# MoonLab-YH/AOD_MEH_HUA

Hardware: AMD Instinct MI355X
Metric: images/sec train+HUA-score, RetinaNet-R50 VOC 512^2 (higher is better)
Workload: dtype bf16x3

## Files before the change

aod_meh_hua_amd/_C.py:

```python
import ctypes as C
import os

import torch

_HERE = os.path.dirname(os.path.abspath(__file__))
LIB_PATH = os.environ.get('AOD_HIP_LIB') or os.path.join(_HERE, 'lib', 'libaodhip.so')


class AodHipError(RuntimeError):
    pass


if not os.path.exists(LIB_PATH):
    raise ImportError(f'{LIB_PATH} is missing: run `python -m aod_meh_hua_amd.build` (hipcc, gfx950). '
                      'There is no CPU fallback for the MEH/HUA hot path.')
lib = C.CDLL(LIB_PATH)


class ConvSeg(C.Structure):
    _fields_ = [('B', C.c_int32), ('H', C.c_int32), ('W', C.c_int32), ('OH', C.c_int32), ('OW', C.c_int32),
                ('src_row0', C.c_int64), ('dst_row0', C.c_int64)]


class ConvDesc(C.Structure):
# ... 76 lines not shown
    'aod_upsample2x_add_bwd': (C.c_int, [P, P, I32, I32, I32, I32, I32, I32, P]),
    'aod_upsample2x_add_to': (C.c_int, [P, P, P, I32, I32, I32, I32, I32, I32, P]),
    'aod_upsample2x_add_bwd_set': (C.c_int, [P, P, I32, I32, I32, I32, I32, I32, P]),
    'aod_act_bwd': (C.c_int, [P, P, P, P, P, P, P, P, P, P, I64, I32, I32, I32, P]),
    'aod_add_relu': (C.c_int, [P, P, P, I64, P]),
    'aod_pad_cast_colsum': (C.c_int, [P, P, P, P, I64, I32, I32, I32, P]),
    'aod_assign_ws_bytes': (SZ, [I32, I32]),
    'aod_max_iou_assign': (C.c_int, [P, P, I64, I32, P, P, P, I32, F32, F32, F32, I32, I32, P, P, P, P, P, P, P, P, P, I32, P, P]),
    'aod_loss_partials_len': (SZ, [I64]),
    'aod_edl_focal_l1_fwd': (C.c_int, [P, P, P, P, P, P, I64, I32, F32, F32, P, P, P, P]),
    'aod_edl_focal_l1_bwd': (C.c_int, [P, P, P, P, P, P, I64, I32, F32, F32, P, P, P, F32, I32, P, P, I32, I32, I32, I32, P]),
    'aod_edl_focal_elem': (C.c_int, [P, P, I64, I32, F32, F32, P, P, P]),
    'aod_meh_loss_fwd': (C.c_int, [P, P, P, I64, P, P, P]),
    'aod_meh_loss_bwd': (C.c_int, [P, P, P, I64, P, P, I32, I32, I32, P]),
    'aod_sigmoid_focal_l1_fwd': (C.c_int, [P, P, P, P, P, P, I64, I32, F32, F32, P, P, P, P]),
    'aod_sigmoid_focal_l1_bwd': (C.c_int, [P, P, P, P, P, P, I64, I32, F32, F32, P, P, P, F32, I32, P, P, I32, I32, I32, I32, P]),
    'aod_sigmoid_focal_elem': (C.c_int, [P, P, I64, I32, F32, F32, P, P, P]),
    'aod_sigmoid_focal_l1_levels_fwd': (C.c_int, [P, P, P, P, P, P, I32, P, I32, F32, F32, P, P, P, P, I32, P, P, P]),
    'aod_sigmoid_focal_l1_levels_bwd': (C.c_int, [P, P, P, P, P, P, I32, P, I32, F32, F32, P, P, P, P, P, I32, I32, I32, I32, P]),
    'aod_loss_levels_partials_len': (SZ, [I32, P]),
    'aod_edl_focal_l1_levels_fwd': (C.c_int, [P, P, P, P, P, P, I32, P, I32, F32, F32, P, P, P, P, I32, P, P, P]),
    'aod_edl_focal_l1_levels_bwd': (C.c_int, [P, P, P, P, P, P, I32, P, I32, F32, F32, P, P, P, P, P, I32, I32, I32, I32, P]),
    'aod_meh_loss_levels_fwd': (C.c_int, [P, P, P, I32, P, P, P, P]),
    'aod_meh_loss_levels_bwd': (C.c_int, [P, P, P, I32, P, P, P, I32, I32, I32, P]),
    'aod_meh_loss_fwd_ex': (C.c_int, [P, P, P, I64, I32, P, P, P]),
    'aod_meh_loss_bwd_ex': (C.c_int, [P, P, P, I64, I32, P, P, I32, I32, I32, P]),
    'aod_meh_loss_levels_fwd_ex': (C.c_int, [P, P, P, I32, P, I32, P, P, P]),
    'aod_meh_loss_levels_bwd_ex': (C.c_int, [P, P, P, I32, P, I32, P, P, I32, I32, I32, P]),
    'aod_softmax_rowmax': (C.c_int, [P, I32, I64, I32, F32, P, P, I32, P]),
    'aod_topk_stable': (C.c_int, [P, I32, I64, I32, P, I64, P]),
    'aod_pre_nms_levels': (C.c_int, [I32, P, P, P, P, P, P, I32, I32, F32, I32, I32, P, P, P, P, F32, P, P, P, P, P, P, P, I64, P]),
    'aod_gather_decode': (C.c_int, [P, P, P, P, P, I32, I64, I32, I32, I64, P, P, P, P, F32, P, P, P, P, I64, I64, I64, I32, P]),
    'aod_nms_ws_bytes': (SZ, [I32, I32, I32]),
    'aod_multiclass_nms': (C.c_int, [P, P, I32, I32, I32, F32, F32, I32, P, P, P, P, P, P]),
    'aod_eval_match': (C.c_int, [P, P, P, P, P, P, P, I32, I32, I32, P, I32, P, P]),
    'aod_coco_match': (C.c_int, [P, P, P, P, P, P, P, P, I32, I32, I32, P, I32, P, I32, P, P]),
    'aod_hua_ws_bytes': (SZ, [I32, I32]),
    'aod_hua_score': (C.c_int, [P, P, P, P, P, P, P, P, P, I32, I32, I32, I32, I32, F32, F32, F32, I32, U64, P, I32, I32, I32, P, P, I32, P, P, P]),
    'aod_hua_score_ex': (C.c_int, [P, P, P, P, P, P, P, P, P, I32, I32, I32, I32, I32, F32, F32, F32, I32, U64, P, I32, I32, I32, P, P, I32, P,
                                   I32, P, P, P, P]),
    'aod_hua_score_ex2': (C.c_int, [P, P, P, P, P, P, P, P, P, I32, I32, I32, I32, I32, F32, F32, F32, I32, U64, P, I32, I32, I32, P, P, I32, P,
                                    I32, I32, P, P, P, P]),
    'aod_maxpool_fwd': (C.c_int, [P, P, I32, I32, I32, I32, I32, I32, I32, I32, I32, P]),
    'aod_maxpool_bwd': (C.c_int, [P, P, P, I32, I32, I32, I32, I32, I32, I32, I32, I32, P]),
    'aod_l2norm_fwd': (C.c_int, [P, P, P, I64, I32, F32, P]),
    'aod_l2norm_bwd': (C.c_int, [P, P, P, P, P, I64, I32, F32, P]),
    'aod_ssd_loss_fwd': (C.c_int, [P, P, P, P, P, P, I32, I32, I32, I32, I32, F32, P, P, P, P]),
    'aod_ssd_loss_bwd': (C.c_int, [P, P, P, P, P, P, P, P, I32, I32, I32, I32, F32, P, P, P, P, P, P]),
    'aod_synth_normal_images': (C.c_int, [P, I32, I64, U64, P, P]),
    'aod_image_xform': (C.c_int, [P, P, I32, I32, I32, P, P]),
    'aod_x3_split': (C.c_int, [P, P, I64, I32, P]),
    'aod_x3_merge': (C.c_int, [P, P, I64, I32, P]),
    'aod_x3_add': (C.c_int, [P, P, P, I64, P]),
    'aod_x3_nchw_f32_to_s2d': (C.c_int, [P, P, I32, I32, I32, I32, P]),
    'aod_x3_maxpool3x3s2': (C.c_int, [P, P, I32, I32, I32, I32, P]),
    'aod_x3_upsample2x_add_to': (C.c_int, [P, P, P, I32, I32, I32, I32, I32, I32, P]),
    'aod_x3_upsample2x_add_bwd_set': (C.c_int, [P, P, I32, I32, I32, I32, I32, I32, P]),
    'aod_x3_act_bwd': (C.c_int, [P, P, P, P, I64, I32, I32, P]),
    'aod_x3_pad_cast_colsum': (C.c_int, [P, P, P, P, I64, I32, P]),
    'aod_x3_pad_cast_colsum_map': (C.c_int, [P, P, P, P, I64, I32, P, P]),
    'aod_x3_nchw_f32_to_nhwc': (C.c_int, [P, P, I32, I32, I32, I32, P]),
    'aod_x3_maxpool_fwd': (C.c_int, [P, P, I32, I32, I32, I32, I32, I32, I32, I32, I32, P]),
    'aod_x3_maxpool_bwd': (C.c_int, [P, P, P, I32, I32, I32, I32, I32, I32, I32, I32, I32, P]),
    'aod_x3_l2norm_fwd': (C.c_int, [P, P, P, I64, I32, F32, P]),
    'aod_x3_l2norm_bwd': (C.c_int, [P, P, P, P, P, I64, I32, F32, P]),
    'aod_sgd_multi': (C.c_int, [P, P, P, P, I32, F32, P, F32, F32, I32, F32, P]),
    'aod_sgd_multi_clipped': (C.c_int, [P, P, P, P, I32, F32, P, F32, F32, I32, F32, P, P]),
    'aod_grad_norm_multi': (C.c_int, [P, P, I32, F32, F32, I32, P, I64, P, P]),
    'aod_ensemble_mi_partials_len': (SZ, [I32, P, I32]),
    'aod_ensemble_mi': (C.c_int, [P, I32, I32, P, I32, I32, P, P, I64, P]),
    'aod_dropout2d_masks': (C.c_int, [P, P, I32, P, I32, I32, F32, U64, C.c_uint32, P]),
    'aod_dropout2d_apply': (C.c_int, [P, P, I64, I32, I32, I32, I32, P]),
    'aod_dropout2d_apply_multi': (C.c_int, [P, P, I64, I32, I32, P, P, P, I32, I32, P]),
    'aod_pool_descriptor': (C.c_int, [P, I32, P, P, I32, I32, I32, P, I64, P]),
    'aod_kcenter_chunk': (C.c_int, []),
    'aod_kcenter_ws_len': (SZ, [I64]),
    'aod_kcenter_greedy': (C.c_int, [P, I64, I32, P, I64, I64, P, P, P, P, P]),
    'aod_kcenter_greedy_ex': (C.c_int, [P, I64, I32, P, I64, I64, P, P, P, P, P, I32]),
    'aod_cdal_chunk': (C.c_int, []),
    'aod_cdal_ws_len': (SZ, [I32, P, I32, I32]),
    'aod_cdal_descriptor': (C.c_int, [P, I32, P, I32, I32, F32, P, I64, P, I64, P]),
    'aod_det_uncertainty': (C.c_int, [P, P, P, P, P, I32, I32, I32, I32, I32, I32, I32, F32, P, P, P, P]),
    'aod_loc_stability_max_levels': (C.c_int, []),
    'aod_pixel_noise': (C.c_int, [P, P, I32, I32, I32, I32, P, P, F32, I32, U64, P, P]),
    'aod_loc_stability': (C.c_int, [P, P, P, I32, I32, I32, F32, I32, I32, P, P, P]),
}
for _n, (_r, _a) in _SIGS.items():
    if hasattr(lib, _n):
        getattr(lib, _n).restype = _r
        getattr(lib, _n).argtypes = _a
lib.aod_last_error.restype = C.c_char_p


def ptr(t):
    if t is None:
        return None
    if not t.is_cuda:
        raise AodHipError('aod_meh_hua_amd ops need tensors on the MI355X (cuda:N); got a CPU tensor. There is no CPU fallback.')
    return C.c_void_p(t.data_ptr())


def stream():
    return C.c_void_p(torch.cuda.current_stream().cuda_stream)


def check(rc, name='aod'):
# ... 7 lines not shown
```

aod_meh_hua_amd/build.py:

```python
import os
import subprocess
import sys

HERE = os.path.dirname(os.path.abspath(__file__))
CSRC = os.path.join(HERE, 'csrc')
LIB = os.path.join(HERE, 'lib', 'libaodhip.so')
FLAGS = ['--offload-arch=gfx950', '-O3', '-std=c++17', '-fPIC', '-ffp-contract=off', '-Wno-unused-result']


def sources():
    return sorted(os.path.join(CSRC, f) for f in os.listdir(CSRC) if f.endswith(('.hip', '.cpp')))


def source_digest():
    import hashlib
    h = hashlib.sha256()
    for f in sources() + [os.path.join(CSRC, 'common.h'), os.path.join(CSRC, 'pointwise.h'), os.path.join(CSRC, 'conv_x3p.h'), os.path.join(CSRC, 'conv_params.h'), os.path.join(HERE, '..', 'include', 'aod_hip.h')]:
        if os.path.exists(f):
            h.update(os.path.basename(f).encode())
            h.update(open(f, 'rb').read())
    return h.hexdigest()[:16]


def needs_build():
    if not os.path.exists(LIB):
        return True
    t = os.path.getmtime(LIB)
    deps = sources() + [os.path.join(CSRC, 'common.h'), os.path.join(CSRC, 'pointwise.h'), os.path.join(CSRC, 'conv_x3p.h'), os.path.join(CSRC, 'conv_params.h'),
                        os.path.join(HERE, '..', 'include', 'aod_hip.h')]
    return any(os.path.getmtime(d) > t for d in deps)


def build(force=False, verbose=True):
    if not force and not needs_build():
        return LIB
    os.makedirs(os.path.dirname(LIB), exist_ok=True)
    objdir = os.path.join(HERE, 'lib', 'obj')
    os.makedirs(objdir, exist_ok=True)
    hipcc = os.environ.get('HIPCC', '/opt/rocm/bin/hipcc')
    procs = []
    objs = []
    for src in sources():
        obj = os.path.join(objdir, os.path.basename(src) + '.o')
        objs.append(obj)
        cmd = [hipcc] + FLAGS + (['-x', 'hip'] if src.endswith('.hip') else []) + ['-c', src, '-o', obj]
        procs.append((src, subprocess.Popen(cmd, stdout=subprocess.PIPE, stderr=subprocess.STDOUT)))
    for src, p in procs:
        out = p.communicate()[0].decode()
        if p.returncode != 0:
            raise RuntimeError(f'hipcc failed on {src}:\n{out}')
        if verbose and out.strip():
            print(out)
    subprocess.check_call([hipcc, '--offload-arch=gfx950', '-shared', '-fPIC', '-o', LIB] + objs)
    if verbose:
        print('built', LIB)
    return LIB


if __name__ == '__main__':
    build(force='--force' in sys.argv)
```

aod_meh_hua_amd/csrc/losses.hip:

```cpp
#include "common.h"

#define FLT_MIN_F 1.17549435e-38f
constexpr int LB = 256;
constexpr int MAXC = 96;

__device__ __forceinline__ float focal_pow(float b, float gamma) { return gamma == 2.f ? b * b : powf(b, gamma); }

#ifndef AOD_LOSS_FAST_MATH
#define AOD_LOSS_FAST_MATH 1
#endif
#if AOD_LOSS_FAST_MATH
__device__ __forceinline__ float l_exp(float x) { return __builtin_amdgcn_exp2f(x * 1.44269504088896341f); }
__device__ __forceinline__ float l_log(float x) { return __builtin_amdgcn_logf(x) * 0.693147180559945309f; }
__device__ __forceinline__ float l_div(float a, float b) { return a * __builtin_amdgcn_rcpf(b); }
#else
__device__ __forceinline__ float l_exp(float x) { return expf(x); }
__device__ __forceinline__ float l_log(float x) { return logf(x); }
__device__ __forceinline__ float l_div(float a, float b) { return a / b; }
#endif

template <int LPR>
__device__ __forceinline__ float grp_max(float v) {
  if (LPR >= 2) v = fmaxf(v, __shfl_xor(v, 1, 64));
  if (LPR >= 4) v = fmaxf(v, __shfl_xor(v, 2, 64));
  return v;
}
template <int LPR>
__device__ __forceinline__ float grp_sum(float v) {
  if (LPR >= 2) v += __shfl_xor(v, 1, 64);
  if (LPR >= 4) v += __shfl_xor(v, 2, 64);
  return v;
}

template <int CT, int LPR>
__device__ __forceinline__ float edl_row_fwd(const float* x, int n, int c0, long long label, float gamma, float alpha, float* p) {
  float m = -INFINITY;
#pragma unroll
  for (int c = 0; c < CT; ++c) if (c < n) m = fmaxf(m, x[c]);
  m = grp_max<LPR>(m);
  float S = 0.f;
#pragma unroll
  for (int c = 0; c < CT; ++c) if (c < n) { p[c] = l_exp(x[c] - m); S += p[c]; }
  S = grp_sum<LPR>(S);
  float tot = 0.f;
#pragma unroll
  for (int c = 0; c < CT; ++c) if (c < n) {
    const float pr = l_div(p[c], S);
    p[c] = pr;
    const float z = l_log(l_div(pr, 1.f - pr + 1e-9f) + 1e-9f);
    const float q = l_div(1.f, 1.f + l_exp(-z));
    const bool pos = label == c0 + c;
    const float lg = l_log(fmaxf(pos ? q : 1.f - q, FLT_MIN_F));
    float l;
    if (pos) l = -alpha * focal_pow(1.f - q, gamma) * lg;
    else l = -(1.f - alpha) * focal_pow(q, gamma) * lg;
    tot += l;
  }
  return grp_sum<LPR>(tot);
}

constexpr int FORM_EDL = 0, FORM_SIGMOID = 1;

__device__ __forceinline__ float sig_focal_term(float x, bool pos, float gamma, float alpha, float* gz) {
  const float q = l_div(1.f, 1.f + l_exp(-x));
  const float lg = l_log(fmaxf(pos ? q : 1.f - q, FLT_MIN_F));
  if (gz) {
    if (pos) *gz = -alpha * focal_pow(1.f - q, gamma) * (1.f - q - gamma * q * lg);
    else *gz = -(1.f - alpha) * focal_pow(q, gamma) * (gamma * (1.f - q) * lg - q);
  }
  return pos ? -alpha * focal_pow(1.f - q, gamma) * lg : -(1.f - alpha) * focal_pow(q, gamma) * lg;
}

template <int CT, int LPR>
__device__ __forceinline__ float sig_row_fwd(const float* x, int n, int c0, long long label, float gamma, float alpha) {
  float tot = 0.f;
#pragma unroll
  for (int c = 0; c < CT; ++c) if (c < n) tot += sig_focal_term(x[c], label == c0 + c, gamma, alpha, nullptr);
  return grp_sum<LPR>(tot);
}

constexpr int MAXLV = 8;
struct LossLevels { int n; int blk_end[MAXLV]; long long row_end[MAXLV]; };
__device__ __forceinline__ void level_of_block(const LossLevels& lv, int bid, int& level, int& blk0, long long& row0, long long& rend) {
  level = 0; blk0 = 0; row0 = 0; rend = lv.row_end[0];
#pragma unroll
  for (int q = 0; q + 1 < MAXLV; ++q)
    if (bid >= lv.blk_end[q]) { level = q + 1; blk0 = lv.blk_end[q]; row0 = lv.row_end[q]; rend = lv.row_end[q + 1]; }
}
static int fill_levels(LossLevels& lv, int nlevels, const int64_t* level_rows, int rows_per_block, long long& total_rows) {
  lv.n = nlevels;
  long long r = 0, b = 0;
  for (int l = 0; l < MAXLV; ++l) {
    if (l < nlevels) { r += level_rows[l]; b += (level_rows[l] + rows_per_block - 1) / rows_per_block; }
    lv.row_end[l] = r;
    lv.blk_end[l] = l < nlevels ? (int)b : 0x7fffffff;
  }
  total_rows = r;
  return (int)b;
}

template <int FORM, int CT, int LPR>
__global__ __launch_bounds__(LB) void edl_l1_fwd_kernel(const float* __restrict__ cls, const long long* __restrict__ labels,
                                                        const float* __restrict__ lw, const float* __restrict__ bp,
                                                        const float* __restrict__ bt, const float* __restrict__ bw, const LossLevels lv, int C,
                                                        float gamma, float alpha, float* __restrict__ loss_noR, float* __restrict__ partials) {
  extern __shared__ __attribute__((aligned(16))) float srow[];
  constexpr int RB = LB / LPR;
  const int P = C | 1;
  int level, blk0; long long row0, rend;
  level_of_block(lv, (int)blockIdx.x, level, blk0, row0, rend);
  const long long r0 = row0 + (long long)((int)blockIdx.x - blk0) * RB;
  const int nr = (int)min((long long)RB, rend - r0);
  aod_stage_rows<LB>(cls + r0 * C, srow, nr, C, P);
  __syncthreads();
  float s_cls = 0.f, s_box = 0.f, s_nor = 0.f;
  const int lrow = threadIdx.x / LPR, part = threadIdx.x % LPR;
  const bool live = lrow < nr;
  const int row = live ? lrow : nr - 1;
  const int cpl = (C + LPR - 1) / LPR, c0 = part * cpl;
  const int n = min(cpl, C - c0);
  {
    const long long r = r0 + row;
    float x[CT], p[CT];
#pragma unroll
    for (int c = 0; c < CT; ++c) x[c] = c < n ? srow[row * P + c0 + c] : 0.f;
    const float l = FORM == FORM_SIGMOID ? sig_row_fwd<CT, LPR>(x, n, c0, labels[r], gamma, alpha)
                                         : edl_row_fwd<CT, LPR>(x, n, c0, labels[r], gamma, alpha, p);
    if (live && part == 0) {
      loss_noR[r] = l;
      s_nor = l;
      s_cls = l * lw[r];
      if (bp) {
        const f32x4 a = *reinterpret_cast<const f32x4*>(bp + r * 4), b = *reinterpret_cast<const f32x4*>(bt + r * 4),
                    w = *reinterpret_cast<const f32x4*>(bw + r * 4);
        for (int j = 0; j < 4; ++j) s_box += fabsf(a[j] - b[j]) * w[j];
      }
    }
  }
  __shared__ float red[3][LB / 64];
  s_cls = wave_sum(s_cls); s_box = wave_sum(s_box); s_nor = wave_sum(s_nor);
  if ((threadIdx.x & 63) == 0) { red[0][threadIdx.x >> 6] = s_cls; red[1][threadIdx.x >> 6] = s_box; red[2][threadIdx.x >> 6] = s_nor; }
  __syncthreads();
  if (threadIdx.x < 3) {
    float v = 0.f;
    for (int i = 0; i < LB / 64; ++i) v += red[threadIdx.x][i];
    partials[(long long)blockIdx.x * 3 + threadIdx.x] = v;
  }
}

__global__ __launch_bounds__(256) void reduce_partials_kernel(const float* __restrict__ partials, long long nblocks, int k, float* __restrict__ out) {
  __shared__ float red[4];
// ... 162 lines not shown
#pragma unroll
    for (int c = 0; c < CT; ++c) x[c] = c < n ? srow[row * P + c0 + c] : 0.f;
    float m = -INFINITY, S = 0.f;
    if (FORM == FORM_EDL) {
#pragma unroll
      for (int c = 0; c < CT; ++c) if (c < n) m = fmaxf(m, x[c]);
      m = grp_max<LPR>(m);
#pragma unroll
      for (int c = 0; c < CT; ++c) if (c < n) { p[c] = l_exp(x[c] - m); S += p[c]; }
      S = grp_sum<LPR>(S);
    }
    const long long label = labels[r];
    const float gc_ = g_div ? g_cls[gl] / g_div[gl] : g_cls[gl];
    const float gn_ = g_noR ? (g_noR_bcast ? (g_div ? g_noR[gl] / g_div[2 * nlv + gl] : g_noR[gl]) : g_noR[r]) : g_noR_s;
    const float coef = gc_ * lw[r] + gn_;
    float dot = 0.f;
    if (FORM == FORM_SIGMOID) {
      if (live) {
#pragma unroll
        for (int c = 0; c < CT; ++c) if (c < n) {
          float gz;
          sig_focal_term(x[c], label == c0 + c, gamma, alpha, &gz);
          srow[row * P + c0 + c] = coef * gz;
        }
      }
    } else {
#pragma unroll
      for (int c = 0; c < CT; ++c) if (c < n) {
        const float pr = l_div(p[c], S);
        p[c] = pr;
        const float om = 1.f - pr + 1e-9f;
        const float u = l_div(pr, om);
        const float z = l_log(u + 1e-9f);
        const float q = l_div(1.f, 1.f + l_exp(-z));
        const bool pos = label == c0 + c;
        const float lg = l_log(fmaxf(pos ? q : 1.f - q, FLT_MIN_F));
        float gz;
        if (pos) gz = -alpha * focal_pow(1.f - q, gamma) * (1.f - q - gamma * q * lg);
        else gz = -(1.f - alpha) * focal_pow(q, gamma) * (gamma * (1.f - q) * lg - q);
        const float g = l_div(coef * gz * (1.f + 1e-9f), om * om * (u + 1e-9f));
        gp[c] = g;
        dot += pr * g;
      }
      dot = grp_sum<LPR>(dot);
      if (live) {
#pragma unroll
        for (int c = 0; c < CT; ++c) if (c < n) srow[row * P + c0 + c] = p[c] * (gp[c] - dot);
      }
    }
    if (live && part == 0 && bp && grad_bbox) {
      const float gb = g_div ? g_bbox[gl] / g_div[nlv + gl] : g_bbox[gl];
      const long long bb = (r / A) * pitch_box + (r % A) * 4;
      for (int j = 0; j < 4; ++j) {
        const float d = bp[r * 4 + j] - bt[r * 4 + j];
        const float sgn = d > 0.f ? 1.f : (d < 0.f ? -1.f : 0.f);
        const float gx = sgn * bw[r * 4 + j] * gb;
        if (OUT_BF16) ((bf16_t*)grad_bbox)[bb + j] = (bf16_t)gx;
        else ((float*)grad_bbox)[bb + j] = gx;
      }
    }
  }
  __syncthreads();
  {
    const int drow = LB / C, dcol = LB - drow * C;
    int row = (int)threadIdx.x / C, c = (int)threadIdx.x - row * C;
    for (int i = threadIdx.x; i < tot; i += LB) {
      const long long o = s_obase[row] + c;
      const float gx = srow[row * P + c];
      if (OUT_BF16) ((bf16_t*)grad_cls)[o] = (bf16_t)gx;
      else ((float*)grad_cls)[o] = gx;
      row += drow; c += dcol;
      if (c >= C) { c -= C; ++row; }
    }
  }
}

#define AOD_FOCAL_BWD_(FORM_, BF, LPR_)                                                                                                    \
  hipLaunchKernelGGL((edl_l1_bwd_kernel<FORM_, BF, 24, LPR_>), dim3((unsigned)nb), dim3(LB), (size_t)(LB / LPR_) * (C | 1) * 4, (hipStream_t)stream, cls, \
                     (const long long*)labels, label_w, bbox_pred, bbox_tgt, bbox_w, lv, C, gamma, alpha, g_cls, g_bbox, g_noR, \
                     g_noR_scalar, g_noR_is_scalar, grad_cls, grad_bbox, A, pitch_cls, pitch_box, g_lstride, g_div, nlv_)
#define AOD_FOCAL_BWD_F(FORM_)                                                                                                             \
  do {                                                                                                                                     \
    if (out_bf16) { if (C <= 24) AOD_FOCAL_BWD_(FORM_, true, 1); else AOD_FOCAL_BWD_(FORM_, true, 4); }                                    \
    else { if (C <= 24) AOD_FOCAL_BWD_(FORM_, false, 1); else AOD_FOCAL_BWD_(FORM_, false, 4); }                                           \
  } while (0)
#define AOD_FOCAL_BWD()                                                                                                                    \
  do {                                                                                                                                     \
    if (form == FORM_SIGMOID) AOD_FOCAL_BWD_F(FORM_SIGMOID); else AOD_FOCAL_BWD_F(FORM_EDL);                                               \
  } while (0)
static int focal_l1_bwd(int form, const char* nm, const float* cls, const int64_t* labels, const float* label_w, const float* bbox_pred,
                        const float* bbox_tgt, const float* bbox_w, int64_t nrows, int C, float gamma, float alpha, const float* g_cls,
                        const float* g_bbox, const float* g_noR, float g_noR_scalar, int g_noR_is_scalar, void* grad_cls, void* grad_bbox,
                        int out_bf16, int A, int pitch_cls, int pitch_box, aod_stream_t stream) {
  AOD_CHECK_ARG(nrows >= 0, "%s: negative row count", nm);
  if (nrows == 0) return 0;
  AOD_CHECK_ARG(cls && labels && label_w && g_cls && grad_cls, "%s: null pointer", nm);
  AOD_CHECK_ARG(C >= 1 && C <= MAXC && A >= 1 && pitch_cls >= A * C, "%s: bad C/A/pitch", nm);
  AOD_CHECK_ARG(!grad_bbox || (bbox_pred && bbox_tgt && bbox_w && g_bbox && pitch_box >= A * 4), "%s: bbox args", nm);
  LossLevels lv; long long tot;
  const long long nb = fill_levels(lv, 1, &nrows, LB / edl_lpr(C), tot);
  const int g_lstride = 0, nlv_ = 1;
  const float* const g_div = nullptr;
  AOD_FOCAL_BWD();
  AOD_LAUNCH_CHECK();
  return 0;
}
extern "C" int aod_edl_focal_l1_bwd(const float* cls, const int64_t* labels, const float* label_w, const float* bbox_pred,
                                    const float* bbox_tgt, const float* bbox_w, int64_t nrows, int C, float gamma, float alpha,
                                    const float* g_cls, const float* g_bbox, const float* g_noR, float g_noR_scalar, int g_noR_is_scalar,
                                    void* grad_cls, void* grad_bbox, int out_bf16, int A, int pitch_cls, int pitch_box, aod_stream_t stream) {
  return focal_l1_bwd(FORM_EDL, "edl_bwd", cls, labels, label_w, bbox_pred, bbox_tgt, bbox_w, nrows, C, gamma, alpha, g_cls, g_bbox, g_noR, g_noR_scalar,
                      g_noR_is_scalar, grad_cls, grad_bbox, out_bf16, A, pitch_cls, pitch_box, stream);
}
extern "C" int aod_sigmoid_focal_l1_bwd(const float* cls, const int64_t* labels, const float* label_w, const float* bbox_pred,
                                        const float* bbox_tgt, const float* bbox_w, int64_t nrows, int C, float gamma, float alpha,
                                        const float* g_cls, const float* g_bbox, const float* g_noR, float g_noR_scalar, int g_noR_is_scalar,
                                        void* grad_cls, void* grad_bbox, int out_bf16, int A, int pitch_cls, int pitch_box, aod_stream_t stream) {
  return focal_l1_bwd(FORM_SIGMOID, "sigmoid_focal_bwd", cls, labels, label_w, bbox_pred, bbox_tgt, bbox_w, nrows, C, gamma, alpha, g_cls, g_bbox, g_noR,
                      g_noR_scalar, g_noR_is_scalar, grad_cls, grad_bbox, out_bf16, A, pitch_cls, pitch_box, stream);
}

static int focal_l1_levels_bwd(int form, const char* nm, const float* cls, const int64_t* labels, const float* label_w, const float* bbox_pred,
                               const float* bbox_tgt, const float* bbox_w, int nlevels, const int64_t* level_rows, int C, float gamma, float alpha,
                               const float* g_sums, const float* divisors, const float* g_noR_rows, void* grad_cls, void* grad_bbox, int out_bf16,
                               int A, int pitch_cls, int pitch_box, aod_stream_t stream) {
  AOD_CHECK_ARG(nlevels >= 1 && nlevels <= MAXLV && level_rows, "%s: 1..8 levels", nm);
  AOD_CHECK_ARG(level_rows_ok(nlevels, level_rows), "%s: negative row count", nm);
  AOD_CHECK_ARG(cls && labels && label_w && g_sums && grad_cls, "%s: null pointer", nm);
  AOD_CHECK_ARG(C >= 1 && C <= MAXC && A >= 1 && pitch_cls >= A * C, "%s: bad C/A/pitch", nm);
  AOD_CHECK_ARG(!grad_bbox || (bbox_pred && bbox_tgt && bbox_w && pitch_box >= A * 4), "%s: bbox args", nm);
  LossLevels lv; long long tot;
  const int nb = fill_levels(lv, nlevels, level_rows, LB / edl_lpr(C), tot);
  if (nb == 0) return 0;
  const float* g_cls = g_sums; const float* g_bbox = g_sums + nlevels;
  const float* g_noR = g_noR_rows ? g_noR_rows : g_sums + 2 * nlevels;
  const float g_noR_scalar = 0.f; const int g_noR_is_scalar = g_noR_rows ? 0 : 1, g_lstride = 1, nlv_ = nlevels;
  const float* const g_div = divisors;
  AOD_FOCAL_BWD();
  AOD_LAUNCH_CHECK();
  return 0;
}
#undef AOD_FOCAL_BWD
#undef AOD_FOCAL_BWD_F
#undef AOD_FOCAL_BWD_
extern "C" int aod_edl_focal_l1_levels_bwd(const float* cls, const int64_t* labels, const float* label_w, const float* bbox_pred,
                                           const float* bbox_tgt, const float* bbox_w, int nlevels, const int64_t* level_rows, int C, float gamma,
                                           float alpha, const float* g_sums, const float* divisors, const float* g_noR_rows, void* grad_cls,
                                           void* grad_bbox, int out_bf16, int A, int pitch_cls, int pitch_box, aod_stream_t stream) {
  return focal_l1_levels_bwd(FORM_EDL, "edl_levels_bwd", cls, labels, label_w, bbox_pred, bbox_tgt, bbox_w, nlevels, level_rows, C, gamma, alpha, g_sums,
                             divisors, g_noR_rows, grad_cls, grad_bbox, out_bf16, A, pitch_cls, pitch_box, stream);
}
extern "C" int aod_sigmoid_focal_l1_levels_bwd(const float* cls, const int64_t* labels, const float* label_w, const float* bbox_pred,
                                               const float* bbox_tgt, const float* bbox_w, int nlevels, const int64_t* level_rows, int C, float gamma,
                                               float alpha, const float* g_sums, const float* divisors, const float* g_noR_rows, void* grad_cls,
                                               void* grad_bbox, int out_bf16, int A, int pitch_cls, int pitch_box, aod_stream_t stream) {
  return focal_l1_levels_bwd(FORM_SIGMOID, "sigmoid_focal_levels_bwd", cls, labels, label_w, bbox_pred, bbox_tgt, bbox_w, nlevels, level_rows, C, gamma,
                             alpha, g_sums, divisors, g_noR_rows, grad_cls, grad_bbox, out_bf16, A, pitch_cls, pitch_box, stream);
}

__device__ __forceinline__ float sign0(float x) { return x > 0.f ? 1.f : (x < 0.f ? -1.f : 0.f); }
template <int FORM>
__global__ __launch_bounds__(256) void meh_fwd_kernel(const float* __restrict__ lam, const float* __restrict__ loss, const float* __restrict__ bw4,
                                                      const LossLevels lv, float* __restrict__ partials) {
  float s = 0.f;
  int level, blk0; long long row0, n;
  level_of_block(lv, (int)blockIdx.x, level, blk0, row0, n);
  const long long i = row0 + (long long)((int)blockIdx.x - blk0) * 256 + threadIdx.x;
  if (i < n) {
    if (FORM == 1) {
      s = fabsf(fabsf(lam[i] + 1e-9f - loss[i]) * bw4[i * 4]);
    } else if (FORM == 2) {
      const float d = fabsf(logf(lam[i] + 1e-9f + 1.f) - logf(loss[i] + 1.f)) * bw4[i * 4];
      s = d * d;
    } else {
      const float d = fabsf(lam[i] + 1e-9f - loss[i]) * bw4[i * 4];
      s = d * d;
    }
  }
  __shared__ float red[4];
  s = wave_sum(s);
  if ((threadIdx.x & 63) == 0) red[threadIdx.x >> 6] = s;
  __syncthreads();
  if (threadIdx.x == 0) partials[blockIdx.x] = red[0] + red[1] + red[2] + red[3];
}
template <bool OUT_BF16, int FORM>
__global__ void meh_bwd_kernel(const float* __restrict__ lam, const float* __restrict__ loss, const float* __restrict__ bw4, const LossLevels lv,
                               const float* __restrict__ g, void* __restrict__ grad, int A, int pitch, int g_lstride) {
  int level, blk0; long long row0, n;
  level_of_block(lv, (int)blockIdx.x, level, blk0, row0, n);
  const long long i = row0 + (long long)((int)blockIdx.x - blk0) * 256 + threadIdx.x;
  if (i < n) {
    const float w = bw4[i * 4];
    float v;
    if (FORM == 1) {
      const float d = lam[i] + 1e-9f - loss[i];
      v = g[level * g_lstride] * sign0(fabsf(d) * w) * w * sign0(d);
    } else if (FORM == 2) {
      const float x = lam[i] + 1e-9f + 1.f;
      const float d = logf(x) - logf(loss[i] + 1.f);
      v = g[level * g_lstride] * 2.f * (fabsf(d) * w) * w * sign0(d) / x;
    } else {
      v = g[level * g_lstride] * 2.f * w * w * (lam[i] + 1e-9f - loss[i]);
    }
    const long long o = (i / A) * pitch + (i % A);
    if (OUT_BF16) ((bf16_t*)grad)[o] = (bf16_t)v; else ((float*)grad)[o] = v;
  }
}
#define AOD_MEH_FWD(nb_)                                                                                                                   \
  do {                                                                                                                                     \
    if (form == 1) hipLaunchKernelGGL(meh_fwd_kernel<1>, dim3((unsigned)(nb_)), dim3(256), 0, (hipStream_t)stream, lam, loss_noR, bbox_w4, lv, partials); \
    else if (form == 2) hipLaunchKernelGGL(meh_fwd_kernel<2>, dim3((unsigned)(nb_)), dim3(256), 0, (hipStream_t)stream, lam, loss_noR, bbox_w4, lv, partials); \
    else hipLaunchKernelGGL(meh_fwd_kernel<0>, dim3((unsigned)(nb_)), dim3(256), 0, (hipStream_t)stream, lam, loss_noR, bbox_w4, lv, partials); \
  } while (0)
#define AOD_MEH_BWD_(BF, F_, nb_, ls_)                                                                                                     \
  hipLaunchKernelGGL((meh_bwd_kernel<BF, F_>), dim3((unsigned)(nb_)), dim3(256), 0, (hipStream_t)stream, lam, loss_noR, bbox_w4, lv, g, grad_lam, A, pitch, ls_)
#define AOD_MEH_BWD(nb_, ls_)                                                                                                              \
  do {                                                                                                                                     \
    if (out_bf16) { if (form == 1) AOD_MEH_BWD_(true, 1, nb_, ls_); else if (form == 2) AOD_MEH_BWD_(true, 2, nb_, ls_); else AOD_MEH_BWD_(true, 0, nb_, ls_); } \
    else { if (form == 1) AOD_MEH_BWD_(false, 1, nb_, ls_); else if (form == 2) AOD_MEH_BWD_(false, 2, nb_, ls_); else AOD_MEH_BWD_(false, 0, nb_, ls_); } \
  } while (0)
extern "C" int aod_meh_loss_fwd_ex(const float* lam, const float* loss_noR, const float* bbox_w4, int64_t n, int form, float* out_sum,
                                   float* partials, aod_stream_t stream) {
  AOD_CHECK_ARG(lam && loss_noR && bbox_w4 && out_sum && partials, "meh_fwd: null pointer");
  AOD_CHECK_ARG(form >= 0 && form <= 2, "meh_fwd: form must be 0 (L2), 1 (L1) or 2 (MSLE)");
  if (n == 0) return 0;
  LossLevels lv; long long tot;
  const long long nb = fill_levels(lv, 1, &n, 256, tot);
  AOD_MEH_FWD(nb);
  hipLaunchKernelGGL(reduce_partials_kernel, dim3(1), dim3(256), 0, (hipStream_t)stream, partials, nb, 1, out_sum);
  AOD_LAUNCH_CHECK();
  return 0;
}
extern "C" int aod_meh_loss_fwd(const float* lam, const float* loss_noR, const float* bbox_w4, int64_t n, float* out_sum, float* partials,
                                aod_stream_t stream) {
  return aod_meh_loss_fwd_ex(lam, loss_noR, bbox_w4, n, 0, out_sum, partials, stream);
}
extern "C" int aod_meh_loss_levels_fwd_ex(const float* lam, const float* loss_noR, const float* bbox_w4, int nlevels, const int64_t* level_rows,
                                          int form, float* out_sums, float* partials, aod_stream_t stream) {
  AOD_CHECK_ARG(nlevels >= 1 && nlevels <= MAXLV && level_rows, "meh_levels_fwd: 1..8 levels");
  AOD_CHECK_ARG(lam && loss_noR && bbox_w4 && out_sums && partials, "meh_levels_fwd: null pointer");
  AOD_CHECK_ARG(form >= 0 && form <= 2, "meh_levels_fwd: form must be 0 (L2), 1 (L1) or 2 (MSLE)");
  LossLevels lv; long long tot;
  const int nb = fill_levels(lv, nlevels, level_rows, 256, tot);
  if (nb) AOD_MEH_FWD(nb);
  hipLaunchKernelGGL(reduce_partials_levels_kernel, dim3(nlevels), dim3(256), 0, (hipStream_t)stream, partials, lv, 1, out_sums, 1, nlevels, (const int*)nullptr,
                     0, (float*)nullptr, (float*)nullptr);
  AOD_LAUNCH_CHECK();
  return 0;
}
extern "C" int aod_meh_loss_levels_fwd(const float* lam, const float* loss_noR, const float* bbox_w4, int nlevels, const int64_t* level_rows,
                                       float* out_sums, float* partials, aod_stream_t stream) {
  return aod_meh_loss_levels_fwd_ex(lam, loss_noR, bbox_w4, nlevels, level_rows, 0, out_sums, partials, stream);
}
extern "C" int aod_meh_loss_bwd_ex(const float* lam, const float* loss_noR, const float* bbox_w4, int64_t n, int form, const float* g,
                                   void* grad_lam, int out_bf16, int A, int pitch, aod_stream_t stream) {
  AOD_CHECK_ARG(lam && loss_noR && bbox_w4 && g && grad_lam && A >= 1 && pitch >= A, "meh_bwd: bad args");
// ... 109 lines not shown
```

aod_meh_hua_amd/csrc/x3_ops.hip:

```cpp
#include "common.h"

static inline int grid_for(long long nvec) {
  long long b = (nvec + 255) / 256;
  return (int)(b > 2048 ? 2048 : (b < 1 ? 1 : b));
}

__device__ __forceinline__ int xoct(int q) { return ((q >> 2) << 6) + ((q & 3) << 3); }

__device__ __forceinline__ void xload(const bf16_t* __restrict__ p, float (&v)[8]) {
  const bf16x8 h = *reinterpret_cast<const bf16x8*>(p), l = *reinterpret_cast<const bf16x8*>(p + 32);
#pragma unroll
  for (int j = 0; j < 8; ++j) v[j] = (float)h[j] + (float)l[j];
}
__device__ __forceinline__ void xstore(bf16_t* __restrict__ p, const float (&v)[8]) {
  bf16x8 h, l;
#pragma unroll
  for (int j = 0; j < 8; ++j) { h[j] = (bf16_t)v[j]; l[j] = (bf16_t)(v[j] - (float)h[j]); }
  *reinterpret_cast<bf16x8*>(p) = h;
  *reinterpret_cast<bf16x8*>(p + 32) = l;
}

__global__ void x3_split_kernel(const float* __restrict__ src, bf16_t* __restrict__ dst, long long M, int C, int Q) {
  const long long n = M * Q;
  for (long long i = blockIdx.x * (long long)blockDim.x + threadIdx.x; i < n; i += (long long)gridDim.x * blockDim.x) {
    const int q = (int)(i % Q); const long long m = i / Q;
    float v[8];
#pragma unroll
    for (int j = 0; j < 8; ++j) v[j] = (q * 8 + j < C) ? src[m * C + q * 8 + j] : 0.f;
    xstore(dst + m * (Q >> 2) * 64 + xoct(q), v);
  }
}
extern "C" int aod_x3_split(const float* src, void* dst, int64_t M, int C, aod_stream_t stream) {
  AOD_CHECK_ARG(src && dst && C >= 1, "x3_split: bad args");
  if (M == 0) return 0;
  const int Q = (C + 31) / 32 * 4;
  hipLaunchKernelGGL(x3_split_kernel, dim3(grid_for(M * Q)), dim3(256), 0, (hipStream_t)stream, src, (bf16_t*)dst, (long long)M, C, Q);
  AOD_LAUNCH_CHECK();
  return 0;
}
__global__ void x3_merge_kernel(const bf16_t* __restrict__ src, float* __restrict__ dst, long long M, int C, int Q) {
  const long long n = M * Q;
  for (long long i = blockIdx.x * (long long)blockDim.x + threadIdx.x; i < n; i += (long long)gridDim.x * blockDim.x) {
    const int q = (int)(i % Q); const long long m = i / Q;
    float v[8];
    xload(src + m * (Q >> 2) * 64 + xoct(q), v);
#pragma unroll
    for (int j = 0; j < 8; ++j)
      if (q * 8 + j < C) dst[m * C + q * 8 + j] = v[j];
  }
}
extern "C" int aod_x3_merge(const void* src, float* dst, int64_t M, int C, aod_stream_t stream) {
  AOD_CHECK_ARG(src && dst && C >= 1, "x3_merge: bad args");
  if (M == 0) return 0;
  const int Q = (C + 31) / 32 * 4;
  hipLaunchKernelGGL(x3_merge_kernel, dim3(grid_for(M * Q)), dim3(256), 0, (hipStream_t)stream, (const bf16_t*)src, dst, (long long)M, C, Q);
  AOD_LAUNCH_CHECK();
  return 0;
}

__global__ void x3_add_kernel(const bf16_t* __restrict__ a, const bf16_t* __restrict__ b, bf16_t* __restrict__ o, long long nq) {
  for (long long i = blockIdx.x * (long long)blockDim.x + threadIdx.x; i < nq; i += (long long)gridDim.x * blockDim.x) {
    const long long off = (i >> 2) * 64 + ((i & 3) << 3);
    float x[8], y[8];
    xload(a + off, x); xload(b + off, y);
#pragma unroll
    for (int j = 0; j < 8; ++j) x[j] += y[j];
    xstore(o + off, x);
  }
}
extern "C" int aod_x3_add(const void* a, const void* b, void* out, int64_t n, aod_stream_t stream) {
  AOD_CHECK_ARG(a && b && out && n % 64 == 0, "x3_add: n (bf16 elements) must be a multiple of 64");
  if (n == 0) return 0;
  hipLaunchKernelGGL(x3_add_kernel, dim3(grid_for(n / 16)), dim3(256), 0, (hipStream_t)stream, (const bf16_t*)a, (const bf16_t*)b, (bf16_t*)out, (long long)(n / 16));
  AOD_LAUNCH_CHECK();
  return 0;
}

__global__ void x3_nchw_to_s2d_kernel(const float* __restrict__ src, bf16_t* __restrict__ dst, int B, int C, int H, int W) {
  const int H2 = H >> 1, W2 = W >> 1;
  const long long n = (long long)B * H2 * W2;
  for (long long i = blockIdx.x * (long long)blockDim.x + threadIdx.x; i < n; i += (long long)gridDim.x * blockDim.x) {
    const int X = (int)(i % W2); long long r = i / W2;
    const int Y = (int)(r % H2); const long long b = r / H2;
    float v[32];
#pragma unroll
    for (int k = 0; k < 32; ++k) v[k] = 0.f;
    for (int c = 0; c < C; ++c)
#pragma unroll
      for (int dy = 0; dy < 2; ++dy) {
        const float2 p = *reinterpret_cast<const float2*>(src + ((b * C + c) * H + 2 * Y + dy) * (long long)W + 2 * X);
        v[(dy * 2 + 0) * C + c] = p.x;
        v[(dy * 2 + 1) * C + c] = p.y;
      }
#pragma unroll
    for (int q = 0; q < 4; ++q) {
      float u[8];
#pragma unroll
      for (int j = 0; j < 8; ++j) u[j] = v[q * 8 + j];
      xstore(dst + i * 64 + q * 8, u);
    }
  }
}
extern "C" int aod_x3_nchw_f32_to_s2d(const float* src, void* dst, int B, int C, int H, int W, aod_stream_t stream) {
  AOD_CHECK_ARG(src && dst && C >= 1 && C <= 4 && H % 2 == 0 && W % 2 == 0, "x3_nchw_to_s2d: C <= 4 and even H, W required (C %d, %d x %d)", C, H, W);
  hipLaunchKernelGGL(x3_nchw_to_s2d_kernel, dim3(grid_for((long long)B * (H / 2) * (W / 2))), dim3(256), 0, (hipStream_t)stream, src, (bf16_t*)dst, B, C, H, W);
  AOD_LAUNCH_CHECK();
  return 0;
}

__global__ void x3_maxpool_kernel(const bf16_t* __restrict__ src, bf16_t* __restrict__ dst, int B, int H, int W, int Q, int OH, int OW) {
  const long long n = (long long)B * OH * OW * Q;
  const int CP = (Q >> 2) * 64;
  for (long long i = blockIdx.x * (long long)blockDim.x + threadIdx.x; i < n; i += (long long)gridDim.x * blockDim.x) {
    const int q = i % Q; long long r = i / Q;
    const int ox = r % OW; r /= OW;
    const int oy = r % OH; const int b = r / OH;
    float m[8];
#pragma unroll
    for (int j = 0; j < 8; ++j) m[j] = -INFINITY;
    for (int dy = 0; dy < 3; ++dy) {
      const int y = oy * 2 - 1 + dy;
      if ((unsigned)y >= (unsigned)H) continue;
      for (int dx = 0; dx < 3; ++dx) {
        const int x = ox * 2 - 1 + dx;
        if ((unsigned)x >= (unsigned)W) continue;
        float v[8];
        xload(src + (((long long)b * H + y) * W + x) * CP + xoct(q), v);
#pragma unroll
        for (int j = 0; j < 8; ++j) m[j] = fmaxf(m[j], v[j]);
      }
    }
    xstore(dst + (i / Q) * CP + xoct(q), m);
  }
}
extern "C" int aod_x3_maxpool3x3s2(const void* src, void* dst, int B, int H, int W, int C, aod_stream_t stream) {
  AOD_CHECK_ARG(src && dst && C % 64 == 0, "x3_maxpool: the X-layout width must be a multiple of 64");
  const int OH = (H + 2 - 3) / 2 + 1, OW = (W + 2 - 3) / 2 + 1, Q = C / 16;
  hipLaunchKernelGGL(x3_maxpool_kernel, dim3(grid_for((long long)B * OH * OW * Q)), dim3(256), 0, (hipStream_t)stream, (const bf16_t*)src, (bf16_t*)dst,
                     B, H, W, Q, OH, OW);
  AOD_LAUNCH_CHECK();
  return 0;
}

__global__ void x3_upsample_add_kernel(const bf16_t* __restrict__ src, const bf16_t* __restrict__ lat, bf16_t* __restrict__ dst, int B, int h, int w,
                                       int Q, int H, int W) {
  const long long n = (long long)B * H * W * Q;
  const int CP = (Q >> 2) * 64;
  for (long long i = blockIdx.x * (long long)blockDim.x + threadIdx.x; i < n; i += (long long)gridDim.x * blockDim.x) {
    const int q = i % Q; long long r = i / Q;
    const long long pix = r;
    const int x = r % W; r /= W;
    const int y = r % H; const int b = r / H;
    const int sy = min((int)(((long long)y * h) / H), h - 1), sx = min((int)(((long long)x * w) / W), w - 1);
    float s[8], d[8];
    xload(src + (((long long)b * h + sy) * w + sx) * CP + xoct(q), s);
    xload(lat + pix * CP + xoct(q), d);
#pragma unroll
    for (int j = 0; j < 8; ++j) d[j] += s[j];
    xstore(dst + pix * CP + xoct(q), d);
  }
}
extern "C" int aod_x3_upsample2x_add_to(const void* top, const void* lateral, void* out, int B, int h, int w, int C, int H, int W, aod_stream_t stream) {
  AOD_CHECK_ARG(top && lateral && out && C % 64 == 0, "x3_upsample_add_to: the X-layout width must be a multiple of 64");
  hipLaunchKernelGGL(x3_upsample_add_kernel, dim3(grid_for((long long)B * H * W * (C / 16))), dim3(256), 0, (hipStream_t)stream, (const bf16_t*)top,
                     (const bf16_t*)lateral, (bf16_t*)out, B, h, w, C / 16, H, W);
  AOD_LAUNCH_CHECK();
  return 0;
}
__global__ void x3_upsample_add_bwd_kernel(const bf16_t* __restrict__ gd, bf16_t* __restrict__ gs, int B, int h, int w, int Q, int H, int W) {
  const long long n = (long long)B * h * w * Q;
  const int CP = (Q >> 2) * 64;
  for (long long i = blockIdx.x * (long long)blockDim.x + threadIdx.x; i < n; i += (long long)gridDim.x * blockDim.x) {
    const int q = i % Q; long long r = i / Q;
    const long long pix = r;
    const int sx = r % w; r /= w;
    const int sy = r % h; const int b = r / h;
    const int y0 = (int)(((long long)sy * H + h - 1) / h), y1 = min(H, (int)(((long long)(sy + 1) * H + h - 1) / h));
    const int x0 = (int)(((long long)sx * W + w - 1) / w), x1 = min(W, (int)(((long long)(sx + 1) * W + w - 1) / w));
    float a[8];
#pragma unroll
    for (int j = 0; j < 8; ++j) a[j] = 0.f;
    for (int y = y0; y < y1; ++y)
      for (int x = x0; x < x1; ++x) {
        float v[8];
        xload(gd + (((long long)b * H + y) * W + x) * CP + xoct(q), v);
#pragma unroll
        for (int j = 0; j < 8; ++j) a[j] += v[j];
      }
    xstore(gs + pix * CP + xoct(q), a);
  }
}
extern "C" int aod_x3_upsample2x_add_bwd_set(const void* g_dst, void* g_src, int B, int h, int w, int C, int H, int W, aod_stream_t stream) {
  AOD_CHECK_ARG(g_dst && g_src && C % 64 == 0, "x3_upsample_add_bwd_set: the X-layout width must be a multiple of 64");
  hipLaunchKernelGGL(x3_upsample_add_bwd_kernel, dim3(grid_for((long long)B * h * w * (C / 16))), dim3(256), 0, (hipStream_t)stream, (const bf16_t*)g_dst,
                     (bf16_t*)g_src, B, h, w, C / 16, H, W);
  AOD_LAUNCH_CHECK();
  return 0;
}

__global__ __launch_bounds__(256) void x3_act_bwd_kernel(const bf16_t* __restrict__ g, const bf16_t* __restrict__ a, bf16_t* __restrict__ dz,
                                                         float* __restrict__ colsum, long long M, int Q, int relu, int rows_per_block, float* __restrict__ cs_ws) {
  __shared__ float sb[8][256 + 8];
  const int t = threadIdx.x, cc = t & 31, rl = t >> 5;
  const int q = blockIdx.x * 32 + cc;
  const int CP = (Q >> 2) * 64;
  const long long r0 = (long long)blockIdx.y * rows_per_block, r1 = min(M, r0 + rows_per_block);
  float s[8];
#pragma unroll
  for (int j = 0; j < 8; ++j) s[j] = 0.f;
  if (q < Q) {
    const int col = xoct(q);
    for (long long m = r0 + rl; m < r1; m += 8) {
      float v[8];
      xload(g + m * CP + col, v);
      if (relu) {
        const bf16x8 av = *reinterpret_cast<const bf16x8*>(a + m * CP + col);
#pragma unroll
        for (int j = 0; j < 8; ++j) v[j] = ((float)av[j] > 0.f) ? v[j] : 0.f;
      }
#pragma unroll
      for (int j = 0; j < 8; ++j) s[j] += v[j];
      if (dz) xstore(dz + m * CP + col, v);
    }
  }
#pragma unroll
  for (int j = 0; j < 8; ++j) sb[rl][cc * 8 + j] = s[j];
  __syncthreads();
  const int n = blockIdx.x * 256 + t;
  if (colsum && n < Q * 8) {
    float b = 0.f;
#pragma unroll
    for (int r = 0; r < 8; ++r) b += sb[r][t];
    if (cs_ws) cs_ws[(long long)blockIdx.y * (Q * 8) + n] = b;
    else atomicAdd(colsum + n, b);
  }
}
extern "C" int aod_x3_act_bwd(const void* g, const void* a, void* dz, float* colsum, int64_t M, int C, int relu, aod_stream_t stream) {
  AOD_CHECK_ARG(g && C % 64 == 0 && M >= 0, "x3_act_bwd: the X-layout width must be a multiple of 64");
  AOD_CHECK_ARG(!relu || a, "x3_act_bwd: relu needs the forward output");
  if (M == 0) return 0;
  const int Q = C / 16, panels = (Q + 31) / 32;
  long long want = 2048 / panels;
  if (want < 1) want = 1;
  long long rpb = (M + want - 1) / want;
  if (rpb < 64) rpb = 64;
  rpb = (rpb + 7) / 8 * 8;
  const int gy = (int)((M + rpb - 1) / rpb);
  float* const cs_ws = colsum ? aod_det_scratch((size_t)gy * Q * 8) : nullptr;
  hipLaunchKernelGGL(x3_act_bwd_kernel, dim3(panels, gy), dim3(256), 0, (hipStream_t)stream, (const bf16_t*)g, (const bf16_t*)a,
                     (bf16_t*)dz, colsum, (long long)M, Q, relu, (int)rpb, cs_ws);
  AOD_LAUNCH_CHECK();
  if (cs_ws) return aod_colsum_finalize(cs_ws, gy, Q * 8, Q * 8, colsum, nullptr, 0, (hipStream_t)stream);
  return 0;
}

__global__ __launch_bounds__(256) void x3_pad_cast_colsum_kernel(const float* __restrict__ g, const float* __restrict__ a, bf16_t* __restrict__ dz,
                                                                 float* __restrict__ colsum, long long M, int N, int Np, int rows_per_block, int TC,
                                                                 float* __restrict__ cs_ws, unsigned char* __restrict__ map) {
  __shared__ float red[256];
  const int RP = 256 / TC;
  const int c0 = threadIdx.x % TC, rl = threadIdx.x / TC;
  const long long r0 = (long long)blockIdx.x * rows_per_block, r1 = min(M, r0 + rows_per_block);
  for (int cb = 0; cb < Np; cb += TC) {
    const int c = cb + c0;
    const int col = ((c >> 5) << 6) + (c & 31);
    float s = 0.f;
    if (c < Np) {
      for (long long m = r0 + rl; m < r1; m += RP) {
        float v = 0.f;
        if (c < N) {
          v = g[m * N + c];
          if (a && !(a[m * N + c] > 0.f)) v = 0.f;
          if (map && !(v == 0.f)) map[m >> 6] = 1;
        }
        const bf16_t h = (bf16_t)v;
        dz[m * 2 * Np + col] = h;
        dz[m * 2 * Np + col + 32] = (bf16_t)(v - (float)h);
        s += v;
      }
    }
    __syncthreads();
    red[threadIdx.x] = s;
    __syncthreads();
    if (rl == 0 && c < N) {
      float tsum = 0.f;
      for (int r = 0; r < RP; ++r) tsum += red[r * TC + c0];
      if (cs_ws) cs_ws[(long long)blockIdx.x * N + c] = tsum;
      else atomicAdd(colsum + c, tsum);
    }
  }
}
__global__ __launch_bounds__(256) void x3_pad_cast_colsum_v8_kernel(const float* __restrict__ g, const float* __restrict__ a, bf16_t* __restrict__ dz,
                                                                    float* __restrict__ colsum, long long M, int N, int Np, int rows_per_block, int TC8,
                                                                    float* __restrict__ cs_ws, unsigned char* __restrict__ map) {
  __shared__ float red[256][9];
  const int RP = 256 / TC8;
  const int c8 = threadIdx.x % TC8, rl = threadIdx.x / TC8;
  const long long r0 = (long long)blockIdx.x * rows_per_block, r1 = min(M, r0 + rows_per_block);
  const int c = c8 * 8;
  const int col = ((c >> 5) << 6) + (c & 31);
  float s[8] = {0.f, 0.f, 0.f, 0.f, 0.f, 0.f, 0.f, 0.f};
  if (c < Np) {
    const bool lo = c + 4 <= N, hi = c + 8 <= N;
    for (long long m = r0 + rl; m < r1; m += RP) {
      f32x4 v0 = {0.f, 0.f, 0.f, 0.f}, v1 = {0.f, 0.f, 0.f, 0.f};
      if (lo) v0 = *reinterpret_cast<const f32x4*>(g + m * N + c);
      if (hi) v1 = *reinterpret_cast<const f32x4*>(g + m * N + c + 4);
      if (a) {
        if (lo) { const f32x4 a0 = *reinterpret_cast<const f32x4*>(a + m * N + c);
#pragma unroll
                  for (int j = 0; j < 4; ++j) if (!(a0[j] > 0.f)) v0[j] = 0.f; }
        if (hi) { const f32x4 a1 = *reinterpret_cast<const f32x4*>(a + m * N + c + 4);
#pragma unroll
                  for (int j = 0; j < 4; ++j) if (!(a1[j] > 0.f)) v1[j] = 0.f; }
      }
      float v[8];
#pragma unroll
      for (int j = 0; j < 4; ++j) { v[j] = v0[j]; v[4 + j] = v1[j]; }
      if (map) {
        bool nz = false;
#pragma unroll
        for (int j = 0; j < 8; ++j) nz = nz || !(v[j] == 0.f);
        if (nz) map[m >> 6] = 1;
      }
      xstore(dz + m * 2 * Np + col, v);
#pragma unroll
      for (int j = 0; j < 8; ++j) s[j] += v[j];
    }
  }
#pragma unroll
  for (int j = 0; j < 8; ++j) red[threadIdx.x][j] = s[j];
  __syncthreads();
  if (threadIdx.x < N) {
    const int cc = threadIdx.x, q8 = cc >> 3, j = cc & 7;
    float tsum = 0.f;
    for (int r = 0; r < RP; ++r) tsum += red[r * TC8 + q8][j];
    if (cs_ws) cs_ws[(long long)blockIdx.x * N + cc] = tsum;
    else atomicAdd(colsum + cc, tsum);
  }
}

extern "C" int aod_x3_pad_cast_colsum_map(const float* g, const float* relu_out_f32, void* dz, float* colsum, int64_t M, int N, void* map_,
                                          aod_stream_t stream) {
  if (M == 0) return 0;
  unsigned char* const map = (unsigned char*)map_;
  AOD_CHECK_ARG(g && dz && colsum && N >= 1, "x3_pad_cast_colsum: bad args");
  if (map && hipMemsetAsync(map, 0, (size_t)((M + 63) / 64), (hipStream_t)stream) != hipSuccess) return aod_set_err(-3, "x3_pad_cast_colsum: memset of the map failed");
  const int Np = (N + 31) / 32 * 32;
  if ((N & 3) == 0 && Np <= 256 && (((size_t)g | (size_t)(relu_out_f32 ? relu_out_f32 : g)) & 15) == 0) {
    int tc8 = 4;
    while (tc8 * 8 < Np) tc8 <<= 1;
    int rpb = (int)((M + 1023) / 1024);
    if (rpb < 64) rpb = 64;
    const int nb = (int)((M + rpb - 1) / rpb);
    float* const cs_ws = aod_det_scratch((size_t)nb * N);
    hipLaunchKernelGGL(x3_pad_cast_colsum_v8_kernel, dim3(nb), dim3(256), 0, (hipStream_t)stream, g, relu_out_f32, (bf16_t*)dz, colsum, (long long)M, N, Np,
                       rpb, tc8, cs_ws, map);
    AOD_LAUNCH_CHECK();
    if (cs_ws) return aod_colsum_finalize(cs_ws, nb, N, N, colsum, nullptr, 0, (hipStream_t)stream);
    return 0;
  }
  int rpb = (int)((M + 1023) / 1024);
  if (rpb < 16) rpb = 16;
  int tc = 32;
  while (tc < Np && tc < 256) tc <<= 1;
  const int nb = (int)((M + rpb - 1) / rpb);
  float* const cs_ws = aod_det_scratch((size_t)nb * N);
  hipLaunchKernelGGL(x3_pad_cast_colsum_kernel, dim3(nb), dim3(256), 0, (hipStream_t)stream, g, relu_out_f32, (bf16_t*)dz, colsum,
                     (long long)M, N, Np, rpb, tc, cs_ws, map);
  AOD_LAUNCH_CHECK();
  if (cs_ws) return aod_colsum_finalize(cs_ws, nb, N, N, colsum, nullptr, 0, (hipStream_t)stream);
  return 0;
}

extern "C" int aod_x3_pad_cast_colsum(const float* g, const float* relu_out_f32, void* dz, float* colsum, int64_t M, int N, aod_stream_t stream) {
  return aod_x3_pad_cast_colsum_map(g, relu_out_f32, dz, colsum, M, N, nullptr, stream);
}

__global__ void x3_nchw_to_nhwc_kernel(const float* __restrict__ src, bf16_t* __restrict__ dst, int B, int C, int HW) {
  const long long n = (long long)B * HW * 4;
  for (long long i = blockIdx.x * (long long)blockDim.x + threadIdx.x; i < n; i += (long long)gridDim.x * blockDim.x) {
    const int q = (int)(i & 3); const long long pix = i >> 2;
    const long long b = pix / HW, px = pix - b * HW;
    float v[8];
#pragma unroll
    for (int j = 0; j < 8; ++j) { const int c = q * 8 + j; v[j] = c < C ? src[(b * C + c) * HW + px] : 0.f; }
    xstore(dst + pix * 64 + q * 8, v);
  }
}
extern "C" int aod_x3_nchw_f32_to_nhwc(const float* src, void* dst, int B, int C, int H, int W, aod_stream_t stream) {
  AOD_CHECK_ARG(src && dst && C >= 1 && C <= 32, "x3_nchw_to_nhwc: at most 32 channels (got %d)", C);
  hipLaunchKernelGGL(x3_nchw_to_nhwc_kernel, dim3(grid_for((long long)B * H * W * 4)), dim3(256), 0, (hipStream_t)stream, src, (bf16_t*)dst, B, C, H * W);
  AOD_LAUNCH_CHECK();
  return 0;
}

__global__ void x3_maxpool_fwd_kernel(const bf16_t* __restrict__ x, bf16_t* __restrict__ y, int B, int H, int W, int Q, int OH, int OW, int k, int s, int p) {
  const long long n = (long long)B * OH * OW * Q;
  const int CP = (Q >> 2) * 64;
  for (long long i = blockIdx.x * (long long)blockDim.x + threadIdx.x; i < n; i += (long long)gridDim.x * blockDim.x) {
    const int q = i % Q; long long r = i / Q;
    const int ox = r % OW; r /= OW;
    const int oy = r % OH; const int b = r / OH;
    float m[8];
#pragma unroll
    for (int j = 0; j < 8; ++j) m[j] = -INFINITY;
    for (int dy = 0; dy < k; ++dy) {
      const int yy = oy * s - p + dy;
      if ((unsigned)yy >= (unsigned)H) continue;
      for (int dx = 0; dx < k; ++dx) {
        const int xx = ox * s - p + dx;
        if ((unsigned)xx >= (unsigned)W) continue;
        float v[8];
        xload(x + (((long long)b * H + yy) * W + xx) * CP + xoct(q), v);
#pragma unroll
        for (int j = 0; j < 8; ++j) m[j] = fmaxf(m[j], v[j]);
      }
    }
    xstore(y + (i / Q) * CP + xoct(q), m);
  }
}
__global__ void x3_maxpool_bwd_kernel(const bf16_t* __restrict__ x, const bf16_t* __restrict__ g, bf16_t* __restrict__ gx, int B, int H, int W, int Q,
                                      int OH, int OW, int k, int s, int p) {
  const long long n = (long long)B * H * W * Q;
  const int CP = (Q >> 2) * 64;
// ... 154 lines not shown
```

aod_meh_hua_amd/functional.py:

```python
import torch
from torch.autograd import Function

from . import hipops as ho
from .hipops import Seg


def as_rows(x):
    B, C, H, W = x.shape
    xr = x.permute(0, 2, 3, 1)
    if not xr.is_contiguous():
        xr = xr.contiguous()
    return xr.view(B * H * W, C)


def as_nchw(rows, B, H, W):
    return rows.view(B, H, W, rows.shape[1]).permute(0, 3, 1, 2)


def multi_rows(tensors):
    rows = [as_rows(t) for t in tensors]
    if len(rows) == 1:
        t = tensors[0]
        return rows[0], [Seg(t.shape[0], t.shape[2], t.shape[3], 0)]
    rb = rows[0].shape[1] * rows[0].element_size()
# ... 122 lines not shown
                r.wf, r.wd = it.wf.data_ptr(), (it.wd.data_ptr() if it.wd is not None else None)
                r.scale, r.shift, r.invstd = ((t.data_ptr() if t is not None else None) for t in (it.scale, it.shift, it.invstd))
                r.O, r.I, r.RS, r.Ipad, r.Opad = it.dims
                r.blk0, r.eps, r.pad_ = blk, it.eps, int(it.x3)
                blk += it.nblk
            host = torch.frombuffer(bytearray(bytes(recs)), dtype=torch.uint8)
            dev = self.order[stale[0]].wf.device
            ent = self.tables[stale] = (host.to(dev), blk)
        self.table = ent[0]
        ho.call('aod_param_prep', ho.ptr(ent[0]), len(stale), ent[1], ho.stream())
        for i in stale:
            self.order[i].ver = self._versions(self.order[i])


PREP = ParamPrep()


import os as _os
_FUSE_ACT = _os.environ.get('AOD_FUSE_ACT', '1') != '0'


_PREC = _os.environ.get('AOD_CONV_PREC', 'bf16x3')
assert _PREC in ('bf16', 'bf16x3'), f'AOD_CONV_PREC={_PREC!r}: bf16x3 (reference precision) or bf16 (fast mode)'
ho.X3 = _PREC == 'bf16x3'


def set_precision(p):
    global _PREC
    assert p in ('bf16', 'bf16x3')
    _PREC = p
    ho.X3 = p == 'bf16x3'


def x3_to_f32(x, channels=None):
    if not ho.X3 or x.dtype != torch.bfloat16:
        return x.float()
    B, Wd, H, W = x.shape
    rows = ho.x3_merge(as_rows(x), channels)
    return as_nchw(rows, B, H, W)


class ForkFn(Function):

    @staticmethod
    def forward(ctx, x, n):
        return tuple(x.view_as(x) for _ in range(n))

    @staticmethod
    def backward(ctx, *gs):
        tot = None
        for g in gs:
            if g is None:
                continue
            g = g.contiguous(memory_format=torch.channels_last)
            tot = g if tot is None else as_nchw(ho.x3_add(as_rows(tot), as_rows(g)), g.shape[0], g.shape[2], g.shape[3])
        return tot, None


def fork(x, n):
    if not ho.X3 or n == 1 or not (torch.is_grad_enabled() and x.requires_grad):
        return [x] * n
    return list(ForkFn.apply(x, n))


def get_precision():
    return _PREC


def mode_key():
    return (_PREC, bool(ho.DETERMINISTIC))


class ActSlot:
    __slots__ = ('masked', 's1', 'res_ok', 'res_grad')

    def __init__(self):
        self.masked, self.s1 = False, None
        self.res_ok, self.res_grad = False, None


class BwdChain:
    __slots__ = ('meta', 'x_rows', 'prep', 'out')

    def __init__(self):
        self.meta, self.x_rows, self.prep, self.out = {}, {}, {}, {}


def bwd_chain_for(blk, x):
    on = _os.environ.get('AOD_FUSE_BOTTLENECK_BWD', '1') != '0' and not ho.DETERMINISTIC
    if ho.X3 and _os.environ.get('AOD_FUSE_BOTTLENECK128_X3_BWD', '1') == '0':
        return None
    return BwdChain() if on and _FUSE_ACT and bottleneck128_train_applies(blk, x) else None


def set_deterministic(on=True):
    ho.set_deterministic(on)


class GradAcc:
    __slots__ = ('n', 'arrived', 'partial', 'slot', '__weakref__')

    def __init__(self, slot=None):
        self.n, self.arrived, self.partial = 0, 0, None
        self.slot = slot


_JUNCTIONS = []


def share_input_grad(x):
    if torch.is_grad_enabled() and x.requires_grad and _os.environ.get('AOD_GRAD_JUNCTIONS', '1') != '0':
        x._aod_acc = GradAcc(getattr(x, '_aod_slot', None) if _FUSE_ACT and _os.environ.get('AOD_JUNCTION_MASK', '1') != '0' else None)
        _JUNCTIONS.append(_weakref.ref(x._aod_acc))
    return x

# ... 26 lines not shown
        return False


def cut(x):
    if _CUTS is None or not torch.is_grad_enabled() or not x.requires_grad:
        return x
    xc = x.detach().requires_grad_()
    if getattr(x, '_aod_slot', None) is not None:
        xc._aod_slot = x._aod_slot
    _CUTS.append((x, xc))
    return xc


def backward_segments(loss, cuts, after=None):
    loss.backward()
    if after is not None:
        after(0)
    for k, (x, xc) in enumerate(reversed(cuts)):
        g, xc.grad = xc.grad, None
        if g is not None:
            x.backward(g)
        if after is not None:
            after(k + 1)


def _grad_rows(gouts, y_segs, O, device):
    if len(gouts) == 1 and gouts[0] is not None:
        return as_rows(gouts[0])
    parts = []
    for g, s in zip(gouts, y_segs):
        parts.append(as_rows(g) if g is not None else torch.zeros(s.rows, O, device=device, dtype=torch.bfloat16))
    dt = torch.float32 if any(p.dtype == torch.float32 for p in parts) else torch.bfloat16
    rb = O * parts[0].element_size()
    adjacent = all(p.dtype == dt and p.is_contiguous() for p in parts) and all(
        parts[i + 1].data_ptr() == parts[i].data_ptr() + parts[i].shape[0] * rb for i in range(len(parts) - 1))
    if adjacent:
        return torch.as_strided(parts[0], (sum(p.shape[0] for p in parts), O), (O, 1))
    return torch.cat([p.to(dt) for p in parts])


def _grad_slice(w, device):
    dst = getattr(w, '_aod_grad_view', None)
    if dst is not None and (w.__dict__.get('_aod_view_busy') or dst.device != device
                            or (w.grad is not None and w.grad.data_ptr() == dst.data_ptr())):
        dst = None
    if dst is not None:
        w._aod_view_busy = True
        dst = dst.detach()
    return dst


_S1_OF = {}
_ROW_MAPS = {}
MAP_LOG = None
FWD_MAP_LOG = None


def _map_of(dz):
    e = _ROW_MAPS.get(dz.data_ptr())
    return e[0] if e is not None and e[1].shape == dz.shape and e[1].dtype == dz.dtype and ho.sparse_bwd() else None


def _keep_map(dx, rmap):
    if rmap is not None:
        if MAP_LOG is not None:
            MAP_LOG.append((tuple(dx.shape), rmap))
        _WgradQueue.begin_pass()
        _ROW_MAPS[dx.data_ptr()] = (rmap, dx)


class _WgradQueue:
    jobs, seen, task, deferred = [], set(), -1, []
    sparse_jobs = []
    enabled = _os.environ.get('AOD_WGRAD_GROUP', '1') != '0'

    @classmethod
    def flush(cls):
        for name in ('jobs', 'sparse_jobs'):
            jobs = getattr(cls, name)
            setattr(cls, name, [])
            if jobs:
                ho.wgrad_unpack_group(jobs)

    @classmethod
    def _verify(cls):
        deferred, cls.deferred = cls.deferred, []
        for _, pref, t in deferred:
            p = pref()
            if p is None or p.grad is None:
                continue
            g = p.grad
            if g.data_ptr() != t.data_ptr() and g.shape == t.shape:
                g.copy_(t)

    @classmethod
    def _end_of_pass(cls):
        cls.task = -1
        cls.seen.clear()
        _S1_OF.clear()
        _ROW_MAPS.clear()
        cls.flush()
        cls._verify()

    @classmethod
    def begin_pass(cls):
        tid = torch._C._current_graph_task_id()
        if tid != cls.task:
            cls.flush()
            cls.deferred = []
            cls.task = tid
            cls.seen.clear()
            _S1_OF.clear()
            _ROW_MAPS.clear()
            if tid >= 0:
                torch.autograd.Variable._execution_engine.queue_callback(cls._end_of_pass)

    @classmethod
    def submit(cls, job, wid, defer):
        cls.begin_pass()
        if wid in cls.seen or not (defer and cls.enabled) or ho.DETERMINISTIC:
            cls.flush()
            job.run_alone()
            cls.deferred = [e for e in cls.deferred if e[0] != wid]
            cls.seen.add(wid)
            return False
        cls.seen.add(wid)
        name = 'sparse_jobs' if job.zmap is not None else 'jobs'
        q = getattr(cls, name)
        if q and ho.wgrad_group_splits(q + [job]) is None:
            setattr(cls, name, [])
            ho.wgrad_unpack_group(q)
            q = getattr(cls, name)
        q.append(job)
        if len(q) == 4:
            setattr(cls, name, [])
            ho.wgrad_unpack_group(q)
        return True


def _wgrad(x_rows, x_segs, dz, dsegs, R, S, stride, pad, dil, alg, w, O, I, dst, scale=None, bn=None, gamma=None, zmap=None):
    dev = dz.device
    gw = dst if dst is not None else torch.empty(O, I, R, S, dtype=torch.float32, device=dev)
    wdot = torch.empty(O, dtype=torch.float32, device=dev) if bn is not None else None
    job = ho.WgradJob(x_rows, x_segs, dz, dsegs, R, S, stride, pad, dil, alg, O, I, gw.detach(), scale=scale,
                      w=w.detach() if bn is not None else None, wdot=wdot.detach() if wdot is not None else None,
                      bn=tuple(t.detach() for t in bn) if bn is not None else None, zmap=zmap)
    hooked = lambda p: p is not None and bool(p._backward_hooks or getattr(p, '_post_accumulate_grad_hooks', None))
    defer = (R * S <= 9 and w.grad is None and (gamma is None or gamma.grad is None) and not torch.is_grad_enabled()
             and not torch.is_anomaly_enabled() and not hooked(w) and not hooked(gamma))
    if _WgradQueue.submit(job, id(w), defer):
        _WgradQueue.deferred.append((id(w), _weakref.ref(w), job.gw))
        if job.wdot is not None and gamma is not None:
            _WgradQueue.deferred.append((id(w), _weakref.ref(gamma), job.wdot))
    return gw, wdot


class ConvFn(Function):

    @staticmethod
    def forward(ctx, meta, w, gamma, beta, mean, var, bias, res, *xs):
        O, I, R, S = w.shape
        cin = xs[0].shape[1]
        x_rows, x_segs = multi_rows(xs)
        pi = PREP.get(w, (gamma, beta, mean, var) if gamma is not None else None, cin, meta['eps'])
        wp, scale, shift, invstd = pi.wf, pi.scale, pi.shift, pi.invstd
        if gamma is None and bias is not None:
            shift = bias.detach()
        res_rows = as_rows(res) if res is not None else None
        out_rows = as_rows(meta['out']) if meta.get('out') is not None else None
        if meta.get('pre') is not None:
            y_rows, y_segs = meta['pre'], ho.out_segs(x_segs, R, S, meta['stride'], meta['pad'], meta['dil'])
        else:
            r = ho.conv2d_rows(x_rows, x_segs, wp, O, R, S, meta['stride'], meta['pad'], meta['dil'], pre_scale=scale,
                               pre_shift=shift, res=res_rows, relu=meta['relu'], out_f32=meta['out_f32'], out=out_rows, alg=(I, O))
            y_rows, y_segs = r[0], r[1]
        ctx.meta, ctx.x_segs, ctx.y_segs = meta, x_segs, y_segs
        ctx.has_bn, ctx.has_bias, ctx.has_res = gamma is not None, bias is not None, res is not None
        ctx.nx = len(xs)
        ctx.scope = ho.SCOPE
        ctx.save_for_backward(w, gamma, mean, scale, invstd, x_rows, y_rows if meta['relu'] else None)
        if meta.get('chain') is not None:
            ch, role = meta['chain']
            ch.meta[role], ch.x_rows[role], ch.prep[role] = meta, x_rows, (w, gamma, mean, cin, x_segs)
        outs = tuple(as_nchw(y_rows[s.row0:s.row0 + s.rows], s.B, s.H, s.W) for s in y_segs)
        return outs

    @staticmethod
    def backward(ctx, *gouts):
        with ho.scope(ctx.scope):
            return ConvFn._backward(ctx, *gouts)

    @staticmethod
    def _backward(ctx, *gouts):
        w, gamma, mean, scale, invstd, x_rows, a_rows = ctx.saved_tensors
        meta = ctx.meta
        O, I, R, S = w.shape
        cin = x_rows.shape[1]
        y_segs = ctx.y_segs
        X = ho.X3
        Opad = ho.xw(O) if X else (O + 7) // 8 * 8
        g_rows = _grad_rows(gouts, y_segs, O if (meta['out_f32'] or not X) else Opad, w.device)
        dsegs = dense_segs(y_segs)
        need_w = ctx.needs_input_grad[1]
        need_x = any(ctx.needs_input_grad[8:])
        need_res = ctx.has_res and ctx.needs_input_grad[7]
        gw = ggamma = gbeta = gbias = gres = None
        if (meta['out_f32'] and X) or (Opad != O and not X):
            if meta.get('sparse_grad') and X and ho.sparse_bwd():
                dz, gbias_v, rmap = ho.pad_cast_colsum(g_rows, Opad, a_rows if meta['relu'] else None, want_map=True)
                _keep_map(dz, rmap)
            else:
                dz, gbias_v = ho.pad_cast_colsum(g_rows, Opad, a_rows if meta['relu'] else None)
            gm = None
        else:
            relu = meta['relu']
            slot = meta.get('slot')
            if slot is not None and slot.masked and g_rows.dtype == torch.bfloat16:
                dz, s1 = g_rows, slot.s1
                slot.masked, slot.s1 = False, None
            else:
                plain = (not relu) and g_rows.dtype == torch.bfloat16
                known = _S1_OF.pop(g_rows.data_ptr(), None) if plain and _os.environ.get('AOD_S1_REUSE', '1') != '0' else None
                if known is not None and known[1].shape == g_rows.shape:
                    dz, s1 = g_rows, known[0]
                else:
                    dz, _, s1, _ = ho.act_bwd(g_rows, a_rows, None, None, None, None, relu=relu, want_gm=False, want_dz=not plain)
                    if plain:
                        dz = g_rows
            gbias_v = s1
        need_bn = ctx.has_bn and ctx.needs_input_grad[2]
        if ctx.has_bias and ctx.needs_input_grad[6]:
            gbias = gbias_v[:O]
        if need_res:
            res_slot = meta.get('res_slot')
            if res_slot is not None:
                res_slot.res_grad = dz
            else:
                s = y_segs[0]
                gres = as_nchw(dz, s.B, s.H, s.W)
                if (Opad == O or X) and len(y_segs) == 1:
                    _WgradQueue.begin_pass()
                    _S1_OF[dz.data_ptr()] = (s1, dz)
        x_segs = ctx.x_segs
        if need_w or need_bn:
            dst = _grad_slice(w, dz.device) if need_w else None
            gw, ggamma = _wgrad(x_rows, x_segs, dz, dsegs, R, S, meta['stride'], meta['pad'], meta['dil'], (I, O), w, O, I, dst,
                                scale=scale if ctx.has_bn else None, bn=(s1, mean, invstd) if need_bn else None, gamma=gamma if need_bn else None,
                                zmap=_map_of(dz))
            if need_bn:
                gbeta = s1
            if not need_w:
                gw = None
        gxs = [None] * ctx.nx
        if need_x:
            wd = PREP.get(w, (gamma, None, mean, None) if ctx.has_bn else None, cin, meta['eps']).wd
            if ho.width(I) != cin or wd is None:
                raise RuntimeError('dgrad through a channel-padded input is not supported')
            xd = dense_segs(x_segs)
            in_slot = meta.get('in_slot')
            fuse = in_slot is not None and all(a.row0 == b.row0 for a, b in zip(x_segs, xd)) and all(ctx.needs_input_grad[8:])
            s1_in = ho.zeros_f32(I, dz.device) if fuse else None
# ... 47 lines not shown
                    acc.partial, acc.arrived = None, 0
        return (None, gw, ggamma, gbeta, None, None, gbias, gres) + tuple(gxs)


def _chain_ready(ch, meta3):
    if set(ch.meta) != {1, 2, 3} or ch.out:
        return False
    m1, m2 = ch.meta[1], ch.meta[2]
    sl1, sl2 = m1.get('in_slot'), m2.get('in_slot')
    if sl1 is None or sl2 is None or meta3.get('res_slot') is not sl1 or sl1.res_grad is None:
        return False
    if m1.get('in_acc') is not None or m2.get('in_acc') is not None:
        return False
    for r in (1, 2, 3):
        segs = ch.prep[r][4]
        if len(segs) != 1 or segs[0].row0 != 0:
            return False
    return True


def conv_bn_act(xs, w, bn=None, bias=None, res=None, stride=1, pad=0, dil=1, relu=False, out_f32=False, out=None, sole_consumer=False,
                shared_input=False, pre=None, chain=None, sparse_grad=False):
    single = torch.is_tensor(xs)
    xl = [xs] if single else list(xs)
    meta = dict(stride=stride, pad=pad, dil=dil, relu=relu, out_f32=out_f32, eps=bn.eps if bn is not None else 0.0, out=out, pre=pre,
                sparse_grad=bool(sparse_grad and out_f32))
    if chain is not None and torch.is_grad_enabled():
        meta['chain'] = chain
    if torch.is_grad_enabled():
        if relu and not out_f32:
            meta['slot'] = ActSlot()
        if sole_consumer and _FUSE_ACT:
            slots = [getattr(x, '_aod_slot', None) for x in xl]
            if slots[0] is not None and all(sl is slots[0] for sl in slots) and all(x.requires_grad for x in xl):
                if sole_consumer != 'res' or len(xl) == 1:
                    meta['in_slot'] = slots[0]
                    slots[0].res_ok = sole_consumer == 'res'
        if shared_input and len(xl) == 1:
            acc = getattr(xl[0], '_aod_acc', None)
            if acc is not None and 'in_slot' not in meta:
                meta['in_acc'] = acc
                acc.n += 1
        rs = getattr(res, '_aod_slot', None) if res is not None else None
        if rs is not None and rs.res_ok:
            meta['res_slot'] = rs
            rs.res_ok = False
    if bn is not None:
        outs = ConvFn.apply(meta, w, bn.weight, bn.bias, bn.running_mean, bn.running_var, None, res, *xl)
    else:
        outs = ConvFn.apply(meta, w, None, None, None, None, bias, res, *xl)
    if meta.get('slot') is not None:
        for o in outs:
            o._aod_slot = meta['slot']
    return outs[0] if single else list(outs)


class ConvPairFn(Function):

    @staticmethod
    def forward(ctx, meta, wA, bA, wB, bB, *xs):
        nl = len(xs) // 2
        O, I, R, S = wA.shape
        rows, segs = zip(multi_rows(xs[:nl]), multi_rows(xs[nl:]))
        assert segs[0] == segs[1] and wB.shape == wA.shape, 'paired tower convs need identical geometry'
        cin = rows[0].shape[1]
        pis = [PREP.get(w, None, cin, 0.0) for w in (wA, wB)]
        rows, wfs, shifts = list(rows), [pi.wf for pi in pis], [bA.detach(), bB.detach()]
        rider = meta.get('rider')
        if rider is not None:
            convL, xL = rider
            rows.append(xL)
            wfs.append(PREP.get(convL.weight, None, cin, 0.0).wf)
            shifts.append(convL.bias.detach())
        fmap = meta.get('fwd_map')
        omaps = [None, fmap] + ([fmap] if rider is not None else []) if fmap is not None else None
        if FWD_MAP_LOG is not None:
            FWD_MAP_LOG.append((len(rows), (sum(s.rows for s in segs[0]), ho.width(O)), omaps))
        outs, y_segs = ho.conv2d_rows_grouped(rows, list(segs[0]), wfs, O, R, S, 1, meta['pad'], meta['dil'], pre_shifts=shifts, relu=True,
                                              alg=(I, O), omaps=omaps)
        if rider is not None:
            meta['rider_out'] = outs[2]
        ctx.meta, ctx.x_segs, ctx.y_segs, ctx.nl = meta, list(segs[0]), y_segs, nl
        ctx.save_for_backward(wA, wB, rows[0], rows[1], outs[0], outs[1])
        return tuple(as_nchw(o[s.row0:s.row0 + s.rows], s.B, s.H, s.W) for o in outs[:2] for s in y_segs)

    @staticmethod
    def backward(ctx, *gouts):
        wA, wB, xA, xB, yA, yB = ctx.saved_tensors
        meta, nl, y_segs, x_segs = ctx.meta, ctx.nl, ctx.y_segs, ctx.x_segs
        O, I, R, S = wA.shape
        dsegs, xd = dense_segs(y_segs), dense_segs(x_segs)
        dzs, gws, gbs = [], [], []
        for gi, (w, x_rows, a_rows) in enumerate(((wA, xA, yA), (wB, xB, yB))):
            g_rows = _grad_rows(gouts[gi * nl:(gi + 1) * nl], y_segs, ho.width(O), w.device)
            slot = meta['slot'][gi]
            if slot is not None and slot.masked and g_rows.dtype == torch.bfloat16:
                dz, s1 = g_rows, slot.s1
                slot.masked, slot.s1 = False, None
            else:
                dz, _, s1, _ = ho.act_bwd(g_rows, a_rows, None, None, None, None, relu=True, want_gm=False, want_dz=True)
            dzs.append(dz)
            gbs.append(s1[:O] if ctx.needs_input_grad[2 + 2 * gi] else None)
            gw = None
            if ctx.needs_input_grad[1 + 2 * gi]:
                gw, _ = _wgrad(x_rows, x_segs, dz, dsegs, R, S, 1, meta['pad'], meta['dil'], (I, O), w, O, I, _grad_slice(w, dz.device),
                               zmap=_map_of(dz))
            gws.append(gw)
# ... 295 lines not shown
            and tuple(conv.stride) == (2, 2) and tuple(conv.padding) == (3, 3) and tuple(conv.dilation) == (1, 1) and conv.bias is None
            and not conv.weight.requires_grad and not any(p.requires_grad for p in bn.parameters()) and not bn.training)


def stem_conv_s2d(img, conv, bn):
    B, Cc, H, W = img.shape
    O = conv.weight.shape[0]
    rows, segs = ho.nchw_to_s2d_rows(img.detach())
    w4 = _stem_w4(conv)
    pi = PREP.get(w4, (bn.weight, bn.bias, bn.running_mean, bn.running_var), rows.shape[1], bn.eps)
    dst = [Seg(B, H // 2, W // 2, 0)]
    y, _ = ho.conv2d_rows(rows, segs, pi.wf, O, 4, 4, 1, 2, 1, pre_scale=pi.scale, pre_shift=pi.shift, relu=True, dst_segs=dst,
                          alg=(49.0 * Cc / 16.0, O))
    return as_nchw(y, B, H // 2, W // 2)


def stem_pool_s2d(img, conv, bn):
    B, Cc, H, W = img.shape
    O = conv.weight.shape[0]
    if _os.environ.get('AOD_STEM_POOL_FUSE', '1') == '0' or (ho.X3 and (Cc != 3 or O != 64)):
        return max_pool_3x3_s2(stem_conv_s2d(img, conv, bn))
    if ho.X3:
        pi = PREP.get(_stem_w4(conv), (bn.weight, bn.bias, bn.running_mean, bn.running_var), ho.xw(16), bn.eps)
        H2, W2 = H // 2, W // 2
        H4, W4 = (H2 - 1) // 2 + 1, (W2 - 1) // 2 + 1
        out = torch.empty(B * H4 * W4, ho.xw(O), dtype=torch.bfloat16, device=img.device)
        src = img.detach().contiguous()
        ho.prof_flops('fwd', (B * H2 * W2, O, 2 * 49 * Cc, 49, 2), 2.0 * B * H2 * W2 * O * 49 * Cc,
                      lambda: ho.call('aod_stem_pool_x3_fwd', ho.ptr(src), ho.ptr(pi.wf), ho.ptr(pi.scale), ho.ptr(pi.shift), ho.ptr(out), B, Cc, H, W,
                                      ho.stream()))
        return as_nchw(out, B, H4, W4)
    assert O == 64 and Cc <= 4
    rows, segs = ho.nchw_to_s2d_rows(img.detach())
    pi = PREP.get(_stem_w4(conv), (bn.weight, bn.bias, bn.running_mean, bn.running_var), 16, bn.eps)
    H2, W2 = H // 2, W // 2
    H4, W4 = (H2 - 1) // 2 + 1, (W2 - 1) // 2 + 1
    out = torch.empty(B * H4 * W4, O, dtype=torch.bfloat16, device=img.device)
    flops = 2.0 * B * H2 * W2 * O * 49 * Cc
    ho.prof_flops('fwd', (B * H2 * W2, O, 49 * Cc, 49, 2), flops,
                  lambda: ho.call('aod_stem_pool_fwd', ho.ptr(rows), ho.ptr(pi.wf), ho.ptr(pi.scale), ho.ptr(pi.shift), ho.ptr(out), B, H2, W2, ho.stream()))
    return as_nchw(out, B, H4, W4)


def max_pool_3x3_s2(x):
    assert not x.requires_grad, 'maxpool backward is not implemented (stem is frozen, resnet.py:612-628)'
    B, C, H, W = x.shape
    rows, s = ho.maxpool3x3s2(as_rows(x), Seg(B, H, W))
    return as_nchw(rows, s.B, s.H, s.W)


class UpsampleAddFn(Function):

    @staticmethod
    def forward(ctx, lateral, top):
        B, C, H, W = lateral.shape
        h, w = top.shape[2:]
        out = ho.upsample_add(as_rows(lateral), Seg(B, H, W), as_rows(top), Seg(B, h, w))
        ctx.dims = (B, C, H, W, h, w)
        return as_nchw(out, B, H, W)

    @staticmethod
    def backward(ctx, g):
        B, C, H, W, h, w = ctx.dims
        g_rows = as_rows(g)
        gt = None
        if ctx.needs_input_grad[1]:
            gt = as_nchw(ho.upsample_add_bwd(g_rows, Seg(B, H, W), Seg(B, h, w)), B, h, w)
        return (g if ctx.needs_input_grad[0] else None), gt


def pyramid_buffer(shapes, channels, device, dtype=torch.bfloat16):
    rows = sum(b * h * w for b, h, w in shapes)
    flat = torch.empty(rows, ho.width(channels) if dtype == torch.bfloat16 else channels, device=device, dtype=dtype)
    views, r = [], 0
    for b, h, w in shapes:
        views.append(as_nchw(flat[r:r + b * h * w], b, h, w))
        r += b * h * w
    return flat, views


def upsample_add(lateral, top):
    return UpsampleAddFn.apply(lateral, top)


class PackedLosses(list):

    def __init__(self, items, packed, group=None):
        super().__init__(items)
        self.packed = packed
        self.group = group


class GradArena:

    def __init__(self, rows_per_level):
        self.row0, r = [], 0
        for n in rows_per_level:
            self.row0.append(r)
            r += int(n)
        self.rows, self.bufs = r, {}

    def slice(self, name, level, rows, width, device):
        buf = self.bufs.get(name)
        if buf is None:
            buf = self.bufs[name] = torch.empty(self.rows, width, dtype=torch.float32, device=device)
        assert buf.shape[1] == width and rows == (self.row0[level + 1] if level + 1 < len(self.row0) else self.rows) - self.row0[level]
        return buf[self.row0[level]:self.row0[level] + rows]


class RetinaLossFn(Function):

    @staticmethod
    def forward(ctx, cls_score, bbox_pred, labels, label_w, bbox_t, bbox_w, gamma, alpha, num_classes, arena=None, level=0, form='edl'):
        B, AC, H, W = cls_score.shape
        ctx.arena, ctx.level, ctx.form = arena, level, form
        ctx.set_materialize_grads(False)
        A = AC // num_classes
        cls_rows = as_rows(cls_score).view(-1, num_classes)
        box_rows = as_rows(bbox_pred).view(-1, 4)
        labels = labels.reshape(-1).contiguous()
        label_w = label_w.reshape(-1).contiguous()
        bbox_t = bbox_t.reshape(-1, 4).contiguous()
        bbox_w = bbox_w.reshape(-1, 4).contiguous()
        noR, sums = ho.edl_focal_l1_fwd(cls_rows, labels, label_w, box_rows, bbox_t, bbox_w, gamma, alpha, form=form)
        ctx.save_for_backward(cls_rows, box_rows, labels, label_w, bbox_t, bbox_w)
        ctx.cfg = (gamma, alpha, cls_score.shape, bbox_pred.shape)
        return sums[0], sums[1], noR, sums[2]

    @staticmethod
    def backward(ctx, g_cls, g_box, g_noR, g_sum):
        cls_rows, box_rows, labels, label_w, bbox_t, bbox_w = ctx.saved_tensors
        gamma, alpha, cshape, bshape = ctx.cfg
        dev = cls_rows.device
        g_cls = torch.zeros(1, device=dev) if g_cls is None else g_cls.reshape(1).float().contiguous()
        g_box = torch.zeros(1, device=dev) if g_box is None else g_box.reshape(1).float().contiguous()
        g_noR_t = None if g_noR is None else g_noR.float().contiguous()
        scalar = False
        if g_sum is not None:
            if g_noR_t is None:
                g_noR_t, scalar = g_sum.reshape(1).float().contiguous(), True
            else:
                g_noR_t = g_noR_t + g_sum.float()
        B, AC, H, W = cshape
        dst_c = dst_b = None
        if ctx.arena is not None:
            dst_c = ctx.arena.slice('cls', ctx.level, B * H * W, AC, dev).view(-1, cls_rows.shape[1])
            dst_b = ctx.arena.slice('box', ctx.level, B * H * W, bshape[1], dev).view(-1, 4)
        gc, gb = ho.edl_focal_l1_bwd(cls_rows, labels, label_w, box_rows, bbox_t, bbox_w, g_cls, g_box, g_noR_t, 0.0, gamma, alpha,
                                     g_noR_is_scalar=scalar, grad_cls=dst_c, grad_bbox=dst_b, form=ctx.form)
        return (as_nchw(gc.view(B * H * W, AC), B, H, W), as_nchw(gb.view(B * H * W, bshape[1]), B, H, W),
                None, None, None, None, None, None, None, None, None, None)


def dense_concat(tensors):
    t0 = tensors[0]
    tail = tuple(t0.shape[1:])
    end = t0.data_ptr()
    rows = 0
    for t in tensors:
        if t.dtype != t0.dtype or tuple(t.shape[1:]) != tail:
            return None
        if t.numel() == 0:
            continue
        if not t.is_contiguous() or t.data_ptr() != end:
            return None
        end += t.numel() * t.element_size()
        rows += t.shape[0]
    if t0.untyped_storage().data_ptr() + t0.untyped_storage().nbytes() < end:
        return None
    shape = (rows,) + tail
    stride, acc = [], 1
    for d in reversed(shape):
        stride.append(acc)
        acc *= d
    return t0.as_strided(shape, tuple(reversed(stride)))


LOSS_LEVELS = __import__('os').environ.get('AOD_LOSS_LEVELS', '1') != '0'


class RetinaLossLevelsFn(Function):

    @staticmethod
    def forward(ctx, cls_rows, box_rows, labels, label_w, bbox_t, bbox_w, gamma, alpha, level_rows, shapes, num_pos=None, form='edl'):
        ctx.set_materialize_grads(False)
        ctx.form = form
        div = nt = None
        if num_pos is None:
            noR, sums = ho.edl_focal_l1_levels_fwd(cls_rows, labels, label_w, box_rows, bbox_t, bbox_w, level_rows, gamma, alpha, form=form)
        else:
            noR, sums, div, nt = ho.edl_focal_l1_levels_fwd(cls_rows, labels, label_w, box_rows, bbox_t, bbox_w, level_rows, gamma, alpha, num_pos,
                                                            form=form)
        ctx.save_for_backward(cls_rows, box_rows, labels, label_w, bbox_t, bbox_w, div)
        ctx.cfg = (gamma, alpha, tuple(level_rows), shapes)
        if nt is None:
            return sums, noR
        nt = nt.view(())
        ctx.mark_non_differentiable(nt)
        return sums, noR, nt

    @staticmethod
    def backward(ctx, g_sums, g_noR, g_nt=None):
        cls_rows, box_rows, labels, label_w, bbox_t, bbox_w, div = ctx.saved_tensors
        gamma, alpha, level_rows, (A, AC, A4) = ctx.cfg
        dev = cls_rows.device
        L = len(level_rows)
        g_sums = torch.zeros(3, L, device=dev) if g_sums is None else g_sums.float().contiguous()
        g_rows = None
        if g_noR is not None:
            g2 = g_sums[2] if div is None else g_sums[2] / div[2]
            g_rows = (g_noR.float() + torch.repeat_interleave(g2, _level_rows_dev(level_rows, dev), output_size=sum(level_rows))).contiguous()
        gc = torch.empty(cls_rows.shape[0] // A, AC, dtype=torch.float32, device=dev)
        gb = torch.empty(cls_rows.shape[0] // A, A4, dtype=torch.float32, device=dev)
        ho.edl_focal_l1_levels_bwd(cls_rows, labels, label_w, box_rows, bbox_t, bbox_w, level_rows, g_sums, g_rows, gc, gb, A, gamma, alpha, divisors=div,
                                   form=ctx.form)
        return gc.view(cls_rows.shape), gb.view(box_rows.shape), None, None, None, None, None, None, None, None, None, None


_LEVEL_ROWS_DEV = {}


def _level_rows_dev(level_rows, dev):
    key = (tuple(level_rows), dev)
    t = _LEVEL_ROWS_DEV.get(key)
    if t is None:
        if len(_LEVEL_ROWS_DEV) > 64:
            _LEVEL_ROWS_DEV.clear()
        t = _LEVEL_ROWS_DEV[key] = torch.tensor(list(level_rows), device=dev)
    return t


class MEHLossLevelsFn(Function):

    @staticmethod
    def forward(ctx, lam, loss_noR, bbox_w, level_rows, A, form='l2'):
        out = ho.meh_loss_levels_fwd(lam, loss_noR, bbox_w, level_rows, form=form)
        ctx.save_for_backward(lam, loss_noR, bbox_w)
        ctx.cfg = (tuple(level_rows), A, form)
        return out

    @staticmethod
    def backward(ctx, g):
        lam, loss_noR, bw = ctx.saved_tensors
        level_rows, A, form = ctx.cfg
        gl = torch.empty(lam.numel() // A, A, dtype=torch.float32, device=lam.device)
        ho.meh_loss_levels_bwd(lam, loss_noR, bw, level_rows, g.float().contiguous(), gl, A, form=form)
        return gl.view(lam.shape), None, None, None, None, None


class _LevelViewsFn(Function):

    @staticmethod
    def forward(ctx, dense, *levels):
        ctx.shapes = [tuple(t.shape) for t in levels]
        return dense.view_as(dense)

    @staticmethod
    def backward(ctx, g):
        outs, r = [], 0
        for B, C, H, W in ctx.shapes:
            outs.append(as_nchw(g[r:r + B * H * W].view(B * H * W, C), B, H, W))
            r += B * H * W
        return (None,) + tuple(outs)


def dense_levels(levels):
    rows = [as_rows(t) for t in levels]
    with torch.no_grad():
        dense = dense_concat([r.detach() for r in rows])
    if dense is None:
        return None
    return _LevelViewsFn.apply(dense, *levels)


class MEHLossFn(Function):

    @staticmethod
    def forward(ctx, L_score, loss_noR, bbox_w, arena=None, level=0, form='l2'):
        ctx.arena, ctx.level, ctx.form = arena, level, form
        lam = as_rows(L_score).view(-1)
        bw = bbox_w.reshape(-1, 4).contiguous()
        loss_noR = loss_noR.contiguous()
        out = ho.meh_loss_fwd(lam, loss_noR, bw, form=form)
        ctx.save_for_backward(lam, loss_noR, bw)
        ctx.shape = L_score.shape
        return out[0]

    @staticmethod
    def backward(ctx, g):
        lam, loss_noR, bw = ctx.saved_tensors
        B, A, H, W = ctx.shape
        dst = ctx.arena.slice('lam', ctx.level, B * H * W, A, lam.device).view(-1, 1) if ctx.arena is not None else None
        gl = ho.meh_loss_bwd(lam, loss_noR, bw, g.reshape(1).float().contiguous(), grad=dst, form=ctx.form)
        return as_nchw(gl.view(B * H * W, A), B, H, W), None, None, None, None, None
```

aod_meh_hua_amd/hipops.py:

```python
import ctypes as C
import os
from dataclasses import dataclass
from typing import List, Optional, Sequence

import torch

from . import _C
from ._C import ConvDesc, ConvSeg, call, lib, ptr, stream


X3 = False
DETERMINISTIC = False


def set_deterministic(on=True):
    global DETERMINISTIC
    rc = lib.aod_set_deterministic(1 if on else 0)
    if rc < 0:
        raise RuntimeError(lib.aod_last_error().decode())
    DETERMINISTIC = bool(on)


def xw(c):
    return 2 * ((c + 31) // 32 * 32)


def width(c):
    return xw(c) if X3 else c


_ROW_TABLES = {}


PROFILE = None
SCOPE = 'head'


class scope:
    def __init__(self, name):
        self.name = name

    def __enter__(self):
        global SCOPE
        self.prev, SCOPE = SCOPE, self.name

    def __exit__(self, *exc):
        global SCOPE
        SCOPE = self.prev
        return False


def _prof(kind, desc, fn, alg=None):
    if PROFILE is None:
        return fn()
    if desc.transposed:
        m = sum(desc.seg[i].B * desc.seg[i].H * desc.seg[i].W for i in range(desc.nseg))
    else:
        m = sum(desc.seg[i].B * desc.seg[i].OH * desc.seg[i].OW for i in range(desc.nseg))
    cn = alg[0] * alg[1] if alg is not None else desc.N * desc.C
    flops = 2.0 * m * desc.R * desc.S * cn
    e0, e1 = torch.cuda.Event(enable_timing=True), torch.cuda.Event(enable_timing=True)
    e0.record()
    r = fn()
    e1.record()
    PROFILE.append((kind, (m, desc.N, desc.R * desc.S * desc.C, desc.R * desc.S, desc.stride), flops, e0, e1, SCOPE))
# ... 514 lines not shown
def bottleneck_bwd(g_rows, B, H, W, wd3, wd2, wd1, act_t2, act_t1, act_x):
    M, Cin = g_rows.shape
    if X3:
        assert M == B * H * W and Cin == 1024 and act_x.shape == g_rows.shape and act_t2.shape == (M, 256) and act_t1.shape == (M, 256)
        dev = g_rows.device
        gx = torch.empty(M, 1024, dtype=torch.bfloat16, device=dev)
        gt2 = torch.empty(M, 256, dtype=torch.bfloat16, device=dev)
        gt1 = torch.empty(M, 256, dtype=torch.bfloat16, device=dev)
        cx, c2, c1 = zeros_f32(512, dev), zeros_f32(128, dev), zeros_f32(128, dev)
        prof_flops('dgrad', (M, 512, 2 * (512 + 9 * 128 + 128), 11, 1), 2.0 * M * (512 * 128 + 9 * 128 * 128 + 128 * 512),
                   lambda: call('aod_bottleneck128x3_bwd', ptr(g_rows), B, H, W, ptr(wd3), ptr(wd2), ptr(wd1), ptr(act_t2), ptr(act_t1), ptr(act_x),
                                ptr(gx), ptr(gt2), ptr(gt1), ptr(c2), ptr(c1), ptr(cx), stream()))
        return gx, gt2, gt1, cx, c2, c1
    assert M == B * H * W and Cin in (512, 1024) and act_x.shape == g_rows.shape
    Pl = Cin // 4
    assert act_t2.shape == (M, Pl) and act_t1.shape == (M, Pl)
    dev = g_rows.device
    gx = torch.empty(M, Cin, dtype=torch.bfloat16, device=dev)
    gt2 = torch.empty(M, Pl, dtype=torch.bfloat16, device=dev)
    gt1 = torch.empty(M, Pl, dtype=torch.bfloat16, device=dev)
    cx, c2, c1 = zeros_f32(Cin, dev), zeros_f32(Pl, dev), zeros_f32(Pl, dev)
    flops = 2.0 * M * (Cin * Pl + 9 * Pl * Pl + Pl * Cin)
    prof_flops('dgrad', (M, Cin, Cin + 9 * Pl + Pl, 11, 1), flops,
               lambda: call('aod_bottleneck_bwd', Pl, ptr(g_rows), B, H, W, ptr(wd3), ptr(wd2), ptr(wd1), ptr(act_t2), ptr(act_t1), ptr(act_x),
                            ptr(gx), ptr(gt2), ptr(gt1), ptr(c2), ptr(c1), ptr(cx), stream()))
    return gx, gt2, gt1, cx, c2, c1


def rows_to_nchw(rows, seg: Seg):
    Cc = rows.shape[1]
    return rows[seg.row0:seg.row0 + seg.rows].view(seg.B, seg.H, seg.W, Cc).permute(0, 3, 1, 2)


def maxpool3x3s2(x_rows, seg: Seg):
    Cc = x_rows.shape[1]
    oh, ow = out_hw(seg.H, seg.W, 3, 3, 2, 1, 1)
    out = torch.empty(seg.B * oh * ow, Cc, dtype=torch.bfloat16, device=x_rows.device)
    call('aod_x3_maxpool3x3s2' if X3 else 'aod_maxpool3x3s2', ptr(x_rows), ptr(out), seg.B, seg.H, seg.W, Cc, stream())
    return out, Seg(seg.B, oh, ow, 0)


def upsample_add_(dst_rows, dst_seg: Seg, src_rows, src_seg: Seg):
    call('aod_upsample2x_add', ptr(src_rows), ptr(dst_rows), dst_seg.B, src_seg.H, src_seg.W, dst_rows.shape[1],
         dst_seg.H, dst_seg.W, stream())
    return dst_rows


def upsample_add(lat_rows, dst_seg: Seg, top_rows, src_seg: Seg):
    out = torch.empty_like(lat_rows)
    call('aod_x3_upsample2x_add_to' if X3 else 'aod_upsample2x_add_to', ptr(top_rows), ptr(lat_rows), ptr(out), dst_seg.B, src_seg.H, src_seg.W, lat_rows.shape[1], dst_seg.H, dst_seg.W, stream())
    return out


def upsample_add_bwd(g_dst_rows, dst_seg: Seg, src_seg: Seg):
    out = torch.empty(src_seg.rows, g_dst_rows.shape[1], dtype=torch.bfloat16, device=g_dst_rows.device)
    call('aod_x3_upsample2x_add_bwd_set' if X3 else 'aod_upsample2x_add_bwd_set', ptr(g_dst_rows), ptr(out), dst_seg.B, src_seg.H, src_seg.W, g_dst_rows.shape[1], dst_seg.H, dst_seg.W, stream())
    return out


def upsample_add_bwd_(g_src_rows, src_seg: Seg, g_dst_rows, dst_seg: Seg):
    call('aod_upsample2x_add_bwd', ptr(g_dst_rows), ptr(g_src_rows), dst_seg.B, src_seg.H, src_seg.W,
         g_dst_rows.shape[1], dst_seg.H, dst_seg.W, stream())
    return g_src_rows


def add_relu(a, b):
    out = torch.empty_like(a)
    call('aod_add_relu', ptr(a), ptr(b), ptr(out), a.numel(), stream())
    return out


def act_bwd(g, a=None, z=None, scale=None, mean=None, invstd=None, relu=True, want_gm=False, want_dz=True):
    M, N = g.shape
    if X3:
        assert z is None and scale is None and not want_gm and g.dtype == torch.bfloat16
        dz = torch.empty(M, N, dtype=torch.bfloat16, device=g.device) if want_dz else None
        dbeta = zeros_f32(N // 2, g.device)
        call('aod_x3_act_bwd', ptr(g), ptr(a), ptr(dz), ptr(dbeta), M, N, int(relu), stream())
        return dz, None, dbeta, None
    dz = torch.empty(M, N, dtype=torch.bfloat16, device=g.device) if want_dz else None
    gm = torch.empty(M, N, dtype=torch.bfloat16, device=g.device) if want_gm else None
    dbeta = zeros_f32(N, g.device)
    dgamma = zeros_f32(N, g.device) if z is not None else None
    call('aod_act_bwd', ptr(g), ptr(a), ptr(z), ptr(scale), ptr(mean), ptr(invstd), ptr(dz), ptr(gm), ptr(dbeta),
         ptr(dgamma), M, N, int(relu), int(g.dtype == torch.float32), stream())
    return dz, gm, dbeta, dgamma


FOCAL_FORMS = {'edl': 'aod_edl_focal', 'sigmoid': 'aod_sigmoid_focal'}


def edl_focal_l1_fwd(cls, labels, label_w, bbox_pred=None, bbox_tgt=None, bbox_w=None, gamma=2.0, alpha=0.25, sums=None, form='edl'):
    rows, Cc = cls.shape
    loss_noR = torch.empty(rows, dtype=torch.float32, device=cls.device)
    if sums is None:
        sums = zeros_f32(3, cls.device)
    part = torch.empty(max(int(_C.lib.aod_loss_partials_len(rows)), 1), dtype=torch.float32, device=cls.device)
    prof_bytes(form + '_l1_fwd', rows * (Cc * 4 + 8 + 4 + (48 if bbox_pred is not None else 0) + 4),
               lambda: call(FOCAL_FORMS[form] + '_l1_fwd', ptr(cls), ptr(labels), ptr(label_w), ptr(bbox_pred), ptr(bbox_tgt), ptr(bbox_w), rows, Cc,
                            gamma, alpha, ptr(loss_noR), ptr(sums), ptr(part), stream()))
    return loss_noR, sums


def edl_focal_l1_bwd(cls, labels, label_w, bbox_pred, bbox_tgt, bbox_w, g_cls, g_bbox, g_noR=None, g_noR_scalar=0.0,
                     gamma=2.0, alpha=0.25, g_noR_is_scalar=False, out_bf16=False, A=1, pitch_cls=None, pitch_box=None, grad_cls=None, grad_bbox=None,
                     form='edl'):
    rows, Cc = cls.shape
    pitch_cls = pitch_cls or A * Cc
    pitch_box = pitch_box or A * 4
# ... 46 lines not shown
    rows, Cc = cls.shape
    L = len(level_rows)
    assert sum(level_rows) == rows
    lr = _level_rows(level_rows)
    loss_noR = torch.empty(rows, dtype=torch.float32, device=cls.device)
    sums = torch.empty(3, L, dtype=torch.float32, device=cls.device)
    div = nt = None
    if num_pos is not None:
        assert num_pos.dtype == torch.int32 and num_pos.is_contiguous()
        div = torch.empty(3, L, dtype=torch.float32, device=cls.device)
        nt = torch.empty(1, dtype=torch.float32, device=cls.device)
    part = torch.empty(max(int(_C.lib.aod_loss_levels_partials_len(L, lr)), 1), dtype=torch.float32, device=cls.device)
    prof_bytes(form + '_l1_fwd', rows * (Cc * 4 + 8 + 4 + (48 if bbox_pred is not None else 0) + 4),
               lambda: call(FOCAL_FORMS[form] + '_l1_levels_fwd', ptr(cls), ptr(labels), ptr(label_w), ptr(bbox_pred), ptr(bbox_tgt), ptr(bbox_w), L, lr, Cc,
                            gamma, alpha, ptr(loss_noR), ptr(sums), ptr(part), ptr(num_pos), 0 if num_pos is None else int(num_pos.numel()), ptr(div),
                            ptr(nt), stream()))
    return (loss_noR, sums) if num_pos is None else (loss_noR, sums, div, nt)


def edl_focal_l1_levels_bwd(cls, labels, label_w, bbox_pred, bbox_tgt, bbox_w, level_rows, g_sums, g_noR_rows, grad_cls, grad_bbox, A,
                            gamma=2.0, alpha=0.25, divisors=None, form='edl'):
    rows, Cc = cls.shape
    L = len(level_rows)
    lr = _level_rows(level_rows)
    assert g_sums.shape == (3, L) and g_sums.is_contiguous() and g_sums.dtype == torch.float32
    prof_bytes(form + '_l1_bwd', rows * (Cc * 4 + 8 + 4 + (4 if g_noR_rows is not None else 0) + Cc * 4 + ((48 + 16) if bbox_pred is not None else 0)),
               lambda: call(FOCAL_FORMS[form] + '_l1_levels_bwd', ptr(cls), ptr(labels), ptr(label_w), ptr(bbox_pred), ptr(bbox_tgt), ptr(bbox_w), L, lr, Cc,
                            gamma, alpha, ptr(g_sums), ptr(divisors), ptr(g_noR_rows), ptr(grad_cls), ptr(grad_bbox), 0, A, A * Cc, A * 4, stream()))
    return grad_cls, grad_bbox


def meh_loss_levels_fwd(lam, loss_noR, bbox_w4, level_rows, form='l2'):
    L = len(level_rows)
    assert sum(level_rows) == lam.numel()
    lr = _level_rows(level_rows)
    out = torch.empty(L, dtype=torch.float32, device=lam.device)
    part = torch.empty(max(int(_C.lib.aod_loss_levels_partials_len(L, lr)), 1), dtype=torch.float32, device=lam.device)
    if form != 'l2':
        call('aod_meh_loss_levels_fwd_ex', ptr(lam), ptr(loss_noR), ptr(bbox_w4), L, lr, MEH_FORMS[form], ptr(out), ptr(part), stream())
        return out
    call('aod_meh_loss_levels_fwd', ptr(lam), ptr(loss_noR), ptr(bbox_w4), L, lr, ptr(out), ptr(part), stream())
    return out


def meh_loss_levels_bwd(lam, loss_noR, bbox_w4, level_rows, g, grad, A, form='l2'):
    L = len(level_rows)
    lr = _level_rows(level_rows)
    assert g.shape == (L,) and g.is_contiguous() and g.dtype == torch.float32
    if form != 'l2':
        call('aod_meh_loss_levels_bwd_ex', ptr(lam), ptr(loss_noR), ptr(bbox_w4), L, lr, MEH_FORMS[form], ptr(g), ptr(grad), 0, A, A, stream())
        return grad
    call('aod_meh_loss_levels_bwd', ptr(lam), ptr(loss_noR), ptr(bbox_w4), L, lr, ptr(g), ptr(grad), 0, A, A, stream())
    return grad


def pad_cast_colsum(g, npad, relu_out=None, want_map=False):
    M, N = g.shape
    assert relu_out is None or relu_out.dtype == torch.float32
    if X3:
        assert g.dtype == torch.float32 and npad == xw(N)
        dz = torch.empty(M, npad, dtype=torch.bfloat16, device=g.device)
        cs = zeros_f32(npad // 2, g.device)
        if want_map:
            rmap = row_map(M, g.device)
            call('aod_x3_pad_cast_colsum_map', ptr(g), ptr(relu_out), ptr(dz), ptr(cs), M, N, ptr(rmap), stream())
            return dz, cs, rmap
        call('aod_x3_pad_cast_colsum', ptr(g), ptr(relu_out), ptr(dz), ptr(cs), M, N, stream())
        return dz, cs
    assert not want_map, 'row-activity maps exist in the reference-precision mode only'
    dz = torch.empty(M, npad, dtype=torch.bfloat16, device=g.device)
    cs = zeros_f32(npad, g.device)
    call('aod_pad_cast_colsum', ptr(g), ptr(relu_out), ptr(dz), ptr(cs), M, N, npad, int(g.dtype == torch.float32), stream())
    return dz, cs


_F4 = C.c_float * 4


def max_iou_assign(anchors, valid, gts, gt_count, gt_labels, pos_thr=0.5, neg_thr=0.4, min_pos_iou=0.0, assign_all=True,
                   num_classes=20, means=(0., 0., 0., 0.), stds=(1., 1., 1., 1.), level_start=None):
    A = anchors.shape[0]
    B, Gmax = gts.shape[:2]
    dev = anchors.device
    assigned = torch.empty(B, A, dtype=torch.int64, device=dev)
    labels = torch.empty(B, A, dtype=torch.int64, device=dev)
    label_w = torch.empty(B, A, dtype=torch.float32, device=dev)
    bbox_t = torch.empty(B, A, 4, dtype=torch.float32, device=dev)
    bbox_w = torch.empty(B, A, 4, dtype=torch.float32, device=dev)
    num_pos = torch.empty(B, dtype=torch.int32, device=dev)
    ws = torch.empty(max(int(_C.lib.aod_assign_ws_bytes(B, Gmax)), 8), dtype=torch.uint8, device=dev)
    if valid is not None:
        valid = valid.view(torch.uint8) if valid.dtype == torch.bool else valid
    call('aod_max_iou_assign', ptr(anchors), ptr(valid), A, B, ptr(gts), ptr(gt_count), ptr(gt_labels), Gmax, pos_thr, neg_thr,
         min_pos_iou, int(assign_all), num_classes, _F4(*means), _F4(*stds), ptr(assigned), ptr(labels), ptr(label_w), ptr(bbox_t),
         ptr(bbox_w), ptr(num_pos), ptr(ws), 0 if level_start is None else len(level_start) - 1,
         None if level_start is None else (C.c_int64 * len(level_start))(*level_start), stream())
    return assigned, labels, label_w, bbox_t, bbox_w, num_pos


def x3_split(t_f32):
    M, Cc = t_f32.shape
    out = torch.empty(M, xw(Cc), dtype=torch.bfloat16, device=t_f32.device)
    call('aod_x3_split', ptr(t_f32.contiguous()), ptr(out), M, Cc, stream())
    return out


def x3_merge(x_rows, Cc=None):
    M, Wd = x_rows.shape
    Cc = Cc or Wd // 2
    out = torch.empty(M, Cc, dtype=torch.float32, device=x_rows.device)
    call('aod_x3_merge', ptr(x_rows.contiguous()), ptr(out), M, Cc, stream())
    return out


def x3_add(a, b):
    out = torch.empty_like(a)
    call('aod_x3_add', ptr(a), ptr(b), ptr(out), a.numel(), stream())
    return out


def dropout2d_masks(table, image_ids, site_offsets, rate, seed, sample):
    B, T = int(image_ids.numel()), int(table.shape[1])
    if not (table.dtype == torch.float32 and table.dim() == 2 and table.is_contiguous() and table.shape[0] >= B):
        raise ValueError(f'dropout2d_masks: the table must be a contiguous fp32 [>= {B}, T] tensor, got {tuple(table.shape)} {table.dtype}')
    if not (image_ids.dtype == torch.int64 and image_ids.is_contiguous() and site_offsets.dtype == torch.int32 and site_offsets.is_contiguous()):
        raise ValueError('dropout2d_masks: image_ids must be contiguous int64 and site_offsets contiguous int32')
    call('aod_dropout2d_masks', ptr(table), ptr(image_ids), B, ptr(site_offsets), int(site_offsets.numel()), T, float(rate),
         int(seed) & 0xFFFFFFFFFFFFFFFF, int(sample), stream())
    return table


def dropout2d_apply(x_rows, table, col0, B, HW, Cc):
    if not (x_rows.dtype == torch.bfloat16 and x_rows.is_contiguous() and tuple(x_rows.shape) == (B * HW, width(Cc))):
        raise ValueError(f'dropout2d_apply: rows {tuple(x_rows.shape)} {x_rows.dtype} are not the contiguous bf16 [{B * HW}, {width(Cc)}] rows of {Cc} channels')
    if not (table.dtype == torch.float32 and table.dim() == 2 and table.stride(1) == 1 and table.shape[0] >= B and 0 <= col0 and col0 + Cc <= table.shape[1]):
        raise ValueError(f'dropout2d_apply: table {tuple(table.shape)} does not hold columns {col0}..{col0 + Cc} of {B} images')
    call('aod_dropout2d_apply', ptr(x_rows), C.c_void_p(table.data_ptr() + 4 * col0), table.stride(0), B, HW, Cc, 1 if X3 else 0, stream())
    return x_rows


def dropout2d_apply_multi(base_rows, table, B, segs, Cc):
    n = len(segs)
    if not (base_rows.dtype == torch.bfloat16 and base_rows.is_contiguous() and base_rows.shape[1] == width(Cc)):
        raise ValueError(f'dropout2d_apply_multi: rows {tuple(base_rows.shape)} {base_rows.dtype} are not contiguous bf16 rows of {Cc} channels')
    if not (table.dtype == torch.float32 and table.dim() == 2 and table.stride(1) == 1 and table.shape[0] >= B
            and all(0 <= off and off + Cc <= table.shape[1] for _, _, off in segs)):
        raise ValueError(f'dropout2d_apply_multi: table {tuple(table.shape)} does not hold the segments\' columns for {B} images')
    call('aod_dropout2d_apply_multi', ptr(base_rows), ptr(table), table.stride(0), B, n, (C.c_int64 * n)(*[s[0] for s in segs]),
         (C.c_int32 * n)(*[s[1] for s in segs]), (C.c_int32 * n)(*[s[2] for s in segs]), Cc, 1 if X3 else 0, stream())
    return base_rows


IMAGE_XFORM_ITEM_BYTES = 80


def image_xform(src_pack, items, B, Hp, Wp, out):
    if not (src_pack.dtype == torch.uint8 and items.dtype == torch.uint8 and items.numel() >= B * IMAGE_XFORM_ITEM_BYTES):
        raise ValueError('image_xform: src_pack / items must be uint8 byte buffers holding B item records')
    if not (tuple(out.shape) == (B, 3, Hp, Wp) and out.dtype == torch.float32 and out.is_contiguous()):
        raise ValueError(f'image_xform: out must be a contiguous float32 [{B}, 3, {Hp}, {Wp}] tensor, got {out.dtype} {tuple(out.shape)}')
    call('aod_image_xform', ptr(src_pack), ptr(items), B, Hp, Wp, ptr(out), stream())
    return out


def pixel_noise(src, dst, hw, inv_std, sigma, level, seed, image_ids):
    for name, t in (('src', src), ('dst', dst)):
        if not (torch.is_tensor(t) and t.dtype == torch.float32 and t.dim() == 4 and t.is_contiguous()):
            raise ValueError(f'pixel_noise: {name} must be a contiguous fp32 [B, C, Hp, Wp] tensor')
    if tuple(dst.shape) != tuple(src.shape):
        raise ValueError(f'pixel_noise: dst has shape {tuple(dst.shape)}, src {tuple(src.shape)}')
    B, Cc, Hp, Wp = (int(v) for v in src.shape)
# ... 24 lines not shown
```

aod_meh_hua_amd/models/dense_heads/Lambda_L2.py:

```python
import numpy as np
import torch
import torch.nn as nn

from ... import functional as AF
from ...core.utils import multi_apply
from ...mmcv_lite import Conv2d, ConvModule, force_fp32
from ..builder import HEADS
from .L_anchor_head import L_AnchorHead


@HEADS.register_module()
class Lambda_L2Net(L_AnchorHead):
    def __init__(self, num_classes, in_channels, stacked_convs=4, conv_cfg=None, norm_cfg=None,
                 anchor_generator=dict(type='AnchorGenerator', octave_base_scale=4, scales_per_octave=3, ratios=[0.5, 1.0, 2.0],
                                       strides=[8, 16, 32, 64, 128]),
                 init_cfg=dict(type='Normal', layer='Conv2d', std=0.01,
                               override=dict(type='Normal', name='retina_cls', std=0.01, bias_prob=0.01)), **kwargs):
        self.stacked_convs, self.conv_cfg, self.norm_cfg = stacked_convs, conv_cfg, norm_cfg
        self.isTrainD = False
        super().__init__(num_classes, in_channels, anchor_generator=anchor_generator, init_cfg=init_cfg, **kwargs)
        self.L_names = ['retina_L', 'L_convs']

    def _init_layers(self):
        self.relu = nn.ReLU(inplace=True)
        self.cls_convs, self.reg_convs, self.L_convs = nn.ModuleList(), nn.ModuleList(), nn.ModuleList()
        for i in range(self.stacked_convs):
            chn = self.in_channels if i == 0 else self.feat_channels
            for tower in (self.cls_convs, self.reg_convs, self.L_convs):
                tower.append(ConvModule(chn, self.feat_channels, 3, stride=1, padding=1, conv_cfg=self.conv_cfg, norm_cfg=self.norm_cfg))
        self.retina_cls = Conv2d(self.feat_channels, self.num_anchors * self.cls_out_channels, 3, padding=1)
        self.retina_reg = Conv2d(self.feat_channels, self.num_anchors * 4, 3, padding=1)
        self.retina_L = Conv2d(self.feat_channels, self.num_anchors, 3, padding=1)

    def forward_train(self, x, img_metas, gt_bboxes, gt_labels=None, gt_bboxes_ignore=None, proposal_cfg=None, **kwargs):
        prepare = getattr(self, '_sparse_fwd_prepare', None)
        targets, fwd_maps = prepare(x, img_metas, gt_bboxes, gt_labels, **kwargs) if prepare is not None else (None, None)
        outs = self.forward(x, **kwargs) if fwd_maps is None else self.forward(x, fwd_maps=fwd_maps, **kwargs)
        loss_inputs = outs + (None, gt_bboxes, gt_labels, img_metas)
        if targets is not None:
            kwargs = dict(kwargs, targets=targets)
        return self.loss(*loss_inputs, gt_bboxes_ignore=gt_bboxes_ignore, **kwargs)

    def _sparse_fwd_prepare(self, x, img_metas, gt_bboxes, gt_labels, **kwargs):
        from ... import hipops as ho
        x = list(x)
        n = len(self.reg_convs)
        ok = (ho.sparse_fwd() and torch.is_grad_enabled() and self.training and kwargs.get('Labeled', True) and not kwargs.get('Pseudo', False)
              and type(self.loss_bbox).__name__ == 'L1Loss' and self._meh_form in ('l2', 'l1', 'msle') and self._rides(x)
              and 1 <= n == len(self.cls_convs) <= 7 and all(m.with_activation for m in list(self.cls_convs) + list(self.reg_convs))
              and all(m.conv.weight.shape[2:] == (3, 3) and m.conv.padding == (1, 1) and m.conv.dilation == (1, 1) and m.conv.stride == (1, 1)
                      for m in list(self.reg_convs) + list(self.L_convs))
              and self.retina_reg.weight.shape[2:] == (3, 3) and self.retina_L.weight.shape[2:] == (3, 3))
        if not ok:
            return None, None
        featmap_sizes = [tuple(f.shape[-2:]) for f in x]
        targets = self.get_targets_batch(featmap_sizes, img_metas, gt_bboxes, gt_labels, x[0].device, raw_num_pos=True)
        bw = AF.dense_concat([t.reshape(-1, 4) for t in targets[3]])
        if bw is None or bw.dtype != torch.float32:
            return targets, None
        B = x[0].shape[0]
        segs = AF.dense_segs([ho.Seg(B, h, w, 0) for h, w in featmap_sizes])
        c = self.feat_channels
        return targets, ho.fwd_row_maps(bw, segs, self.num_anchors, ho.width(c), c, 3, 3, 1, 1, n + 1)

    def _rides(self, feats):
        import os
        return (torch.is_grad_enabled() and self.training and os.environ.get('AOD_MEH_RIDER', '1') != '0'
                and len(self.L_convs) == len(self.cls_convs) and all(m.with_activation for m in self.L_convs)
                and feats[0].dtype == torch.bfloat16)

    def forward_train_L(self, prev_loss, head_out, x, **kwargs):
        L_scores = self.forward_L(x, head_out, **kwargs)
        return self.loss_L(L_scores, head_out, prev_loss, **kwargs)

    def forward(self, feats, fwd_maps=None, **kwargs):
        feats = list(feats)
        cls_feat, reg_feat = (list(t) for t in zip(*[AF.fork(f, 2) for f in feats]))
        if len(self.cls_convs) == len(self.reg_convs) and all(m.with_activation for m in list(self.cls_convs) + list(self.reg_convs)):
            ride = self._rides(feats)
            nl = len(self.cls_convs)
            self._L_pre = None
            L_rows, L_outs = (AF.multi_rows([f.detach() for f in feats])[0] if ride else None), []
            for i, (cc, rc) in enumerate(zip(self.cls_convs, self.reg_convs)):
                if L_rows is not None:
                    cls_feat, reg_feat, L_rows = AF.conv_pair_act(cls_feat, reg_feat, cc.conv, rc.conv, sole_consumer=i > 0,
                                                                  rider=(self.L_convs[i].conv, L_rows),
                                                                  fwd_map=fwd_maps[nl - i] if fwd_maps is not None else None)
                    L_outs.append(L_rows)
                else:
                    cls_feat, reg_feat = AF.conv_pair_act(cls_feat, reg_feat, cc.conv, rc.conv, sole_consumer=i > 0)
            if ride and len(L_outs) == len(self.L_convs) and all(o is not None for o in L_outs):
                self._L_pre = (feats[0].data_ptr(), tuple(feats[0].shape), [m.conv.weight._version for m in self.L_convs], L_outs)
        else:
            for i, conv in enumerate(self.cls_convs):
                cls_feat = conv(cls_feat, sole_consumer=i > 0)
            for i, conv in enumerate(self.reg_convs):
                reg_feat = conv(reg_feat, sole_consumer=i > 0)
        return (self.retina_cls(cls_feat, out_f32=True, sole_consumer=len(self.cls_convs) > 0),
                self.retina_reg(reg_feat, out_f32=True, sole_consumer=len(self.reg_convs) > 0, sparse_grad=True))

    def forward_cls_dropout(self, feats):
        assert AF.mc_dropout_active() and not torch.is_grad_enabled()
        cls_feat = list(feats)
        for i, conv in enumerate(self.cls_convs):
            cls_feat = conv(cls_feat)
            if conv.with_activation:
                AF.dropout_apply(cls_feat, [f'.cls_convs.{i}@{l}' for l in range(len(cls_feat))], self)
        return self.retina_cls(cls_feat, out_f32=True)

    def forward_L(self, feats, head_out=None, **kwargs):
        L_feat = list(feats)
        pre, self._L_pre = getattr(self, '_L_pre', None), None
        if pre is not None and not (torch.is_grad_enabled() and pre[0] == L_feat[0].data_ptr() and pre[1] == tuple(L_feat[0].shape)
                                    and pre[2] == [m.conv.weight._version for m in self.L_convs]):
            pre = None
        for i, conv in enumerate(self.L_convs):
            L_feat = conv(L_feat, sole_consumer=i > 0, pre=pre[3][i] if pre is not None else None)
        return self.retina_L(L_feat, relu=True, out_f32=True, sole_consumer=len(self.L_convs) > 0, sparse_grad=True)

    def forward_single(self, x):
        c, r = self.forward([x])
        return c[0], r[0]

    def forward_single_L(self, x):
        return self.forward_L([x])[0], 0

    _can_defer_avg = True
    _meh_form = 'l2'
    _hua_lam = 'scaled'
    _hua_thr_kwargs = False
    _hua_entropy_avg = False
    _focal_form = 'edl'
    _loss_cls_type = 'EDL_Softmax_FocalLoss'

    @force_fp32(apply_to=('cls_score', 'bbox_pred'))
    def loss_single(self, cls_score, bbox_pred, anchors, labels, label_weights, bbox_targets, bbox_weights, sIdx, num_total_samples, **kwargs):
        if not (kwargs.get('Labeled', True) and not kwargs.get('Pseudo', False)):
            raise NotImplementedError('pseudo-label branch (Lambda_L2.py:122-232) is dead code in the reference driver')
        assert type(self.loss_bbox).__name__ == 'L1Loss' and type(self.loss_cls).__name__ == self._loss_cls_type
        sum_cls, sum_box, loss_noR, sum_noR = AF.RetinaLossFn.apply(cls_score, bbox_pred, labels, label_weights, bbox_targets, bbox_weights,
                                                                    float(self.loss_cls.gamma), float(self.loss_cls.alpha), self.cls_out_channels,
                                                                    kwargs.get('grad_arena'), int(sIdx), self._focal_form)
        wc, wb = self.loss_cls.loss_weight, self.loss_bbox.loss_weight
        scaled = lambda w, t: t if w == 1.0 else w * t
        if kwargs.get('defer_avg'):
            return scaled(wc, sum_cls), scaled(wb, sum_box), scaled(wc, loss_noR), scaled(wc, sum_noR)
        loss_cls = scaled(wc, sum_cls) / num_total_samples
        loss_bbox = scaled(wb, sum_box) / num_total_samples
        return loss_cls, loss_bbox, scaled(wc, loss_noR)

    def loss_all_levels(self, cls_scores, bbox_preds, labels_list, lw_list, bt_list, bw_list, num_pos=None, **kwargs):
        if not (kwargs.get('Labeled', True) and not kwargs.get('Pseudo', False)):
            raise NotImplementedError('pseudo-label branch (Lambda_L2.py:122-232) is dead code in the reference driver')
        if self.loss_cls.loss_weight != 1.0 or self.loss_bbox.loss_weight != 1.0:
            return None
        assert type(self.loss_bbox).__name__ == 'L1Loss' and type(self.loss_cls).__name__ == self._loss_cls_type
        C = self.cls_out_channels
        cls_d, box_d = AF.dense_levels(cls_scores), AF.dense_levels(bbox_preds)
        flat = [AF.dense_concat([t.reshape(-1, *t.shape[2:]) for t in ts]) for ts in (labels_list, lw_list, bt_list, bw_list)]
        if cls_d is None or box_d is None or any(f is None for f in flat) or cls_d.dtype != torch.float32 or box_d.dtype != torch.float32:
            return None
        A = cls_d.shape[1] // C
        level_rows = [c.shape[0] * c.shape[2] * c.shape[3] * A for c in cls_scores]
        out = AF.RetinaLossLevelsFn.apply(cls_d.view(-1, C), box_d.view(-1, 4), flat[0], flat[1], flat[2], flat[3],
                                          float(self.loss_cls.gamma), float(self.loss_cls.alpha), level_rows,
                                          (A, cls_d.shape[1], box_d.shape[1]), num_pos, self._focal_form)
        return (out[0], list(out[1].split(level_rows))) + tuple(out[2:])

    def loss_all_levels_L(self, L_scores, losses, bw_list, **kwargs):
        lam_d = AF.dense_levels(L_scores)
        noR = AF.dense_concat([t.reshape(-1) for t in losses])
        bw = AF.dense_concat([t.reshape(-1, 4) for t in bw_list])
        if lam_d is None or noR is None or bw is None or lam_d.dtype != torch.float32 or noR.dtype != torch.float32 or noR.requires_grad:
            return None
        A = lam_d.shape[1]
        level_rows = [l.shape[0] * l.shape[2] * l.shape[3] * A for l in L_scores]
        if [int(t.numel()) for t in losses] != level_rows:
            return None
        return AF.MEHLossLevelsFn.apply(lam_d.view(-1), noR, bw, level_rows, A, self._meh_form)

    @force_fp32(apply_to=('L_score'))
    def loss_single_L(self, L_score, loss, label_weights, bbox_weights, sIdx=0, **kwargs):
        s = AF.MEHLossFn.apply(L_score, loss, bbox_weights, kwargs.get('grad_arena'), int(sIdx), self._meh_form)
        if kwargs.get('defer_scale'):
            return s, 5.0 / loss.numel()
        return s * (5.0 / loss.numel()), 0

    def forward_all_towers(self, feats):
        feats = list(feats)
        c, r, l = feats, feats, feats
        for cc, rc, lc in zip(self.cls_convs, self.reg_convs, self.L_convs):
            c, r, l = AF.conv_towers_nograd([c, r, l], [cc.conv, rc.conv, lc.conv], relu=True)
        outs = (self.retina_cls(c, out_f32=True), self.retina_reg(r, out_f32=True))
        return outs, self.retina_L(l, relu=True, out_f32=True)

    def test_heads(self, feats, with_L=True):
        import os
        if not with_L:
            return self.forward(feats), None
        x3_ok = AF.get_precision() == 'bf16' or all(m.conv.weight.shape[0] % 256 == 0 and m.conv.weight.shape[1] % 32 == 0 for m in self.cls_convs)
        if (not torch.is_grad_enabled() and x3_ok and os.environ.get('AOD_GROUP_TOWERS', '1') != '0'
                and len(self.cls_convs) == len(self.reg_convs) == len(self.L_convs) > 0 and all(m.with_activation for m in self.cls_convs)):
            return self.forward_all_towers(feats)
        outs = self.forward(feats)
        return outs, self.forward_L(feats, head_out=None)

    def simple_test(self, feats, img_metas, rescale=False, _preds=None, **kwargs):
        from ...scoring import POSTERIOR_POOLS
        if not kwargs['isEval'] and kwargs.get('isUnc') and kwargs.get('uPool') in POSTERIOR_POOLS:
            outs = _preds[0] if _preds is not None else self.test_heads(feats, with_L=False)[0]
            results_list = self.get_bboxes(*outs, img_metas, rescale=rescale, with_nms=True, **kwargs)
            return (results_list[0], *results_list[1:])
        outs, L_scores = _preds if _preds is not None else self.test_heads(feats)
        if not kwargs['isEval'] and kwargs['uPool'] == 'Entropy_NoNMS':
            results_list = self.get_bboxes(*outs, img_metas, rescale=rescale, with_nms=False, **kwargs)
        elif not kwargs['isEval'] and kwargs['uPool'] == 'Entropy_Avg':
            results_list = self.get_bboxes(*outs, img_metas, rescale=rescale, with_nms=False, L_scores=L_scores, **kwargs)
        elif not kwargs['isEval'] and kwargs['uPool'] == 'Entropy_ALL':
            results_list = self.get_bboxes(*outs, img_metas, rescale=rescale, with_nms=bool(kwargs.get('showNMS')), L_scores=L_scores, **kwargs)
        elif not kwargs['isEval'] and kwargs['uPool'] == 'Entropy_NMS':
            results_list = self.get_bboxes(*outs, img_metas, rescale=rescale, with_nms=True, L_scores=L_scores, **kwargs)
        elif kwargs['isEval'] and kwargs.get('detUnc'):
            results_list = self.get_bboxes(*outs, img_metas, rescale=rescale, L_scores=L_scores, **kwargs)
        else:
            results_list = self.get_bboxes(*outs, img_metas, rescale=rescale, **kwargs)
        if not kwargs['isEval']:
            if kwargs.get('scaleUnc'):
                return results_list
            return (results_list[0], *results_list[1:])
        return results_list

    @force_fp32(apply_to=('mlvl_cls_scores', 'mlvl_bbox_preds', 'mlvl_anchors'))
# ... 5 lines not shown
```

aod_meh_hua_amd/models/dense_heads/MyRetinaHead.py:

```python
import torch
import torch.nn as nn

from ... import functional as AF
from ...mmcv_lite import Conv2d, ConvModule
from ..builder import HEADS
from .L_anchor_head import L_AnchorHead
from .Lambda_L2 import Lambda_L2Net


@HEADS.register_module()
class MyRetinaHead(L_AnchorHead):
    def __init__(self, num_classes, in_channels, stacked_convs=4, conv_cfg=None, norm_cfg=None,
                 anchor_generator=dict(type='AnchorGenerator', octave_base_scale=4, scales_per_octave=3, ratios=[0.5, 1.0, 2.0],
                                       strides=[8, 16, 32, 64, 128]),
                 init_cfg=dict(type='Normal', layer='Conv2d', std=0.01,
                               override=dict(type='Normal', name='retina_cls', std=0.01, bias_prob=0.01)), **kwargs):
        self.stacked_convs, self.conv_cfg, self.norm_cfg = stacked_convs, conv_cfg, norm_cfg
        super().__init__(num_classes, in_channels, anchor_generator=anchor_generator, init_cfg=init_cfg, **kwargs)
        if self.last_activation != 'sigmoid' or type(self.loss_cls).__name__ != 'FocalLoss' or type(self.loss_bbox).__name__ != 'L1Loss':
            raise ValueError("MyRetinaHead is built for loss_cls=FocalLoss(last_activation='sigmoid') + loss_bbox=L1Loss "
                             f'(got {type(self.loss_cls).__name__}/{self.last_activation} + {type(self.loss_bbox).__name__})')

    def _init_layers(self):
        self.relu = nn.ReLU(inplace=True)
        self.cls_convs, self.reg_convs = nn.ModuleList(), nn.ModuleList()
        for i in range(self.stacked_convs):
            chn = self.in_channels if i == 0 else self.feat_channels
            for tower in (self.cls_convs, self.reg_convs):
                tower.append(ConvModule(chn, self.feat_channels, 3, stride=1, padding=1, conv_cfg=self.conv_cfg, norm_cfg=self.norm_cfg))
        self.retina_cls = Conv2d(self.feat_channels, self.num_anchors * self.cls_out_channels, 3, padding=1)
        self.retina_reg = Conv2d(self.feat_channels, self.num_anchors * 4, 3, padding=1)

    forward_train = Lambda_L2Net.forward_train

    def forward_train_L(self, *args, **kwargs):
        raise ValueError('MyRetinaHead has no lambda (no Model Evidence Head): there is no MEH step to train')

    def forward(self, feats, **kwargs):
        feats = list(feats)
        cls_feat, reg_feat = (list(t) for t in zip(*[AF.fork(f, 2) for f in feats]))
        if all(m.with_activation for m in list(self.cls_convs) + list(self.reg_convs)):
            for i, (cc, rc) in enumerate(zip(self.cls_convs, self.reg_convs)):
                cls_feat, reg_feat = AF.conv_pair_act(cls_feat, reg_feat, cc.conv, rc.conv, sole_consumer=i > 0)
        else:
            for i, conv in enumerate(self.cls_convs):
                cls_feat = conv(cls_feat, sole_consumer=i > 0)
            for i, conv in enumerate(self.reg_convs):
                reg_feat = conv(reg_feat, sole_consumer=i > 0)
        return (self.retina_cls(cls_feat, out_f32=True, sole_consumer=len(self.cls_convs) > 0),
                self.retina_reg(reg_feat, out_f32=True, sole_consumer=len(self.reg_convs) > 0, sparse_grad=True))

    forward_single = Lambda_L2Net.forward_single

    def forward_cls_dropout(self, feats):
        assert AF.mc_dropout_active() and not torch.is_grad_enabled()
        cls_feat = list(feats)
        for i, conv in enumerate(self.cls_convs):
            cls_feat = conv(cls_feat)
            if conv.with_activation:
                AF.dropout_apply(cls_feat, [f'.cls_convs.{i}@{l}' for l in range(len(cls_feat))], self)
        return self.retina_cls(cls_feat, out_f32=True)

    _can_defer_avg = True
    _focal_form = 'sigmoid'
    _loss_cls_type = 'FocalLoss'
    loss_single = Lambda_L2Net.loss_single
    loss_all_levels = Lambda_L2Net.loss_all_levels

    def loss_L(self, *args, **kwargs):
        raise ValueError('MyRetinaHead has no lambda (no Model Evidence Head): there is no MEH loss')

    def test_heads(self, feats):
        import os
        x3_ok = AF.get_precision() == 'bf16' or all(m.conv.weight.shape[0] % 256 == 0 and m.conv.weight.shape[1] % 32 == 0 for m in self.cls_convs)
        if (not torch.is_grad_enabled() and x3_ok and os.environ.get('AOD_GROUP_TOWERS', '1') != '0'
                and len(self.cls_convs) == len(self.reg_convs) > 0 and all(m.with_activation for m in list(self.cls_convs) + list(self.reg_convs))):
            c = r = list(feats)
            for cc, rc in zip(self.cls_convs, self.reg_convs):
                c, r = AF.conv_towers_nograd([c, r], [cc.conv, rc.conv], relu=True)
            return (self.retina_cls(c, out_f32=True), self.retina_reg(r, out_f32=True)), None
        return self.forward(feats), None

    def simple_test(self, feats, img_metas, rescale=False, _preds=None, **kwargs):
        from ...scoring import refuse_hua
        refuse_hua(self, **kwargs)
        outs, _ = _preds if _preds is not None else self.test_heads(feats)
        with_nms = not (not kwargs['isEval'] and kwargs.get('uPool') == 'Entropy_NoNMS')
        results_list = self.get_bboxes(*outs, img_metas, rescale=rescale, with_nms=with_nms, **kwargs)
        if not kwargs['isEval']:
            from ...scoring import POSTERIOR_POOLS
            if kwargs.get('isUnc') and kwargs.get('uPool') in POSTERIOR_POOLS:
                return (results_list[0], *results_list[1:])
            return (results_list,)
# ... 4 lines not shown
```

include/aod_hip.h:

```cpp
#ifndef AOD_HIP_H
#define AOD_HIP_H
#include <stddef.h>
#include <stdint.h>

#ifdef __cplusplus
extern "C" {
#endif

typedef void* aod_stream_t;

const char* aod_last_error(void);
int aod_version(void);

typedef struct {
  int32_t B, H, W;
  int32_t OH, OW;
  int64_t src_row0;
  int64_t dst_row0;
} aod_conv_seg_t;

typedef struct {
  int32_t C, N;
  int32_t R, S;
  int32_t stride, pad, dil;
// ... 275 lines not shown
  int32_t to_rgb;
  float pad_val;
  float mean[3], std[3];
  int32_t reserved;
} aod_image_xform_item_t;
int aod_image_xform(const void* src_pack, const aod_image_xform_item_t* items_dev, int B, int Hp, int Wp, float* dst, aod_stream_t stream);

int aod_sgd_multi(void* const* params, void* const* grads, void* const* moms, const int64_t* sizes, int ntensors,
                  float lr, const float* lr_dev, float momentum, float weight_decay, int first_step, float grad_scale,
                  aod_stream_t stream);
int aod_sgd_multi_clipped(void* const* params, void* const* grads, void* const* moms, const int64_t* sizes, int ntensors,
                          float lr, const float* lr_dev, float momentum, float weight_decay, int first_step, float grad_scale,
                          const float* coef_dev, aod_stream_t stream);
int aod_grad_norm_multi(void* const* grads, const int64_t* sizes, int ntensors, float grad_scale, float max_norm, int flags,
                        float* partials_ws, int64_t ws_capacity, float* state, aod_stream_t stream);

size_t aod_ensemble_mi_partials_len(int L, const int64_t* n_per_level, int B);
int aod_ensemble_mi(const void* const* maps, int K, int L, const int64_t* n_per_level, int B, int n_cls, float* out, float* partials_ws,
                    int64_t ws_capacity, aod_stream_t stream);

int aod_dropout2d_masks(float* table, const int64_t* image_ids, int B, const int32_t* site_offsets, int n_sites, int T, float rate,
                        uint64_t seed, uint32_t sample, aod_stream_t stream);
int aod_dropout2d_apply(void* x, const float* table_row0, int64_t row_stride_T, int B, int HW, int C, int x3, aod_stream_t stream);
int aod_dropout2d_apply_multi(void* x, const float* table, int64_t row_stride_T, int B, int nseg, const int64_t* seg_row0,
                              const int32_t* seg_hw, const int32_t* seg_off, int C, int x3, aod_stream_t stream);

int aod_pool_descriptor(const void* base, int nseg, const int64_t* seg_row0, const int32_t* seg_hw, int C, int x3, int B, float* out,
                        int64_t out_stride, aod_stream_t stream);
int aod_kcenter_chunk(void);
size_t aod_kcenter_ws_len(int64_t N);
int aod_kcenter_greedy(const float* desc, int64_t N, int D, const int64_t* labelled, int64_t n_labelled, int64_t budget, int64_t* picks,
                       float* radius, float* mind, void* ws, aod_stream_t stream);

int aod_cdal_chunk(void);
size_t aod_cdal_ws_len(int L, const int64_t* rows_per_level, int C, int B);
int aod_cdal_descriptor(const void* const* maps, int L, const int64_t* rows_per_level, int C, int B, float score_thr, float* out,
                        int64_t out_stride, float* ws, int64_t ws_capacity, aod_stream_t stream);
int aod_kcenter_greedy_ex(const float* desc, int64_t N, int D, const int64_t* labelled, int64_t n_labelled, int64_t budget, int64_t* picks,
                          float* radius, float* mind, void* ws, aod_stream_t stream, int metric);

int aod_det_uncertainty(const float* boxes, const float* scores, const float* dets, const int64_t* labels, const int32_t* num, int B, int n,
                        int W, int max_num, int layout, int measure, int aggregate, float score_thr, float* unc, float* obj_out,
                        int32_t* missing, aod_stream_t stream);

int aod_loc_stability_max_levels(void);
int aod_pixel_noise(const float* src, float* dst, int B, int C, int Hp, int Wp, const int32_t* hw, const float* inv_std, float sigma, int level,
                    uint64_t seed, const int64_t* image_ids, aod_stream_t stream);
int aod_loc_stability(const float* dets, const int64_t* labels, const int32_t* num, int K, int B, int max_num, float score_thr, int same_class,
                      int combine, float* unc, float* stab_out, aod_stream_t stream);

int aod_x3_split(const float* src, void* dst, int64_t M, int C, aod_stream_t stream);
int aod_x3_merge(const void* src, float* dst, int64_t M, int C, aod_stream_t stream);
int aod_x3_add(const void* a, const void* b, void* out, int64_t n, aod_stream_t stream);
int aod_x3_nchw_f32_to_s2d(const float* src, void* dst, int B, int C, int H, int W, aod_stream_t stream);
int aod_x3_maxpool3x3s2(const void* src, void* dst, int B, int H, int W, int C, aod_stream_t stream);
int aod_x3_upsample2x_add_to(const void* top, const void* lateral, void* out, int B, int h, int w, int C, int H, int W, aod_stream_t stream);
int aod_x3_upsample2x_add_bwd_set(const void* g_dst, void* g_src, int B, int h, int w, int C, int H, int W, aod_stream_t stream);
int aod_x3_act_bwd(const void* g, const void* a, void* dz, float* colsum, int64_t M, int C, int relu, aod_stream_t stream);
int aod_x3_pad_cast_colsum(const float* g, const float* relu_out_f32, void* dz, float* colsum, int64_t M, int N, aod_stream_t stream);
int aod_x3_pad_cast_colsum_map(const float* g, const float* relu_out_f32, void* dz, float* colsum, int64_t M, int N, void* map,
                               aod_stream_t stream);

int aod_bottleneck64x3_fwd(const void* x, int Cin, int B, int H, int W, const void* w1, const float* s1, const float* b1, const void* w2,
                           const float* s2, const float* b2, const void* w3, const float* s3, const float* b3, const void* res, void* y,
                           aod_stream_t stream);

int aod_bottleneck64x3_ds_fwd(const void* x, int B, int H, int W, const void* w1, const float* s1, const float* b1, const void* w2,
                              const float* s2, const float* b2, const void* w3, const float* s3, const float* b3, const void* wd,
                              const float* sd, const float* bd, void* y, aod_stream_t stream);

int aod_bottleneck128x3_fwd(const void* x, int B, int H, int W, const void* w1, const float* s1, const float* b1, const void* w2,
                            const float* s2, const float* b2, const void* w3, const float* s3, const float* b3, void* y, void* t1, void* t2,
                            aod_stream_t stream);

int aod_bottleneck128x3_bwd(const void* g, int B, int H, int W, const void* wd3, const void* wd2, const void* wd1, const void* act_t2,
                            const void* act_t1, const void* act_x, void* gx, void* gt2, void* gt1, float* colsum_t2, float* colsum_t1,
                            float* colsum_x, aod_stream_t stream);

int aod_halo_conv3x3_x3_applies(const aod_conv_desc_t* desc);
int aod_halo_conv3x3_x3(const aod_conv_desc_t* desc, const void* src, const void* w_packed, void* dst, const float* pre_shift,
                        aod_stream_t stream);

int aod_mfma_clock_probe(int iters, int workgroups, void* out_u64_pairs, float* sink, aod_stream_t stream);

int aod_stem_pool_x3_fwd(const float* img, const void* w_x, const float* scale, const float* shift, void* y, int B, int C, int H, int W,
                         aod_stream_t stream);

int aod_x3_nchw_f32_to_nhwc(const float* src, void* dst, int B, int C, int H, int W, aod_stream_t stream);
int aod_x3_maxpool_fwd(const void* x, void* y, int B, int H, int W, int C, int OH, int OW, int k, int s, int p, aod_stream_t stream);
int aod_x3_maxpool_bwd(const void* x, const void* g, void* gx, int B, int H, int W, int C, int OH, int OW, int k, int s, int p, aod_stream_t stream);
int aod_x3_l2norm_fwd(const void* x, const float* w, void* y, int64_t rows, int C, float eps, aod_stream_t stream);
int aod_x3_l2norm_bwd(const void* x, const float* w, const void* g, void* gx, float* gw, int64_t rows, int C, float eps, aod_stream_t stream);

#ifdef __cplusplus
}
#endif
#endif
```

Before: 757.8.

## Fuse loss-gradient generation into X3 pad-cast-colsum and batch head junction adds

Adds source functors so the MEH and box-loss backward gradients are computed directly inside the pad-cast-colsum kernel that writes bf16x3 dz and column sums, which removes the intermediate fp32 gradient tensors and a separate kernel pass. It also adds a multi-range x3 add kernel that sums several level pairs in one launch, and an upsample-backward variant that accumulates into an existing gradient. The heads now use fork_levels and head_junction hooks so per-level work is batched. The cost is more complex templated kernels and extra per-element level lookups inside the fused kernel.

```diff
diff --git a/aod_meh_hua_amd/_C.py b/aod_meh_hua_amd/_C.py
--- a/aod_meh_hua_amd/_C.py
+++ b/aod_meh_hua_amd/_C.py
@@ -152,6 +152,10 @@
     'aod_x3_split': (C.c_int, [P, P, I64, I32, P]),
     'aod_x3_merge': (C.c_int, [P, P, I64, I32, P]),
     'aod_x3_add': (C.c_int, [P, P, P, I64, P]),
+    'aod_x3_add_multi': (C.c_int, [I32, P, P, P, P, P]),
+    'aod_x3_upsample2x_add_bwd_acc': (C.c_int, [P, P, P, I32, I32, I32, I32, I32, I32, P]),
+    'aod_meh_loss_levels_bwd_x': (C.c_int, [P, P, P, I32, P, I32, P, I32, P, P, I32, P, P]),
+    'aod_x3_box_levels_bwd_x': (C.c_int, [P, P, P, I32, P, P, P, P, P, I32, P, P]),
     'aod_x3_nchw_f32_to_s2d': (C.c_int, [P, P, I32, I32, I32, I32, P]),
     'aod_x3_maxpool3x3s2': (C.c_int, [P, P, I32, I32, I32, I32, P]),
     'aod_x3_upsample2x_add_to': (C.c_int, [P, P, P, I32, I32, I32, I32, I32, I32, P]),
diff --git a/aod_meh_hua_amd/build.py b/aod_meh_hua_amd/build.py
--- a/aod_meh_hua_amd/build.py
+++ b/aod_meh_hua_amd/build.py
@@ -15,7 +15,7 @@
 def source_digest():
     import hashlib
     h = hashlib.sha256()
-    for f in sources() + [os.path.join(CSRC, 'common.h'), os.path.join(CSRC, 'pointwise.h'), os.path.join(CSRC, 'conv_x3p.h'), os.path.join(CSRC, 'conv_params.h'), os.path.join(HERE, '..', 'include', 'aod_hip.h')]:
+    for f in sources() + [os.path.join(CSRC, 'common.h'), os.path.join(CSRC, 'pointwise.h'), os.path.join(CSRC, 'conv_x3p.h'), os.path.join(CSRC, 'conv_params.h'), os.path.join(CSRC, 'loss_terms.h'), os.path.join(HERE, '..', 'include', 'aod_hip.h')]:
         if os.path.exists(f):
             h.update(os.path.basename(f).encode())
             h.update(open(f, 'rb').read())
@@ -26,7 +26,7 @@
     if not os.path.exists(LIB):
         return True
     t = os.path.getmtime(LIB)
-    deps = sources() + [os.path.join(CSRC, 'common.h'), os.path.join(CSRC, 'pointwise.h'), os.path.join(CSRC, 'conv_x3p.h'), os.path.join(CSRC, 'conv_params.h'),
+    deps = sources() + [os.path.join(CSRC, 'common.h'), os.path.join(CSRC, 'pointwise.h'), os.path.join(CSRC, 'conv_x3p.h'), os.path.join(CSRC, 'conv_params.h'), os.path.join(CSRC, 'loss_terms.h'),
                         os.path.join(HERE, '..', 'include', 'aod_hip.h')]
     return any(os.path.getmtime(d) > t for d in deps)
 
diff --git a/aod_meh_hua_amd/csrc/loss_terms.h b/aod_meh_hua_amd/csrc/loss_terms.h
--- /dev/null
+++ b/aod_meh_hua_amd/csrc/loss_terms.h
@@ -0,0 +1,50 @@
+#pragma once
+#include "common.h"
+
+constexpr int MAXLV = 8;
+struct LossLevels { int n; int blk_end[MAXLV]; long long row_end[MAXLV]; };
+__device__ __forceinline__ void level_of_block(const LossLevels& lv, int bid, int& level, int& blk0, long long& row0, long long& rend) {
+  level = 0; blk0 = 0; row0 = 0; rend = lv.row_end[0];
+#pragma unroll
+  for (int q = 0; q + 1 < MAXLV; ++q)
+    if (bid >= lv.blk_end[q]) { level = q + 1; blk0 = lv.blk_end[q]; row0 = lv.row_end[q]; rend = lv.row_end[q + 1]; }
+}
+__device__ __forceinline__ int level_of_row(const LossLevels& lv, long long r) {
+  int level = 0;
+#pragma unroll
+  for (int q = 0; q + 1 < MAXLV; ++q)
+    if (q + 1 < lv.n && r >= lv.row_end[q]) level = q + 1;
+  return level;
+}
+static inline int fill_levels(LossLevels& lv, int nlevels, const int64_t* level_rows, int rows_per_block, long long& total_rows) {
+  lv.n = nlevels;
+  long long r = 0, b = 0;
+  for (int l = 0; l < MAXLV; ++l) {
+    if (l < nlevels) { r += level_rows[l]; b += (level_rows[l] + rows_per_block - 1) / rows_per_block; }
+    lv.row_end[l] = r;
+    lv.blk_end[l] = l < nlevels ? (int)b : 0x7fffffff;
+  }
+  total_rows = r;
+  return (int)b;
+}
+
+__device__ __forceinline__ float sign0(float x) { return x > 0.f ? 1.f : (x < 0.f ? -1.f : 0.f); }
+
+template <int FORM>
+__device__ __forceinline__ float meh_grad_term(float lam, float loss, float w, float g) {
+  if (FORM == 1) {
+    const float d = lam + 1e-9f - loss;
+    return g * sign0(fabsf(d) * w) * w * sign0(d);
+  } else if (FORM == 2) {
+    const float x = lam + 1e-9f + 1.f;
+    const float d = logf(x) - logf(loss + 1.f);
+    return g * 2.f * (fabsf(d) * w) * w * sign0(d) / x;
+  }
+  return g * 2.f * w * w * (lam + 1e-9f - loss);
+}
+
+__device__ __forceinline__ float box_grad_term(float p, float t, float w, float gb) {
+  const float d = p - t;
+  const float sgn = d > 0.f ? 1.f : (d < 0.f ? -1.f : 0.f);
+  return sgn * w * gb;
+}
diff --git a/aod_meh_hua_amd/csrc/losses.hip b/aod_meh_hua_amd/csrc/losses.hip
--- a/aod_meh_hua_amd/csrc/losses.hip
+++ b/aod_meh_hua_amd/csrc/losses.hip
@@ -1,4 +1,5 @@
 #include "common.h"
+#include "loss_terms.h"
 
 #define FLT_MIN_F 1.17549435e-38f
 constexpr int LB = 256;
@@ -77,26 +78,6 @@
 #pragma unroll
   for (int c = 0; c < CT; ++c) if (c < n) tot += sig_focal_term(x[c], label == c0 + c, gamma, alpha, nullptr);
   return grp_sum<LPR>(tot);
-}
-
-constexpr int MAXLV = 8;
-struct LossLevels { int n; int blk_end[MAXLV]; long long row_end[MAXLV]; };
-__device__ __forceinline__ void level_of_block(const LossLevels& lv, int bid, int& level, int& blk0, long long& row0, long long& rend) {
-  level = 0; blk0 = 0; row0 = 0; rend = lv.row_end[0];
-#pragma unroll
-  for (int q = 0; q + 1 < MAXLV; ++q)
-    if (bid >= lv.blk_end[q]) { level = q + 1; blk0 = lv.blk_end[q]; row0 = lv.row_end[q]; rend = lv.row_end[q + 1]; }
-}
-static int fill_levels(LossLevels& lv, int nlevels, const int64_t* level_rows, int rows_per_block, long long& total_rows) {
-  lv.n = nlevels;
-  long long r = 0, b = 0;
-  for (int l = 0; l < MAXLV; ++l) {
-    if (l < nlevels) { r += level_rows[l]; b += (level_rows[l] + rows_per_block - 1) / rows_per_block; }
-    lv.row_end[l] = r;
-    lv.blk_end[l] = l < nlevels ? (int)b : 0x7fffffff;
-  }
-  total_rows = r;
-  return (int)b;
 }
 
 template <int FORM, int CT, int LPR>
@@ -365,9 +346,7 @@
       const float gb = g_div ? g_bbox[gl] / g_div[nlv + gl] : g_bbox[gl];
       const long long bb = (r / A) * pitch_box + (r % A) * 4;
       for (int j = 0; j < 4; ++j) {
-        const float d = bp[r * 4 + j] - bt[r * 4 + j];
-        const float sgn = d > 0.f ? 1.f : (d < 0.f ? -1.f : 0.f);
-        const float gx = sgn * bw[r * 4 + j] * gb;
+        const float gx = box_grad_term(bp[r * 4 + j], bt[r * 4 + j], bw[r * 4 + j], gb);
         if (OUT_BF16) ((bf16_t*)grad_bbox)[bb + j] = (bf16_t)gx;
         else ((float*)grad_bbox)[bb + j] = gx;
       }
@@ -471,7 +450,6 @@
                              alpha, g_sums, divisors, g_noR_rows, grad_cls, grad_bbox, out_bf16, A, pitch_cls, pitch_box, stream);
 }
 
-__device__ __forceinline__ float sign0(float x) { return x > 0.f ? 1.f : (x < 0.f ? -1.f : 0.f); }
 template <int FORM>
 __global__ __launch_bounds__(256) void meh_fwd_kernel(const float* __restrict__ lam, const float* __restrict__ loss, const float* __restrict__ bw4,
                                                       const LossLevels lv, float* __restrict__ partials) {
@@ -503,18 +481,7 @@
   level_of_block(lv, (int)blockIdx.x, level, blk0, row0, n);
   const long long i = row0 + (long long)((int)blockIdx.x - blk0) * 256 + threadIdx.x;
   if (i < n) {
-    const float w = bw4[i * 4];
-    float v;
-    if (FORM == 1) {
-      const float d = lam[i] + 1e-9f - loss[i];
-      v = g[level * g_lstride] * sign0(fabsf(d) * w) * w * sign0(d);
-    } else if (FORM == 2) {
-      const float x = lam[i] + 1e-9f + 1.f;
-      const float d = logf(x) - logf(loss[i] + 1.f);
-      v = g[level * g_lstride] * 2.f * (fabsf(d) * w) * w * sign0(d) / x;
-    } else {
-      v = g[level * g_lstride] * 2.f * w * w * (lam[i] + 1e-9f - loss[i]);
-    }
+    const float v = meh_grad_term<FORM>(lam[i], loss[i], bw4[i * 4], g[level * g_lstride]);
     const long long o = (i / A) * pitch + (i % A);
     if (OUT_BF16) ((bf16_t*)grad)[o] = (bf16_t)v; else ((float*)grad)[o] = v;
   }
diff --git a/aod_meh_hua_amd/csrc/x3_ops.hip b/aod_meh_hua_amd/csrc/x3_ops.hip
--- a/aod_meh_hua_amd/csrc/x3_ops.hip
+++ b/aod_meh_hua_amd/csrc/x3_ops.hip
@@ -1,4 +1,5 @@
 #include "common.h"
+#include "loss_terms.h"
 
 static inline int grid_for(long long nvec) {
   long long b = (nvec + 255) / 256;
@@ -72,6 +73,46 @@
   AOD_CHECK_ARG(a && b && out && n % 64 == 0, "x3_add: n (bf16 elements) must be a multiple of 64");
   if (n == 0) return 0;
   hipLaunchKernelGGL(x3_add_kernel, dim3(grid_for(n / 16)), dim3(256), 0, (hipStream_t)stream, (const bf16_t*)a, (const bf16_t*)b, (bf16_t*)out, (long long)(n / 16));
+  AOD_LAUNCH_CHECK();
+  return 0;
+}
+
+constexpr int X3_ADD_MAXR = 8;
+struct X3AddRanges { int n; int blk_end[X3_ADD_MAXR]; const bf16_t* a[X3_ADD_MAXR]; const bf16_t* b[X3_ADD_MAXR]; bf16_t* o[X3_ADD_MAXR]; long long nq[X3_ADD_MAXR]; };
+__global__ void x3_add_multi_kernel(const X3AddRanges rg) {
+  int blk0 = 0, blk1 = rg.blk_end[0];
+  const bf16_t* a = rg.a[0]; const bf16_t* b = rg.b[0]; bf16_t* o = rg.o[0];
+  long long nq = rg.nq[0];
+#pragma unroll
+  for (int k = 0; k + 1 < X3_ADD_MAXR; ++k)
+    if ((int)blockIdx.x >= rg.blk_end[k]) { blk0 = rg.blk_end[k]; blk1 = rg.blk_end[k + 1]; a = rg.a[k + 1]; b = rg.b[k + 1]; o = rg.o[k + 1]; nq = rg.nq[k + 1]; }
+  const long long stride = (long long)(blk1 - blk0) * blockDim.x;
+  for (long long i = ((long long)blockIdx.x - blk0) * blockDim.x + threadIdx.x; i < nq; i += stride) {
+    const long long off = (i >> 2) * 64 + ((i & 3) << 3);
+    float x[8], y[8];
+    xload(a + off, x); xload(b + off, y);
+#pragma unroll
+    for (int j = 0; j < 8; ++j) x[j] += y[j];
+    xstore(o + off, x);
+  }
+}
+extern "C" int aod_x3_add_multi(int nranges, const void* const* a, const void* const* b, void* const* out, const int64_t* n, aod_stream_t stream) {
+  AOD_CHECK_ARG(nranges >= 1 && nranges <= X3_ADD_MAXR && a && b && out && n, "x3_add_multi: 1..8 ranges");
+  X3AddRanges rg;
+  long long blocks = 0;
+  for (int k = 0; k < X3_ADD_MAXR; ++k) {
+    const bool on = k < nranges;
+    if (on) {
+      AOD_CHECK_ARG(n[k] >= 0 && n[k] % 64 == 0 && (n[k] == 0 || (a[k] && b[k] && out[k])), "x3_add_multi: range %d: n (bf16 elements) must be a multiple of 64", k);
+      if (n[k] > 0) blocks += grid_for(n[k] / 16);
+    }
+    rg.a[k] = on ? (const bf16_t*)a[k] : nullptr; rg.b[k] = on ? (const bf16_t*)b[k] : nullptr; rg.o[k] = on ? (bf16_t*)out[k] : nullptr;
+    rg.nq[k] = on ? (long long)(n[k] / 16) : 0;
+    rg.blk_end[k] = on ? (int)blocks : 0x7fffffff;
+  }
+  rg.n = nranges;
+  if (blocks == 0) return 0;
+  hipLaunchKernelGGL(x3_add_multi_kernel, dim3((unsigned)blocks), dim3(256), 0, (hipStream_t)stream, rg);
   AOD_LAUNCH_CHECK();
   return 0;
 }
@@ -167,7 +208,8 @@
   AOD_LAUNCH_CHECK();
   return 0;
 }
-__global__ void x3_upsample_add_bwd_kernel(const bf16_t* __restrict__ gd, bf16_t* __restrict__ gs, int B, int h, int w, int Q, int H, int W) {
+__global__ void x3_upsample_add_bwd_kernel(const bf16_t* __restrict__ gd, const bf16_t* __restrict__ acc, bf16_t* __restrict__ gs, int B, int h, int w,
+                                           int Q, int H, int W) {
   const long long n = (long long)B * h * w * Q;
   const int CP = (Q >> 2) * 64;
   for (long long i = blockIdx.x * (long long)blockDim.x + threadIdx.x; i < n; i += (long long)gridDim.x * blockDim.x) {
@@ -187,13 +229,30 @@
 #pragma unroll
         for (int j = 0; j < 8; ++j) a[j] += v[j];
       }
+    if (acc) {
+      float x[8];
+      xload(acc + pix * CP + xoct(q), x);
+#pragma unroll
+      for (int j = 0; j < 8; ++j) {
+        const bf16_t hh = (bf16_t)a[j];
+        const bf16_t ll = (bf16_t)(a[j] - (float)hh);
+        a[j] = x[j] + ((float)hh + (float)ll);
+      }
+    }
     xstore(gs + pix * CP + xoct(q), a);
   }
+}
+extern "C" int aod_x3_upsample2x_add_bwd_acc(const void* g_dst, const void* acc, void* g_src, int B, int h, int w, int C, int H, int W, aod_stream_t stream) {
+  AOD_CHECK_ARG(g_dst && acc && g_src && C % 64 == 0, "x3_upsample_add_bwd_acc: the X-layout width must be a multiple of 64");
+  hipLaunchKernelGGL(x3_upsample_add_bwd_kernel, dim3(grid_for((long long)B * h * w * (C / 16))), dim3(256), 0, (hipStream_t)stream, (const bf16_t*)g_dst,
+                     (const bf16_t*)acc, (bf16_t*)g_src, B, h, w, C / 16, H, W);
+  AOD_LAUNCH_CHECK();
+  return 0;
 }
 extern "C" int aod_x3_upsample2x_add_bwd_set(const void* g_dst, void* g_src, int B, int h, int w, int C, int H, int W, aod_stream_t stream) {
   AOD_CHECK_ARG(g_dst && g_src && C % 64 == 0, "x3_upsample_add_bwd_set: the X-layout width must be a multiple of 64");
   hipLaunchKernelGGL(x3_upsample_add_bwd_kernel, dim3(grid_for((long long)B * h * w * (C / 16))), dim3(256), 0, (hipStream_t)stream, (const bf16_t*)g_dst,
-                     (bf16_t*)g_src, B, h, w, C / 16, H, W);
+                     (const bf16_t*)nullptr, (bf16_t*)g_src, B, h, w, C / 16, H, W);
   AOD_LAUNCH_CHECK();
   return 0;
 }
@@ -254,7 +313,48 @@
   return 0;
 }
 
-__global__ __launch_bounds__(256) void x3_pad_cast_colsum_kernel(const float* __restrict__ g, const float* __restrict__ a, bf16_t* __restrict__ dz,
+struct SrcRows {
+  const float* g;
+  __device__ __forceinline__ float at(long long m, int c, int N) const { return g[m * N + c]; }
+  __device__ __forceinline__ f32x4 at4(long long m, int c, int N) const { return *reinterpret_cast<const f32x4*>(g + m * N + c); }
+};
+template <int FORM>
+struct SrcMeh {
+  const float* lam; const float* loss; const float* bw4; const float* g; LossLevels lv;
+  __device__ __forceinline__ float at(long long m, int c, int N) const {
+    const long long i = m * N + c;
+    return meh_grad_term<FORM>(lam[i], loss[i], bw4[i * 4], g[level_of_row(lv, i)]);
+  }
+  __device__ __forceinline__ f32x4 at4(long long m, int c, int N) const {
+    f32x4 v;
+#pragma unroll
+    for (int j = 0; j < 4; ++j) v[j] = at(m, c + j, N);
+    return v;
+  }
+};
+struct SrcBox {
+  const float* bp; const float* bt; const float* bw; const float* g_bbox; const float* g_div; int nlv; LossLevels lv;
+  __device__ __forceinline__ float gb_of(long long e) const {
+    const int gl = level_of_row(lv, e >> 2);
+    return g_div ? g_bbox[gl] / g_div[nlv + gl] : g_bbox[gl];
+  }
+  __device__ __forceinline__ float at(long long m, int c, int N) const {
+    const long long e = m * N + c;
+    return box_grad_term(bp[e], bt[e], bw[e], gb_of(e));
+  }
+  __device__ __forceinline__ f32x4 at4(long long m, int c, int N) const {
+    const long long e = m * N + c;
+    const f32x4 p = *reinterpret_cast<const f32x4*>(bp + e), t = *reinterpret_cast<const f32x4*>(bt + e), w = *reinterpret_cast<const f32x4*>(bw + e);
+    const float gb = gb_of(e);
+    f32x4 v;
+#pragma unroll
+    for (int j = 0; j < 4; ++j) v[j] = box_grad_term(p[j], t[j], w[j], gb);
+    return v;
+  }
+};
+
+template <class SRC>
+__global__ __launch_bounds__(256) void x3_pad_cast_colsum_kernel(const SRC g, const float* __restrict__ a, bf16_t* __restrict__ dz,
                                                                  float* __restrict__ colsum, long long M, int N, int Np, int rows_per_block, int TC,
                                                                  float* __restrict__ cs_ws, unsigned char* __restrict__ map) {
   __shared__ float red[256];
@@ -269,7 +369,7 @@
       for (long long m = r0 + rl; m < r1; m += RP) {
         float v = 0.f;
         if (c < N) {
-          v = g[m * N + c];
+          v = g.at(m, c, N);
           if (a && !(a[m * N + c] > 0.f)) v = 0.f;
           if (map && !(v == 0.f)) map[m >> 6] = 1;
         }
@@ -290,7 +390,8 @@
     }
   }
 }
-__global__ __launch_bounds__(256) void x3_pad_cast_colsum_v8_kernel(const float* __restrict__ g, const float* __restrict__ a, bf16_t* __restrict__ dz,
+template <class SRC>
+__global__ __launch_bounds__(256) void x3_pad_cast_colsum_v8_kernel(const SRC g, const float* __restrict__ a, bf16_t* __restrict__ dz,
                                                                     float* __restrict__ colsum, long long M, int N, int Np, int rows_per_block, int TC8,
                                                                     float* __restrict__ cs_ws, unsigned char* __restrict__ map) {
   __shared__ float red[256][9];
@@ -304,8 +405,8 @@
     const bool lo = c + 4 <= N, hi = c + 8 <= N;
     for (long long m = r0 + rl; m < r1; m += RP) {
       f32x4 v0 = {0.f, 0.f, 0.f, 0.f}, v1 = {0.f, 0.f, 0.f, 0.f};
-      if (lo) v0 = *reinterpret_cast<const f32x4*>(g + m * N + c);
-      if (hi) v1 = *reinterpret_cast<const f32x4*>(g + m * N + c + 4);
+      if (lo) v0 = g.at4(m, c, N);
+      if (hi) v1 = g.at4(m, c + 4, N);
       if (a) {
         if (lo) { const f32x4 a0 = *reinterpret_cast<const f32x4*>(a + m * N + c);
 #pragma unroll
@@ -340,21 +441,22 @@
   }
 }
 
-extern "C" int aod_x3_pad_cast_colsum_map(const float* g, const float* relu_out_f32, void* dz, float* colsum, int64_t M, int N, void* map_,
-                                          aod_stream_t stream) {
+template <class SRC>
+static int pad_cast_colsum_launch(const SRC& src, bool g_al16, const float* relu_out_f32, void* dz, float* colsum, int64_t M, int N, void* map_,
+                                  aod_stream_t stream) {
   if (M == 0) return 0;
   unsigned char* const map = (unsigned char*)map_;
-  AOD_CHECK_ARG(g && dz && colsum && N >= 1, "x3_pad_cast_colsum: bad args");
+  AOD_CHECK_ARG(dz && colsum && N >= 1, "x3_pad_cast_colsum: bad args");
   if (map && hipMemsetAsync(map, 0, (size_t)((M + 63) / 64), (hipStream_t)stream) != hipSuccess) return aod_set_err(-3, "x3_pad_cast_colsum: memset of the map failed");
   const int Np = (N + 31) / 32 * 32;
-  if ((N & 3) == 0 && Np <= 256 && (((size_t)g | (size_t)(relu_out_f32 ? relu_out_f32 : g)) & 15) == 0) {
+  if ((N & 3) == 0 && Np <= 256 && g_al16 && ((size_t)relu_out_f32 & 15) == 0) {
     int tc8 = 4;
     while (tc8 * 8 < Np) tc8 <<= 1;
     int rpb = (int)((M + 1023) / 1024);
     if (rpb < 64) rpb = 64;
     const int nb = (int)((M + rpb - 1) / rpb);
     float* const cs_ws = aod_det_scratch((size_t)nb * N);
-    hipLaunchKernelGGL(x3_pad_cast_colsum_v8_kernel, dim3(nb), dim3(256), 0, (hipStream_t)stream, g, relu_out_f32, (bf16_t*)dz, colsum, (long long)M, N, Np,
+    hipLaunchKernelGGL(x3_pad_cast_colsum_v8_kernel<SRC>, dim3(nb), dim3(256), 0, (hipStream_t)stream, src, relu_out_f32, (bf16_t*)dz, colsum, (long long)M, N, Np,
                        rpb, tc8, cs_ws, map);
     AOD_LAUNCH_CHECK();
     if (cs_ws) return aod_colsum_finalize(cs_ws, nb, N, N, colsum, nullptr, 0, (hipStream_t)stream);
@@ -366,11 +468,43 @@
   while (tc < Np && tc < 256) tc <<= 1;
   const int nb = (int)((M + rpb - 1) / rpb);
   float* const cs_ws = aod_det_scratch((size_t)nb * N);
-  hipLaunchKernelGGL(x3_pad_cast_colsum_kernel, dim3(nb), dim3(256), 0, (hipStream_t)stream, g, relu_out_f32, (bf16_t*)dz, colsum,
+  hipLaunchKernelGGL(x3_pad_cast_colsum_kernel<SRC>, dim3(nb), dim3(256), 0, (hipStream_t)stream, src, relu_out_f32, (bf16_t*)dz, colsum,
                      (long long)M, N, Np, rpb, tc, cs_ws, map);
   AOD_LAUNCH_CHECK();
   if (cs_ws) return aod_colsum_finalize(cs_ws, nb, N, N, colsum, nullptr, 0, (hipStream_t)stream);
   return 0;
+}
+extern "C" int aod_x3_pad_cast_colsum_map(const float* g, const float* relu_out_f32, void* dz, float* colsum, int64_t M, int N, void* map_,
+                                          aod_stream_t stream) {
+  if (M == 0) return 0;
+  AOD_CHECK_ARG(g, "x3_pad_cast_colsum: bad args");
+  return pad_cast_colsum_launch(SrcRows{g}, ((size_t)g & 15) == 0, relu_out_f32, dz, colsum, M, N, map_, stream);
+}
+
+extern "C" int aod_meh_loss_levels_bwd_x(const float* lam, const float* loss_noR, const float* bbox_w4, int nlevels, const int64_t* level_rows, int form,
+                                       const float* g, int relu, void* dz, float* colsum, int A, void* map, aod_stream_t stream) {
+  AOD_CHECK_ARG(nlevels >= 1 && nlevels <= MAXLV && level_rows, "meh_levels_bwd_x: 1..8 levels");
+  AOD_CHECK_ARG(lam && loss_noR && bbox_w4 && g && A >= 1, "meh_levels_bwd_x: bad args");
+  AOD_CHECK_ARG(form >= 0 && form <= 2, "meh_levels_bwd_x: form must be 0 (L2), 1 (L1) or 2 (MSLE)");
+  LossLevels lv; long long tot = 0;
+  for (int l = 0; l < nlevels; ++l) AOD_CHECK_ARG(level_rows[l] >= 0 && level_rows[l] % A == 0, "meh_levels_bwd_x: a level's rows must be whole pixels");
+  fill_levels(lv, nlevels, level_rows, 256, tot);
+  const int64_t M = tot / A;
+  const float* const a = relu ? lam : nullptr;
+  if (form == 1) return pad_cast_colsum_launch(SrcMeh<1>{lam, loss_noR, bbox_w4, g, lv}, true, a, dz, colsum, M, A, map, stream);
+  if (form == 2) return pad_cast_colsum_launch(SrcMeh<2>{lam, loss_noR, bbox_w4, g, lv}, true, a, dz, colsum, M, A, map, stream);
+  return pad_cast_colsum_launch(SrcMeh<0>{lam, loss_noR, bbox_w4, g, lv}, true, a, dz, colsum, M, A, map, stream);
+}
+extern "C" int aod_x3_box_levels_bwd_x(const float* bbox_pred, const float* bbox_tgt, const float* bbox_w, int nlevels, const int64_t* level_rows,
+                                       const float* g_sums, const float* divisors, void* dz, float* colsum, int A, void* map, aod_stream_t stream) {
+  AOD_CHECK_ARG(nlevels >= 1 && nlevels <= MAXLV && level_rows, "box_levels_bwd_x: 1..8 levels");
+  AOD_CHECK_ARG(bbox_pred && bbox_tgt && bbox_w && g_sums && A >= 1, "box_levels_bwd_x: bad args");
+  LossLevels lv; long long tot = 0;
+  for (int l = 0; l < nlevels; ++l) AOD_CHECK_ARG(level_rows[l] >= 0 && level_rows[l] % A == 0, "box_levels_bwd_x: a level's rows must be whole pixels");
+  fill_levels(lv, nlevels, level_rows, 256, tot);
+  const bool al16 = (((size_t)bbox_pred | (size_t)bbox_tgt | (size_t)bbox_w) & 15) == 0;
+  return pad_cast_colsum_launch(SrcBox{bbox_pred, bbox_tgt, bbox_w, g_sums + nlevels, divisors, nlevels, lv}, al16, nullptr, dz, colsum, tot / A, 4 * A, map,
+                                stream);
 }
 
 extern "C" int aod_x3_pad_cast_colsum(const float* g, const float* relu_out_f32, void* dz, float* colsum, int64_t M, int N, aod_stream_t stream) {
diff --git a/aod_meh_hua_amd/functional.py b/aod_meh_hua_amd/functional.py
--- a/aod_meh_hua_amd/functional.py
+++ b/aod_meh_hua_amd/functional.py
@@ -198,15 +198,68 @@
         for g in gs:
             if g is None:
                 continue
+            pend = _UP_PENDING.pop(g.data_ptr(), None) if _UP_PENDING else None
+            if pend is not None:
+                _, g_rows, dseg, sseg = pend
+                if tot is None:
+                    ho.upsample_add_bwd(g_rows, dseg, sseg, out=as_rows(g))
+                    tot = g
+                else:
+                    tot = as_nchw(ho.upsample_add_bwd_acc(g_rows, dseg, sseg, as_rows(tot)), g.shape[0], g.shape[2], g.shape[3])
+                continue
             g = g.contiguous(memory_format=torch.channels_last)
             tot = g if tot is None else as_nchw(ho.x3_add(as_rows(tot), as_rows(g)), g.shape[0], g.shape[2], g.shape[3])
         return tot, None
 
 
+_UP_PENDING = {}
+
+
 def fork(x, n):
     if not ho.X3 or n == 1 or not (torch.is_grad_enabled() and x.requires_grad):
         return [x] * n
-    return list(ForkFn.apply(x, n))
+    outs = list(ForkFn.apply(x, n))
+    for o in outs:
+        o._aod_fork = True
+    return outs
+
+
+class ForkLevelsFn(Function):
+
+    @staticmethod
+    def forward(ctx, n, *xs):
+        ctx.n, ctx.L = n, len(xs)
+        return tuple(x.view_as(x) for _ in range(n) for x in xs)
+
+    @staticmethod
+    def backward(ctx, *gs):
+        n, L = ctx.n, ctx.L
+        tots = [None] * L
+        for k in range(n):
+            pairs, where = [], []
+            for l in range(L):
+                g = gs[k * L + l]
+                if g is None:
+                    continue
+                g = g.contiguous(memory_format=torch.channels_last)
+                if tots[l] is None:
+                    tots[l] = g
+                else:
+                    pairs.append((as_rows(tots[l]), as_rows(g)))
+                    where.append((l, g.shape))
+            if pairs:
+                for (l, shp), o in zip(where, ho.x3_add_multi(pairs)):
+                    tots[l] = as_nchw(o, shp[0], shp[2], shp[3])
+        return (None,) + tuple(tots)
+
+
+def fork_levels(xs, n):
+    xs = list(xs)
+    if (ho.X3 and ho.HEAD_JUNCTION and n > 1 and len(xs) > 1 and torch.is_grad_enabled() and all(x.requires_grad for x in xs)
+            and all(x.dtype == torch.bfloat16 for x in xs)):
+        outs, L = ForkLevelsFn.apply(n, *xs), len(xs)
+        return [list(outs[k * L:(k + 1) * L]) for k in range(n)]
+    return [list(t) for t in zip(*[fork(x, n) for x in xs])]
 
 
 def get_precision():
@@ -339,6 +392,7 @@
 
 _S1_OF = {}
 _ROW_MAPS = {}
+_HEAD_PRE = {}
 MAP_LOG = None
 FWD_MAP_LOG = None
 
@@ -388,6 +442,12 @@
         _ROW_MAPS.clear()
         cls.flush()
         cls._verify()
+        if _UP_PENDING or _HEAD_PRE:
+            left = len(_UP_PENDING) + len(_HEAD_PRE)
+            _UP_PENDING.clear()
+            _HEAD_PRE.clear()
+            raise RuntimeError(f'head junction: {left} gradient placeholder(s) never reached the backward they were meant for (a prediction conv / '
+                               'a fork); the gradients behind them are undefined.  AOD_HEAD_JUNCTION=0 restores the two-step path')
 
     @classmethod
     def begin_pass(cls):
@@ -399,6 +459,8 @@
             cls.seen.clear()
             _S1_OF.clear()
             _ROW_MAPS.clear()
+            _UP_PENDING.clear()
+            _HEAD_PRE.clear()
             if tid >= 0:
                 torch.autograd.Variable._execution_engine.queue_callback(cls._end_of_pass)
 
@@ -493,7 +555,15 @@
         need_res = ctx.has_res and ctx.needs_input_grad[7]
         gw = ggamma = gbeta = gbias = gres = None
         if (meta['out_f32'] and X) or (Opad != O and not X):
-            if meta.get('sparse_grad') and X and ho.sparse_bwd():
+            pre = _HEAD_PRE.pop(g_rows.data_ptr(), None) if (X and _HEAD_PRE) else None
+            want_map = bool(meta.get('sparse_grad') and X and ho.sparse_bwd())
+            if pre is not None:
+                if not (pre[0].numel() == g_rows.numel() and tuple(pre[1].shape) == (g_rows.shape[0], Opad) and (pre[3] is not None) == want_map
+                        and pre[4] == bool(meta['relu'])):
+                    raise RuntimeError('head junction: the precomputed gradient rows do not fit the prediction conv that received them')
+                dz, gbias_v, rmap = pre[1], pre[2], pre[3]
+                _keep_map(dz, rmap)
+            elif want_map:
                 dz, gbias_v, rmap = ho.pad_cast_colsum(g_rows, Opad, a_rows if meta['relu'] else None, want_map=True)
                 _keep_map(dz, rmap)
             else:
@@ -647,7 +717,32 @@
     if meta.get('slot') is not None:
         for o in outs:
             o._aod_slot = meta['slot']
+    if out_f32 and ho.X3 and torch.is_grad_enabled():
+        tag = [bool(relu), bool(meta['sparse_grad']), [_weakref.ref(o) for o in outs]]
+        for o in outs:
+            o._aod_pred = tag
     return outs[0] if single else list(outs)
+
+
+def head_junction(levels):
+    if not (ho.X3 and ho.HEAD_JUNCTION and torch.is_grad_enabled()):
+        return None
+    tags = [getattr(t, '_aod_pred', None) for t in levels]
+    if tags[0] is None or any(t is not tags[0] for t in tags) or len(tags[0][2]) != len(tags):
+        return None
+    if any(t.retains_grad or t._backward_hooks for t in levels):
+        return None
+    return tags[0]
+
+
+def _junction_live(tag):
+    if tag is None or not (ho.X3 and ho.HEAD_JUNCTION) or torch.is_anomaly_enabled() or torch.is_grad_enabled():
+        return None
+    for r in tag[2]:
+        t = r()
+        if t is not None and (t.retains_grad or t._backward_hooks):
+            return None
+    return tag
 
 
 class ConvPairFn(Function):
@@ -1049,11 +1144,12 @@
 class UpsampleAddFn(Function):
 
     @staticmethod
-    def forward(ctx, lateral, top):
+    def forward(ctx, lateral, top, to_fork=False):
         B, C, H, W = lateral.shape
         h, w = top.shape[2:]
         out = ho.upsample_add(as_rows(lateral), Seg(B, H, W), as_rows(top), Seg(B, h, w))
         ctx.dims = (B, C, H, W, h, w)
+        ctx.to_fork = bool(to_fork)
         return as_nchw(out, B, H, W)
 
     @staticmethod
@@ -1062,8 +1158,15 @@
         g_rows = as_rows(g)
         gt = None
         if ctx.needs_input_grad[1]:
-            gt = as_nchw(ho.upsample_add_bwd(g_rows, Seg(B, H, W), Seg(B, h, w)), B, h, w)
-        return (g if ctx.needs_input_grad[0] else None), gt
+            if (ctx.to_fork and ho.X3 and ho.HEAD_JUNCTION and g_rows.dtype == torch.bfloat16 and not torch.is_anomaly_enabled()
+                    and not torch.is_grad_enabled()):
+                gt_rows = torch.empty(B * h * w, g_rows.shape[1], dtype=torch.bfloat16, device=g_rows.device)
+                _WgradQueue.begin_pass()
+                _UP_PENDING[gt_rows.data_ptr()] = (gt_rows, g_rows, Seg(B, H, W), Seg(B, h, w))
+                gt = as_nchw(gt_rows, B, h, w)
+            else:
+                gt = as_nchw(ho.upsample_add_bwd(g_rows, Seg(B, H, W), Seg(B, h, w)), B, h, w)
+        return (g if ctx.needs_input_grad[0] else None), gt, None
 
 
 def pyramid_buffer(shapes, channels, device, dtype=torch.bfloat16):
@@ -1077,7 +1180,7 @@
 
 
 def upsample_add(lateral, top):
-    return UpsampleAddFn.apply(lateral, top)
+    return UpsampleAddFn.apply(lateral, top, bool(getattr(top, '_aod_fork', False)))
 
 
 class PackedLosses(list):
@@ -1179,9 +1282,10 @@
 class RetinaLossLevelsFn(Function):
 
     @staticmethod
-    def forward(ctx, cls_rows, box_rows, labels, label_w, bbox_t, bbox_w, gamma, alpha, level_rows, shapes, num_pos=None, form='edl'):
+    def forward(ctx, cls_rows, box_rows, labels, label_w, bbox_t, bbox_w, gamma, alpha, level_rows, shapes, num_pos=None, form='edl', box_junction=None):
         ctx.set_materialize_grads(False)
         ctx.form = form
+        ctx.box_junction = box_junction
         div = nt = None
         if num_pos is None:
             noR, sums = ho.edl_focal_l1_levels_fwd(cls_rows, labels, label_w, box_rows, bbox_t, bbox_w, level_rows, gamma, alpha, form=form)
@@ -1209,9 +1313,14 @@
             g_rows = (g_noR.float() + torch.repeat_interleave(g2, _level_rows_dev(level_rows, dev), output_size=sum(level_rows))).contiguous()
         gc = torch.empty(cls_rows.shape[0] // A, AC, dtype=torch.float32, device=dev)
         gb = torch.empty(cls_rows.shape[0] // A, A4, dtype=torch.float32, device=dev)
-        ho.edl_focal_l1_levels_bwd(cls_rows, labels, label_w, box_rows, bbox_t, bbox_w, level_rows, g_sums, g_rows, gc, gb, A, gamma, alpha, divisors=div,
-                                   form=ctx.form)
-        return gc.view(cls_rows.shape), gb.view(box_rows.shape), None, None, None, None, None, None, None, None, None, None
+        bj = _junction_live(ctx.box_junction) if A4 == 4 * A else None
+        if bj is not None:
+            dzb, csb, mapb = ho.box_levels_bwd_x(box_rows, bbox_t, bbox_w, level_rows, g_sums, A, bool(bj[1] and ho.sparse_bwd()), divisors=div)
+            _WgradQueue.begin_pass()
+            _HEAD_PRE[gb.data_ptr()] = (gb, dzb, csb, mapb, bool(bj[0]))
+        ho.edl_focal_l1_levels_bwd(cls_rows, labels, label_w, box_rows, bbox_t, bbox_w, level_rows, g_sums, g_rows, gc, None if bj is not None else gb, A,
+                                   gamma, alpha, divisors=div, form=ctx.form)
+        return gc.view(cls_rows.shape), gb.view(box_rows.shape), None, None, None, None, None, None, None, None, None, None, None
 
 
 _LEVEL_ROWS_DEV = {}
@@ -1230,10 +1339,11 @@
 class MEHLossLevelsFn(Function):
 
     @staticmethod
-    def forward(ctx, lam, loss_noR, bbox_w, level_rows, A, form='l2'):
+    def forward(ctx, lam, loss_noR, bbox_w, level_rows, A, form='l2', junction=None):
         out = ho.meh_loss_levels_fwd(lam, loss_noR, bbox_w, level_rows, form=form)
         ctx.save_for_backward(lam, loss_noR, bbox_w)
         ctx.cfg = (tuple(level_rows), A, form)
+        ctx.junction = junction
         return out
 
     @staticmethod
@@ -1241,8 +1351,14 @@
         lam, loss_noR, bw = ctx.saved_tensors
         level_rows, A, form = ctx.cfg
         gl = torch.empty(lam.numel() // A, A, dtype=torch.float32, device=lam.device)
-        ho.meh_loss_levels_bwd(lam, loss_noR, bw, level_rows, g.float().contiguous(), gl, A, form=form)
-        return gl.view(lam.shape), None, None, None, None, None
+        j = _junction_live(ctx.junction)
+        if j is not None:
+            dz, cs, rmap = ho.meh_levels_bwd_x(lam, loss_noR, bw, level_rows, g.float().contiguous(), A, j[0], bool(j[1] and ho.sparse_bwd()), form=form)
+            _WgradQueue.begin_pass()
+            _HEAD_PRE[gl.data_ptr()] = (gl, dz, cs, rmap, bool(j[0]))
+        else:
+            ho.meh_loss_levels_bwd(lam, loss_noR, bw, level_rows, g.float().contiguous(), gl, A, form=form)
+        return gl.view(lam.shape), None, None, None, None, None, None
 
 
 class _LevelViewsFn(Function):
diff --git a/aod_meh_hua_amd/hipops.py b/aod_meh_hua_amd/hipops.py
--- a/aod_meh_hua_amd/hipops.py
+++ b/aod_meh_hua_amd/hipops.py
@@ -11,6 +11,15 @@
 
 X3 = False
 DETERMINISTIC = False
+
+
+HEAD_JUNCTION = os.environ.get('AOD_HEAD_JUNCTION', '1') != '0'
+
+
+def set_head_junction(on=True):
+    global HEAD_JUNCTION
+    prev, HEAD_JUNCTION = HEAD_JUNCTION, bool(on)
+    return prev
 
 
 def set_deterministic(on=True):
@@ -631,9 +640,18 @@
     return out
 
 
-def upsample_add_bwd(g_dst_rows, dst_seg: Seg, src_seg: Seg):
-    out = torch.empty(src_seg.rows, g_dst_rows.shape[1], dtype=torch.bfloat16, device=g_dst_rows.device)
+def upsample_add_bwd(g_dst_rows, dst_seg: Seg, src_seg: Seg, out=None):
+    if out is None:
+        out = torch.empty(src_seg.rows, g_dst_rows.shape[1], dtype=torch.bfloat16, device=g_dst_rows.device)
+    assert out.is_contiguous() and tuple(out.shape) == (src_seg.rows, g_dst_rows.shape[1]) and out.dtype == torch.bfloat16
     call('aod_x3_upsample2x_add_bwd_set' if X3 else 'aod_upsample2x_add_bwd_set', ptr(g_dst_rows), ptr(out), dst_seg.B, src_seg.H, src_seg.W, g_dst_rows.shape[1], dst_seg.H, dst_seg.W, stream())
+    return out
+
+
+def upsample_add_bwd_acc(g_dst_rows, dst_seg: Seg, src_seg: Seg, acc_rows):
+    assert X3 and acc_rows.dtype == torch.bfloat16 and acc_rows.is_contiguous() and tuple(acc_rows.shape) == (src_seg.rows, g_dst_rows.shape[1])
+    out = torch.empty_like(acc_rows)
+    call('aod_x3_upsample2x_add_bwd_acc', ptr(g_dst_rows), ptr(acc_rows), ptr(out), dst_seg.B, src_seg.H, src_seg.W, g_dst_rows.shape[1], dst_seg.H, dst_seg.W, stream())
     return out
 
 
@@ -786,6 +804,32 @@
         return grad
     call('aod_meh_loss_levels_bwd', ptr(lam), ptr(loss_noR), ptr(bbox_w4), L, lr, ptr(g), ptr(grad), 0, A, A, stream())
     return grad
+
+
+def meh_levels_bwd_x(lam, loss_noR, bbox_w4, level_rows, g, A, relu, want_map, form='l2'):
+    L = len(level_rows)
+    lr = _level_rows(level_rows)
+    assert X3 and g.shape == (L,) and g.is_contiguous() and g.dtype == torch.float32 and sum(level_rows) == lam.numel()
+    M = lam.numel() // A
+    dz = torch.empty(M, xw(A), dtype=torch.bfloat16, device=lam.device)
+    cs = zeros_f32(xw(A) // 2, lam.device)
+    rmap = row_map(M, lam.device) if want_map else None
+    call('aod_meh_loss_levels_bwd_x', ptr(lam), ptr(loss_noR), ptr(bbox_w4), L, lr, MEH_FORMS[form], ptr(g), int(bool(relu)), ptr(dz), ptr(cs), A,
+         ptr(rmap), stream())
+    return dz, cs, rmap
+
+
+def box_levels_bwd_x(bbox_pred, bbox_tgt, bbox_w, level_rows, g_sums, A, want_map, divisors=None):
+    L = len(level_rows)
+    lr = _level_rows(level_rows)
+    assert X3 and g_sums.shape == (3, L) and g_sums.is_contiguous() and g_sums.dtype == torch.float32 and sum(level_rows) == bbox_pred.shape[0]
+    M = bbox_pred.shape[0] // A
+    dz = torch.empty(M, xw(4 * A), dtype=torch.bfloat16, device=bbox_pred.device)
+    cs = zeros_f32(xw(4 * A) // 2, bbox_pred.device)
+    rmap = row_map(M, bbox_pred.device) if want_map else None
+    call('aod_x3_box_levels_bwd_x', ptr(bbox_pred), ptr(bbox_tgt), ptr(bbox_w), L, lr, ptr(g_sums), ptr(divisors), ptr(dz), ptr(cs), A, ptr(rmap),
+         stream())
+    return dz, cs, rmap
 
 
 def pad_cast_colsum(g, npad, relu_out=None, want_map=False):
@@ -851,6 +895,17 @@
     out = torch.empty_like(a)
     call('aod_x3_add', ptr(a), ptr(b), ptr(out), a.numel(), stream())
     return out
+
+
+def x3_add_multi(pairs):
+    outs = [torch.empty_like(a) for a, _ in pairs]
+    for k in range(0, len(pairs), 8):
+        ch, oc = pairs[k:k + 8], outs[k:k + 8]
+        n = len(ch)
+        vp = C.c_void_p * n
+        call('aod_x3_add_multi', n, vp(*[a.data_ptr() for a, _ in ch]), vp(*[b.data_ptr() for _, b in ch]), vp(*[o.data_ptr() for o in oc]),
+             (C.c_int64 * n)(*[a.numel() for a, _ in ch]), stream())
+    return outs
 
 
 def dropout2d_masks(table, image_ids, site_offsets, rate, seed, sample):
diff --git a/aod_meh_hua_amd/models/dense_heads/Lambda_L2.py b/aod_meh_hua_amd/models/dense_heads/Lambda_L2.py
--- a/aod_meh_hua_amd/models/dense_heads/Lambda_L2.py
+++ b/aod_meh_hua_amd/models/dense_heads/Lambda_L2.py
@@ -75,7 +75,7 @@
 
     def forward(self, feats, fwd_maps=None, **kwargs):
         feats = list(feats)
-        cls_feat, reg_feat = (list(t) for t in zip(*[AF.fork(f, 2) for f in feats]))
+        cls_feat, reg_feat = AF.fork_levels(feats, 2)
         if len(self.cls_convs) == len(self.reg_convs) and all(m.with_activation for m in list(self.cls_convs) + list(self.reg_convs)):
             ride = self._rides(feats)
             nl = len(self.cls_convs)
@@ -164,7 +164,7 @@
         level_rows = [c.shape[0] * c.shape[2] * c.shape[3] * A for c in cls_scores]
         out = AF.RetinaLossLevelsFn.apply(cls_d.view(-1, C), box_d.view(-1, 4), flat[0], flat[1], flat[2], flat[3],
                                           float(self.loss_cls.gamma), float(self.loss_cls.alpha), level_rows,
-                                          (A, cls_d.shape[1], box_d.shape[1]), num_pos, self._focal_form)
+                                          (A, cls_d.shape[1], box_d.shape[1]), num_pos, self._focal_form, AF.head_junction(bbox_preds))
         return (out[0], list(out[1].split(level_rows))) + tuple(out[2:])
 
     def loss_all_levels_L(self, L_scores, losses, bw_list, **kwargs):
@@ -177,7 +177,7 @@
         level_rows = [l.shape[0] * l.shape[2] * l.shape[3] * A for l in L_scores]
         if [int(t.numel()) for t in losses] != level_rows:
             return None
-        return AF.MEHLossLevelsFn.apply(lam_d.view(-1), noR, bw, level_rows, A, self._meh_form)
+        return AF.MEHLossLevelsFn.apply(lam_d.view(-1), noR, bw, level_rows, A, self._meh_form, AF.head_junction(L_scores))
 
     @force_fp32(apply_to=('L_score'))
     def loss_single_L(self, L_score, loss, label_weights, bbox_weights, sIdx=0, **kwargs):
diff --git a/aod_meh_hua_amd/models/dense_heads/MyRetinaHead.py b/aod_meh_hua_amd/models/dense_heads/MyRetinaHead.py
--- a/aod_meh_hua_amd/models/dense_heads/MyRetinaHead.py
+++ b/aod_meh_hua_amd/models/dense_heads/MyRetinaHead.py
@@ -38,7 +38,7 @@
 
     def forward(self, feats, **kwargs):
         feats = list(feats)
-        cls_feat, reg_feat = (list(t) for t in zip(*[AF.fork(f, 2) for f in feats]))
+        cls_feat, reg_feat = AF.fork_levels(feats, 2)
         if all(m.with_activation for m in list(self.cls_convs) + list(self.reg_convs)):
             for i, (cc, rc) in enumerate(zip(self.cls_convs, self.reg_convs)):
                 cls_feat, reg_feat = AF.conv_pair_act(cls_feat, reg_feat, cc.conv, rc.conv, sole_consumer=i > 0)
diff --git a/include/aod_hip.h b/include/aod_hip.h
--- a/include/aod_hip.h
+++ b/include/aod_hip.h
@@ -351,14 +351,20 @@
 int aod_x3_split(const float* src, void* dst, int64_t M, int C, aod_stream_t stream);
 int aod_x3_merge(const void* src, float* dst, int64_t M, int C, aod_stream_t stream);
 int aod_x3_add(const void* a, const void* b, void* out, int64_t n, aod_stream_t stream);
+int aod_x3_add_multi(int nranges, const void* const* a, const void* const* b, void* const* out, const int64_t* n, aod_stream_t stream);
 int aod_x3_nchw_f32_to_s2d(const float* src, void* dst, int B, int C, int H, int W, aod_stream_t stream);
 int aod_x3_maxpool3x3s2(const void* src, void* dst, int B, int H, int W, int C, aod_stream_t stream);
 int aod_x3_upsample2x_add_to(const void* top, const void* lateral, void* out, int B, int h, int w, int C, int H, int W, aod_stream_t stream);
 int aod_x3_upsample2x_add_bwd_set(const void* g_dst, void* g_src, int B, int h, int w, int C, int H, int W, aod_stream_t stream);
+int aod_x3_upsample2x_add_bwd_acc(const void* g_dst, const void* acc, void* g_src, int B, int h, int w, int C, int H, int W, aod_stream_t stream);
 int aod_x3_act_bwd(const void* g, const void* a, void* dz, float* colsum, int64_t M, int C, int relu, aod_stream_t stream);
 int aod_x3_pad_cast_colsum(const float* g, const float* relu_out_f32, void* dz, float* colsum, int64_t M, int N, aod_stream_t stream);
 int aod_x3_pad_cast_colsum_map(const float* g, const float* relu_out_f32, void* dz, float* colsum, int64_t M, int N, void* map,
                                aod_stream_t stream);
+int aod_meh_loss_levels_bwd_x(const float* lam, const float* loss_noR, const float* bbox_w4, int nlevels, const int64_t* level_rows, int form,
+                            const float* g, int relu, void* dz, float* colsum, int A, void* map, aod_stream_t stream);
+int aod_x3_box_levels_bwd_x(const float* bbox_pred, const float* bbox_tgt, const float* bbox_w, int nlevels, const int64_t* level_rows,
+                            const float* g_sums, const float* divisors, void* dz, float* colsum, int A, void* map, aod_stream_t stream);
 
 int aod_bottleneck64x3_fwd(const void* x, int Cin, int B, int H, int W, const void* w1, const float* s1, const float* b1, const void* w2,
                            const float* s2, const float* b2, const void* w3, const float* s3, const float* b3, const void* res, void* y,
```

New measurement: 757.3, median of 3. No clear change (-0.1%).
